# StandeHaas/Hydrodynamic-Limits-of-Active-Particle-Systems-with-Mean-Field-Interactions

Hardware: AMD Instinct MI355X
Metric: particle-steps/sec at N=1e5 (higher is better)
Workload: dtype f64; 1 GPU; BASELINE config 2: N=100000 particles, L=200000 sites, K=1, reflecting walls, sigma=0.005 (4001-tap table), beta=0.7, dt=0.0125, exclusion on; method=tiles

## Files before the change

### hydrodynamic-limits-of-active-particle-systems-with-mean-field-interactions_amd/capi.py

```python
from __future__ import annotations

import ctypes as C
import importlib.util
import os
import re
import sys

import numpy as np

HERE = os.path.dirname(os.path.abspath(__file__))
LIB_PATH = os.environ.get("APS_LIB") or os.path.join(HERE, "libaps_hip.so")
HEADER_PATH = os.path.join(os.path.dirname(HERE), "include", "aps.h")

APS_OK, APS_ERR_ARG, APS_ERR_HIP, APS_ERR_STATE, APS_ERR_NODEVICE = 0, -1, -2, -3, -4
METHODS = {"auto": 0, "pairs": 1, "lattice": 2, "tiles": 3}
KERNELS = ("pair_accumulate", "propose", "claim", "apply", "plan_tiles", "propose_lattice", "field_update", "tile_step")


class ApsError(RuntimeError):
    def __init__(self, code, text):
        super().__init__(f"libaps_hip error {code}: {text}")
        self.code = code


class ApsParams(C.Structure):
    _fields_ = [
        ("L", C.c_int32), ("K", C.c_int32), ("periodic", C.c_int32), ("minus_anchor", C.c_int32),
        ("immobilize", C.c_int32), ("suppress_flip", C.c_int32), ("crowding", C.c_int32),
        ("n_ensembles", C.c_int32), ("n_particles", C.c_int64), ("sigma_grid", C.c_double),
        ("rate_diffusion", C.c_double), ("rate_active", C.c_double), ("k_on", C.c_double),
        ("k_off", C.c_double), ("k_exit", C.c_double), ("dt", C.c_double), ("seed", C.c_uint64),
        ("beta", C.POINTER(C.c_double)), ("anchor_mask", C.POINTER(C.c_uint8)), ("device", C.c_int32),
        ("rank", C.c_int32), ("world", C.c_int32), ("sort_by_site", C.c_int32),
        ("ensemble_base", C.c_int32), ("method", C.c_int32), ("fp32", C.c_int32), ("halo_interval", C.c_int32),
    ]


_lib = None


def header_symbols():
    with open(HEADER_PATH) as fh:
        text = fh.read()
    return sorted(set(re.findall(r"\b(aps_[a-z_0-9]+)\s*\(", text)))


def _share_hip_runtime_with_torch():
    if "torch" in sys.modules or os.environ.get("APS_SYSTEM_HIP_RUNTIME") == "1":
        return None
    spec = importlib.util.find_spec("torch")
    if spec is None or not spec.submodule_search_locations:
        return None
    cand = os.path.join(list(spec.submodule_search_locations)[0], "lib", "libamdhip64.so")
    return C.CDLL(cand, mode=C.RTLD_GLOBAL) if os.path.exists(cand) else None


def load():
    global _lib
    if _lib is not None:
        return _lib
    _share_hip_runtime_with_torch()
    if not os.path.exists(LIB_PATH):
        raise ImportError(f"{LIB_PATH} is missing: build it with `python {os.path.join(HERE, 'build.py')}` "
                          "(hipcc --offload-arch=gfx950). There is no CPU fallback.")
    lib = C.CDLL(LIB_PATH)
    vp, i32, i64, dbl = C.c_void_p, C.c_int32, C.c_int64, C.c_double
    P = C.POINTER
    protos = {
        "aps_device_count": (C.c_int, []),
        "aps_last_error": (C.c_char_p, [vp]),
        "aps_create": (C.c_int, [P(ApsParams), P(vp)]),
        "aps_destroy": (None, [vp]),
        "aps_set_stream": (C.c_int, [vp, vp]),
        "aps_set_state": (C.c_int, [vp, i32, vp, vp, vp, vp, i64]),
        "aps_get_state": (C.c_int, [vp, i32, vp, vp, vp, vp, i64]),
        "aps_pair_accumulate": (C.c_int, [vp, i32, vp, vp, vp, i64]),
        "aps_step": (C.c_int, [vp, i64]),
        "aps_propose": (C.c_int, [vp]),
        "aps_commit": (C.c_int, [vp]),
        "aps_exchange_buffer": (C.c_int, [vp, P(vp), P(i64), P(i64), P(i64)]),
        "aps_bind_exchange_buffer": (C.c_int, [vp, vp, i64]),
        "aps_observe": (C.c_int, [vp, i32, vp, vp, vp]),
        "aps_field_from_counts": (C.c_int, [vp, i32, vp, vp, vp]),
        "aps_time": (C.c_int, [vp, P(dbl), P(i64)]),
        "aps_get_exits": (C.c_int, [vp, i32, vp, i64, P(i64)]),
        "aps_get_table": (C.c_int, [vp, vp, i32, P(i32), P(i32)]),
        "aps_resort": (C.c_int, [vp]),
        "aps_step_timed": (C.c_int, [vp, i64, P(dbl), P(i64), P(dbl)]),
        "aps_step_profile": (C.c_int, [vp, i64, vp, vp]),
        "aps_step_info": (C.c_int, [vp, P(i64), P(i64)]),
        "aps_set_resident_loop": (C.c_int, [vp, i32]),
        "aps_step_loop_timed": (C.c_int, [vp, i64, P(dbl), P(i64)]),
        "aps_loop_info": (C.c_int, [vp, P(i64), P(i32), C.c_char_p, i32]),
        "aps_copy_bandwidth": (C.c_int, [vp, i64, i32, P(dbl)]),
        "aps_lattice_accumulate": (C.c_int, [vp, i32, vp, vp, vp, i64]),
        "aps_get_lattice": (C.c_int, [vp, i32, vp, vp, vp]),
        "aps_method": (C.c_int, [vp]),
        "aps_mark_reference": (C.c_int, [vp, i32]),
        "aps_observe_scalars": (C.c_int, [vp, i32, i32, i32, i32, vp, vp]),
        "aps_observe_scalars_all": (C.c_int, [vp, i32, vp, vp, vp]),
        "aps_event_overhead": (C.c_int, [vp, i32, P(dbl)]),
        "aps_observe_structure": (C.c_int, [vp, i32, i32, vp]),
        "aps_observe_bins": (C.c_int, [vp, i32, i32, vp, vp]),
        "aps_rates_from_field": (C.c_int, [vp, i32, vp, vp, vp, i64, vp, vp, vp, vp]),
        "aps_comm_unique_id": (C.c_int, [vp]),
        "aps_comm_init": (C.c_int, [vp, vp]),
        "aps_comm_ranks": (C.c_int, [vp, P(i32)]),
        "aps_owned_sites": (C.c_int, [vp, P(i32), P(i32)]),
        "aps_halo_copy": (C.c_int, [vp, vp]),
        "aps_halo_pack": (C.c_int, [vp, i32, vp, i64, P(i64)]),
        "aps_halo_unpack": (C.c_int, [vp, i32, vp, i64]),
        "aps_halo_info": (C.c_int, [vp, P(i32), P(i32), P(i32)]),
        "aps_comm_selftest": (C.c_int, [vp, i64]),
        "aps_halo_sizes": (C.c_int, [vp, P(i64), P(i64)]),
        "aps_ipc_export": (C.c_int, [vp, vp]),
        "aps_ipc_connect": (C.c_int, [vp, vp, vp]),
        "aps_exchange_kind": (C.c_int, [vp]),
        "aps_set_flip_table": (C.c_int, [vp, vp, i32]),
        "aps_ntt_info": (C.c_int, [vp, P(i32), P(i32), P(dbl), P(i64)]),
        "aps_ntt_launches": (C.c_int, [vp]),
        "aps_tiles_info": (C.c_int, [vp, P(i32), P(i32), P(i32), P(i32)]),
    }
    lenient = os.environ.get("APS_LIB_LENIENT") == "1"
    for name, (res, args) in protos.items():
        if lenient and not hasattr(lib, name):
            continue
        fn = getattr(lib, name)
        fn.restype, fn.argtypes = res, args
    lib._aps_protos = protos
    _lib = lib
    return lib


def _ptr(a):
    return None if a is None else a.ctypes.data_as(C.c_void_p)


class Handle:

    def __init__(self, *, L, K, periodic, sigma_grid, rate_diffusion, rate_active, beta, dt, seed,
                 n_particles, minus_anchor=True, immobilize=True, suppress_flip=True, crowding=False,
                 k_on=0.0, k_off=0.0, k_exit=0.0, anchor_mask=None, device=0, rank=0, world=1,
                 sort_by_site=True, ensemble_base=0, method="auto", fp32=False, halo_interval=0):
        self.lib = load()
        self._h = C.c_void_p()
        betas = np.atleast_1d(np.asarray(beta, dtype=np.float64)).copy()
        self.E, self.n, self.L, self.K = len(betas), int(n_particles), int(L), int(K)
        self.dt = float(dt)
        mask = None if anchor_mask is None else np.ascontiguousarray(anchor_mask, dtype=np.uint8)
        if mask is not None and not mask.any():
            mask = None
        par = ApsParams(L=L, K=K, periodic=int(bool(periodic)), minus_anchor=int(bool(minus_anchor)),
                        immobilize=int(bool(immobilize)), suppress_flip=int(bool(suppress_flip)),
                        crowding=int(bool(crowding)), n_ensembles=self.E, n_particles=self.n,
                        sigma_grid=float(sigma_grid), rate_diffusion=float(rate_diffusion),
                        rate_active=float(rate_active), k_on=float(k_on), k_off=float(k_off),
                        k_exit=float(k_exit), dt=self.dt, seed=int(seed) & (2 ** 64 - 1),
                        beta=betas.ctypes.data_as(C.POINTER(C.c_double)),
                        anchor_mask=None if mask is None else mask.ctypes.data_as(C.POINTER(C.c_uint8)),
                        device=int(device), rank=int(rank), world=int(world),
                        sort_by_site=int(bool(sort_by_site)), ensemble_base=int(ensemble_base), method=METHODS[method],
                        fp32=int(bool(fp32)), halo_interval=int(halo_interval))
        rc = self.lib.aps_create(C.byref(par), C.byref(self._h))
        if rc != APS_OK:
            raise ApsError(rc, self.lib.aps_last_error(None).decode())
        self.method = {1: "pairs", 2: "lattice", 3: "tiles"}[self.lib.aps_method(self._h)]

    def _ck(self, rc):
        if rc != APS_OK:
            raise ApsError(rc, self.lib.aps_last_error(self._h).decode())

    def close(self):
        if getattr(self, "_h", None) is not None and self._h.value:
            self.lib.aps_destroy(self._h)
            self._h = C.c_void_p()

    def __del__(self):
        try:
            self.close()
        except Exception:
            pass

    def set_stream(self, raw_stream):
        self._ck(self.lib.aps_set_stream(self._h, C.c_void_p(raw_stream)))

    def set_state(self, pos, sigma, bound=None, alive=None, ensemble=0):
        pos = np.ascontiguousarray(pos, dtype=np.int32)
        sigma = np.ascontiguousarray(sigma, dtype=np.int8)
        bound = None if bound is None else np.ascontiguousarray(bound, dtype=np.uint8)
        alive = None if alive is None else np.ascontiguousarray(alive, dtype=np.uint8)
        self._ck(self.lib.aps_set_state(self._h, ensemble, _ptr(pos), _ptr(sigma), _ptr(bound), _ptr(alive), len(pos)))
        self._n_set = getattr(self, "_n_set", {})
        self._n_set[ensemble] = len(pos)

    def get_state(self, ensemble=0):
        n = self._n_set[ensemble]
        pos, sigma = np.zeros(n, np.int32), np.zeros(n, np.int8)
        bound, alive = np.zeros(n, np.uint8), np.zeros(n, np.uint8)
        self._ck(self.lib.aps_get_state(self._h, ensemble, _ptr(pos), _ptr(sigma), _ptr(bound), _ptr(alive), n))
        return pos, sigma, bound, alive

    def pair_accumulate(self, ensemble=0):
        n = self._n_set[ensemble]
        S, W, occ4 = np.zeros(n), np.zeros(n), np.zeros((n, 4), np.int32)
        self._ck(self.lib.aps_pair_accumulate(self._h, ensemble, _ptr(S), _ptr(W), _ptr(occ4), n))
        return S, W, occ4

    def lattice_accumulate(self, ensemble=0):
        n = self._n_set[ensemble]
        S, W, occ4 = np.zeros(n), np.zeros(n), np.zeros((n, 4), np.int32)
        self._ck(self.lib.aps_lattice_accumulate(self._h, ensemble, _ptr(S), _ptr(W), _ptr(occ4), n))
        return S, W, occ4

    def get_lattice(self, ensemble=0):
        W, S, occ = np.zeros(self.L), np.zeros(self.L), np.zeros(self.L, np.int32)
        self._ck(self.lib.aps_get_lattice(self._h, ensemble, _ptr(W), _ptr(S), _ptr(occ)))
        return W, S, occ

    def step(self, nsteps=1):
        self._ck(self.lib.aps_step(self._h, int(nsteps)))

    def propose(self):
        self._ck(self.lib.aps_propose(self._h))

    def commit(self):
        self._ck(self.lib.aps_commit(self._h))

    def exchange_buffer(self):
        ptr, tot, off, mine = C.c_void_p(), C.c_int64(), C.c_int64(), C.c_int64()
        self._ck(self.lib.aps_exchange_buffer(self._h, C.byref(ptr), C.byref(tot), C.byref(off), C.byref(mine)))
        return ptr.value, tot.value, off.value, mine.value

    def bind_exchange_buffer(self, dev_ptr, nbytes):
        self._ck(self.lib.aps_bind_exchange_buffer(self._h, C.c_void_p(dev_ptr), int(nbytes)))

    def comm_init(self, id128: bytes):
        buf = (C.c_uint8 * 128).from_buffer_copy(id128)
        self._ck(self.lib.aps_comm_init(self._h, C.cast(buf, C.c_void_p)))

    def owned_sites(self):
        lo, hi = C.c_int32(), C.c_int32()
        self._ck(self.lib.aps_owned_sites(self._h, C.byref(lo), C.byref(hi)))
        return lo.value, hi.value

    def halo_from(self, neighbour):
        self._ck(self.lib.aps_halo_copy(self._h, neighbour._h))

    def halo_info(self):
        k, age, due = C.c_int32(0), C.c_int32(0), C.c_int32(0)
        self._ck(self.lib.aps_halo_info(self._h, C.byref(k), C.byref(age), C.byref(due)))
        return int(k.value), int(age.value), bool(due.value)

    def halo_sizes(self):
        snd, rcv = (C.c_int64 * 2)(), (C.c_int64 * 2)()
        self._ck(self.lib.aps_halo_sizes(self._h, snd, rcv))
        return (int(snd[0]), int(snd[1])), (int(rcv[0]), int(rcv[1]))

    def halo_pack(self, side):
        n = C.c_int64()
        self._ck(self.lib.aps_halo_pack(self._h, int(side), None, 0, C.byref(n)))
        buf = np.zeros(max(n.value, 1), np.uint8)
        self._ck(self.lib.aps_halo_pack(self._h, int(side), _ptr(buf), len(buf), C.byref(n)))
        return buf[:n.value]

    def halo_unpack(self, from_side, data):
        data = np.ascontiguousarray(data, dtype=np.uint8)
        self._ck(self.lib.aps_halo_unpack(self._h, int(from_side), _ptr(data), len(data)))

    def comm_selftest(self, nbytes=1 << 16):
        self._ck(self.lib.aps_comm_selftest(self._h, int(nbytes)))

    def ipc_export(self) -> bytes:
        buf = (C.c_uint8 * 256)()
        self._ck(self.lib.aps_ipc_export(self._h, C.cast(buf, C.c_void_p)))
        return bytes(buf)

    def ipc_connect(self, left_blob, right_blob):
        keep = [None if b is None else (C.c_uint8 * 256).from_buffer_copy(b) for b in (left_blob, right_blob)]
        self._ck(self.lib.aps_ipc_connect(self._h, *[None if k is None else C.cast(k, C.c_void_p) for k in keep]))

    def set_flip_table(self, table):
        if table is None:
            self._ck(self.lib.aps_set_flip_table(self._h, None, 0))
            return
        tab = np.ascontiguousarray(table, dtype=np.float64)
        assert tab.ndim == 2 and tab.shape[0] == 2 and tab.shape[1] >= 2
        self._ck(self.lib.aps_set_flip_table(self._h, _ptr(tab), tab.shape[1] - 1))

    def ntt_info(self):
        on, m, ms, n = C.c_int32(), C.c_int32(), C.c_double(), C.c_int64()
        self._ck(self.lib.aps_ntt_info(self._h, C.byref(on), C.byref(m), C.byref(ms), C.byref(n)))
        return dict(on=bool(on.value), log2_m=m.value, prof_ms=ms.value, prof_launches=n.value, launches=int(self.lib.aps_ntt_launches(self._h)))

    def tiles_info(self):
        v = [C.c_int32() for _ in range(4)]
        self._ck(self.lib.aps_tiles_info(self._h, *[C.byref(x) for x in v]))
        return dict(frame_sites=v[0].value, owned_sites=v[1].value, n_tiles=v[2].value, table_in_lds=bool(v[3].value))

    def exchange_kind(self):
        return {0: "none", 1: "rccl", 2: "ipc-peer"}[self.lib.aps_exchange_kind(self._h)]

    def comm_ranks(self):
        n = C.c_int32()
        self._ck(self.lib.aps_comm_ranks(self._h, C.byref(n)))
        return n.value

    def step_timed(self, nsteps):
        ms, n, pairs = C.c_double(), C.c_int64(), C.c_double()
        self._ck(self.lib.aps_step_timed(self._h, int(nsteps), C.byref(ms), C.byref(n), C.byref(pairs)))
        return ms.value, n.value, pairs.value

    def step_profile(self, nsteps):
        ms, cnt = np.zeros(len(KERNELS)), np.zeros(len(KERNELS), np.int64)
        self._ck(self.lib.aps_step_profile(self._h, int(nsteps), _ptr(ms), _ptr(cnt)))
        return {k: (float(m), int(c)) for k, m, c in zip(KERNELS, ms, cnt)}

    def step_info(self):
        g, k = C.c_int64(), C.c_int64()
        self._ck(self.lib.aps_step_info(self._h, C.byref(g), C.byref(k)))
        return g.value, k.value

    def set_resident_loop(self, on=True):
        self._ck(self.lib.aps_set_resident_loop(self._h, 1 if on else 0))

    def step_loop_timed(self, nsteps):
        ms, n = C.c_double(), C.c_int64()
        self._ck(self.lib.aps_step_loop_timed(self._h, int(nsteps), C.byref(ms), C.byref(n)))
        return ms.value, n.value

    def loop_info(self):
        n, st, why = C.c_int64(), C.c_int32(), C.create_string_buffer(256)
        self._ck(self.lib.aps_loop_info(self._h, C.byref(n), C.byref(st), why, 256))
        return n.value, st.value, why.value.decode()

    def copy_bandwidth(self, nbytes=1 << 30, reps=5):
        r = C.c_double()
        self._ck(self.lib.aps_copy_bandwidth(self._h, int(nbytes), int(reps), C.byref(r)))
        return r.value

    def event_overhead(self, reps=50):
        ms = C.c_double()
        self._ck(self.lib.aps_event_overhead(self._h, int(reps), C.byref(ms)))
        return ms.value

    SCALARS = ("n", "sum_sigma", "sum_pos", "n_wall", "max_pos", "n_range", "attempts", "blocked", "sum_d", "sum_d2", "n_d")

    def mark_reference(self, ensemble=0):
        self._ck(self.lib.aps_mark_reference(self._h, ensemble))

    def observe_scalars(self, ensemble=0, x_wall=0, range_lo=0, range_hi=-1, block_table=None):
        out = np.zeros(len(self.SCALARS), np.int64)
        tab = None if block_table is None else np.ascontiguousarray(block_table, dtype=np.uint8)
        if tab is not None and tab.size != (self.K + 1) ** 2:
            raise ValueError("block_table must have (K+1)*(K+1) entries")
        self._ck(self.lib.aps_observe_scalars(self._h, ensemble, int(x_wall), int(range_lo), int(range_hi), _ptr(tab), _ptr(out)))
        return {k: int(v) for k, v in zip(self.SCALARS, out)}

    def observe_scalars_all(self, x_wall=0, ranges=None, block_table=None):
        out = np.zeros((self.E, len(self.SCALARS)), np.int64)
        tab = None if block_table is None else np.ascontiguousarray(block_table, dtype=np.uint8)
        rng = None if ranges is None else np.ascontiguousarray(ranges, dtype=np.int32).reshape(self.E, 2)
        self._ck(self.lib.aps_observe_scalars_all(self._h, int(x_wall), _ptr(rng), _ptr(tab), _ptr(out)))
        return [{k: int(v) for k, v in zip(self.SCALARS, row)} for row in out]

    def observe_bins(self, nbins, ensemble=0):
        cp, cm = np.zeros(nbins, np.int64), np.zeros(nbins, np.int64)
        self._ck(self.lib.aps_observe_bins(self._h, ensemble, int(nbins), _ptr(cp), _ptr(cm)))
        return cp, cm

    def observe_structure(self, ensemble=0, k_max=25):
        k_max = int(min(k_max, self.L))
        out = np.zeros(4 + 2 * k_max)
        self._ck(self.lib.aps_observe_structure(self._h, ensemble, k_max, _ptr(out)))
        return int(out[0]), float(out[1]), float(out[2]), float(out[3]), out[4:].reshape(k_max, 2)

    def observe(self, ensemble=0, want_field=True):
        cp, cm = np.zeros(self.L, np.int64), np.zeros(self.L, np.int64)
        m = np.zeros(self.L) if want_field else None
        self._ck(self.lib.aps_observe(self._h, ensemble, _ptr(cp), _ptr(cm), _ptr(m)))
        return cp, cm, m

    def field_from_counts(self, counts_p, counts_m, ensemble=0):
        cp = np.ascontiguousarray(counts_p, dtype=np.int64)
        cm = np.ascontiguousarray(counts_m, dtype=np.int64)
        m = np.zeros(self.L)
        self._ck(self.lib.aps_field_from_counts(self._h, ensemble, _ptr(cp), _ptr(cm), _ptr(m)))
        return m

    def rates_from_field(self, pos, sigma, bound, m_field, counts_p, counts_m, ensemble=0):
        pos = np.ascontiguousarray(pos, dtype=np.int32)
        sigma = np.ascontiguousarray(sigma, dtype=np.int8)
        bound = np.ascontiguousarray(bound, dtype=np.uint8)
        m_field = np.ascontiguousarray(m_field, dtype=np.float64)
        cp = np.ascontiguousarray(counts_p, dtype=np.int64)
        cm = np.ascontiguousarray(counts_m, dtype=np.int64)
        out = np.zeros((9, len(pos)))
        self._ck(self.lib.aps_rates_from_field(self._h, ensemble, _ptr(pos), _ptr(sigma), _ptr(bound), len(pos), _ptr(m_field),
                                               _ptr(cp), _ptr(cm), _ptr(out)))
        return dict(zip(("diff", "act", "flip", "bind", "unbind", "exit", "left", "right", "total"), out))

    def time(self):
        t, k = C.c_double(), C.c_int64()
        self._ck(self.lib.aps_time(self._h, C.byref(t), C.byref(k)))
        return t.value, k.value

    def exits(self, ensemble=0):
        n = C.c_int64()
        self._ck(self.lib.aps_get_exits(self._h, ensemble, None, 0, C.byref(n)))
        rows = np.zeros((max(n.value, 1), 3))
        self._ck(self.lib.aps_get_exits(self._h, ensemble, _ptr(rows), len(rows), C.byref(n)))
        return rows[:n.value]

    def table(self):
        tlen, q = C.c_int32(), C.c_int32()
        self._ck(self.lib.aps_get_table(self._h, None, 0, C.byref(tlen), C.byref(q)))
        out = np.zeros(max(tlen.value, 1))
        self._ck(self.lib.aps_get_table(self._h, _ptr(out), len(out), C.byref(tlen), C.byref(q)))
        return out[:tlen.value], q.value

    def resort(self):
        self._ck(self.lib.aps_resort(self._h))


def device_count():
    return load().aps_device_count()


def comm_unique_id() -> bytes:
    lib = load()
    buf = (C.c_uint8 * 128)()
    rc = lib.aps_comm_unique_id(C.cast(buf, C.c_void_p))
    if rc != APS_OK:
        raise ApsError(rc, lib.aps_last_error(None).decode())
    return bytes(buf)
```

### hydrodynamic-limits-of-active-particle-systems-with-mean-field-interactions_amd/csrc/aps_hip.hip

```cpp

#include <hip/hip_runtime.h>
#include <hip/hip_ext.h>
#include <dlfcn.h>
#include <unistd.h>
#include <rccl/rccl.h>
#include <algorithm>
#include <cmath>
#include <cstdint>
#include <cstdio>
#include <cstdlib>
#include <cstring>
#include <numeric>
#include <string>
#include <vector>

#include "aps.h"
#include "aps_common.hpp"
#include "dev_mem.hpp"

namespace {

constexpr uint32_t POS_MASK = 0x07FFFFFFu;
constexpr uint32_t SPIN_BIT = 1u << 27;
constexpr uint32_t BOUND_BIT = 1u << 28;
// ... 1161 lines not shown
            (uint32_t)s | ((c & CELL_PLUS) ? SPIN_BIT : 0u) | ((c & CELL_BOUND) ? BOUND_BIT : 0u);
    }
    occ_site[(size_t)e * L + s] = (uint32_t)n;
}

__global__ __launch_bounds__(256) void mark_away(uint32_t *src, size_t n) {
    const size_t i = (size_t)blockIdx.x * blockDim.x + threadIdx.x;
    if (i < n && !(src[i] & DEAD_BIT)) src[i] |= AWAY_BIT;
}

__global__ __launch_bounds__(256) void derive_slots(const uint32_t *__restrict__ src, uint32_t *sp8, int4 *tinfo, int Npad, int ntiles) {
    const size_t slot = (size_t)blockIdx.x * blockDim.x + threadIdx.x;
    const int e = blockIdx.y;
    const uint32_t me = src[(size_t)e * Npad + slot];
    const bool live = !(me & (DEAD_BIT | AWAY_BIT));
    const int p = (int)(me & POS_MASK);
    sp8[(size_t)e * Npad + slot] = live ? (((uint32_t)p << 3) | ((me & SPIN_BIT) ? 1u : 0u)) : DEAD_P8;
    int lo = live ? p : 0x7fffffff, hi = live ? p : -1, cnt = live ? 1 : 0;
#pragma unroll
    for (int off = 32; off > 0; off >>= 1) {
        lo = min(lo, __shfl_xor(lo, off)); hi = max(hi, __shfl_xor(hi, off)); cnt += __shfl_xor(cnt, off);
    }
    if ((threadIdx.x & 63) == 0) tinfo[(size_t)e * ntiles + slot / TILE] = make_int4(lo, hi, cnt < TILE ? 1 : 0, cnt);
}

__global__ __launch_bounds__(256) void tile_parts(const uint32_t *__restrict__ cell, long long *gpart, long long *gsum, int L, int K, int own, int ntile) {
    const int tile = blockIdx.x, e = blockIdx.y;
    const int s0 = tile * own, s1 = min(s0 + own, L);
    long long sp = 0, n = 0;
    for (int i = threadIdx.x; i < (s1 - s0) * K; i += blockDim.x) {
        const uint32_t c = cell[((size_t)e * L + s0) * K + i];
        if (c != CELL_EMPTY) { sp += (c & CELL_PLUS) ? 1 : -1; n += 1; }
    }
    __shared__ long long acc[2];
    if (threadIdx.x == 0) acc[0] = acc[1] = 0;
    __syncthreads();
    const long long a0 = wave_sum(sp), a1 = wave_sum(n);
    if ((threadIdx.x & 63) == 0) {
        atomicAdd(reinterpret_cast<unsigned long long *>(&acc[0]), (unsigned long long)a0);
        atomicAdd(reinterpret_cast<unsigned long long *>(&acc[1]), (unsigned long long)a1);
    }
    __syncthreads();
    if (threadIdx.x == 0) {
        gpart[((size_t)e * ntile + tile) * 2] = acc[0]; gpart[((size_t)e * ntile + tile) * 2 + 1] = acc[1];
        atomicAdd(reinterpret_cast<unsigned long long *>(&gsum[2 * e]), (unsigned long long)acc[0]);
        atomicAdd(reinterpret_cast<unsigned long long *>(&gsum[2 * e + 1]), (unsigned long long)acc[1]);
    }
}

__global__ __launch_bounds__(256) void structure_sites(const uint32_t *__restrict__ cnt_pm, const double *__restrict__ m_field, int L, double *out) {
    double c2 = 0.0, m1 = 0.0, m2 = 0.0;
    for (int x = blockIdx.x * blockDim.x + threadIdx.x; x < L; x += gridDim.x * blockDim.x) {
        const uint32_t c = cnt_pm[x];
        const double tot = (double)((c & 0xFFFFu) + (c >> 16)), m = m_field[x];
        c2 += tot * tot; m1 += m; m2 += m * m;
    }
#pragma unroll
    for (int off = 32; off > 0; off >>= 1) { c2 += __shfl_xor(c2, off); m1 += __shfl_xor(m1, off); m2 += __shfl_xor(m2, off); }
    if ((threadIdx.x & 63) == 0) { atomicAdd(&out[1], c2); atomicAdd(&out[2], m1); atomicAdd(&out[3], m2); }
}

__global__ __launch_bounds__(256) void structure_dft(const uint32_t *__restrict__ src, int Npad, int L, double *out) {
    const int k = blockIdx.x;
    double re = 0.0, im = 0.0, n = 0.0;
    for (int i = threadIdx.x; i < Npad; i += blockDim.x) {
        const uint32_t w = src[i];
        if (w & (DEAD_BIT | AWAY_BIT)) continue;
        const long long r = ((long long)k * (long long)(w & POS_MASK)) % (long long)L;
        double sn, cs;
        sincospi(-2.0 * ((double)r / (double)L), &sn, &cs);
        re += cs; im += sn; n += 1.0;
    }
    __shared__ double acc[3];
    if (threadIdx.x < 3) acc[threadIdx.x] = 0.0;
    __syncthreads();
#pragma unroll
    for (int off = 32; off > 0; off >>= 1) { re += __shfl_xor(re, off); im += __shfl_xor(im, off); n += __shfl_xor(n, off); }
    if ((threadIdx.x & 63) == 0) { atomicAdd(&acc[0], re); atomicAdd(&acc[1], im); atomicAdd(&acc[2], n); }
    __syncthreads();
    if (threadIdx.x == 0) { out[4 + 2 * k] = acc[0]; out[5 + 2 * k] = acc[1]; if (k == 0) out[0] = acc[2]; }
}

__global__ __launch_bounds__(256) void bin_counts(const uint32_t *__restrict__ src, int Npad, int bin_sites, unsigned long long *plus, unsigned long long *minus,
                                                  int site_lo, int site_hi) {
    const int i = blockIdx.x * blockDim.x + threadIdx.x;
    if (i >= Npad) return;
    const uint32_t w = src[i];
    if (w & (DEAD_BIT | AWAY_BIT)) return;
    if ((int)(w & POS_MASK) < site_lo || (int)(w & POS_MASK) >= site_hi) return;
    atomicAdd(((w & SPIN_BIT) ? plus : minus) + (w & POS_MASK) / (uint32_t)bin_sites, 1ull);
}

std::string g_create_error;

}

struct aps_handle {
    DevMem mem;
    aps_params p{};
    Model model{};
    std::vector<double> beta;
    std::vector<double> table;
    int tlen = 0, q = 0;
    bool table_in_lds = true;
    size_t lds_bytes = 0, lds_bytes_field = 0;
    int E = 1, world = 1, rank = 0;
    int64_t N = 0, Npad = 0, SH = 0, ntiles = 0;
    hipStream_t stream = nullptr;
    bool own_stream = false;
    uint32_t *d_src = nullptr, *d_orig = nullptr, *d_pcnt = nullptr, *d_plist = nullptr;
    uint8_t *d_prop = nullptr, *d_prop_own = nullptr, *d_anchor = nullptr;
    uint32_t *d_sp8 = nullptr;
    int4 *d_tinfo = nullptr;
    unsigned long long *d_stamps = nullptr;
    uint32_t *d_plan = nullptr, *d_plan_n = nullptr;
    double *d_accW = nullptr, *d_accS = nullptr;
    unsigned *d_occ = nullptr;
    int split = 1;
    bool plan_dirty = true;
    int plan_interval = 1, plan_age = 0;
    int num_cu = 256, wgs_per_cu = 1;
    double *d_table = nullptr, *d_beta = nullptr, *d_exit = nullptr, *d_S = nullptr, *d_W = nullptr, *d_mfield = nullptr;
    int *d_occ4 = nullptr;
    long long *d_gsum = nullptr;
    unsigned *d_nexit = nullptr;
    uint32_t *d_tmp_sp8 = nullptr; int4 *d_tmp_tinfo = nullptr; size_t tmp_cap = 0;
    int exit_cap = 0;
    int64_t step = 0;
    std::vector<int64_t> n_set;
    std::vector<hipEvent_t> events;
    ncclComm_t comm = nullptr;
    int method = APS_METHOD_PAIRS;
    double2 *d_ws = nullptr;
    uint32_t *d_occ_site = nullptr;
    uint32_t *d_dcnt = nullptr, *d_dep = nullptr;
    unsigned long long *d_stepw = nullptr;
    int bshift = 8, nb = 0, dcap = 0, fu_R = 1;
    bool fu_table_in_lds = true;
    bool field_dirty = true;
    hipStream_t cap_stream = nullptr;
    hipGraphExec_t gexec_f[2][2][6] = {};
    hipGraphExec_t gexact_f[2][2][65] = {};
    bool graphs_built_f[2] = {false, false};
    int flip = 0;
    int64_t last_graph_steps = 0, last_single_steps = 0;
    double2 *d_wsb[2] = {nullptr, nullptr};
    uint32_t *d_cell[2] = {nullptr, nullptr}, *d_tdcnt[2] = {nullptr, nullptr}, *d_tdep[2] = {nullptr, nullptr};
    long long *d_gpart[2] = {nullptr, nullptr};
    uint32_t *d_slot_of = nullptr;
    Model *d_model = nullptr; TileRare *d_rare = nullptr;
    unsigned long long *d_xrec = nullptr;
    unsigned *d_abort = nullptr, *h_abort = nullptr, *h_abort_dev = nullptr;
    int loop_rec = 0, loop_drec = 0, loop_seg = 0;
    int loop_state = -2;
    int loop_wanted = 1;
    uint32_t loop_tag = 0;
    int64_t last_loop_steps = 0;
    unsigned loop_stall = 0u;
    uint32_t *loop_dbg = nullptr; int loop_dbg_n = 0;
    bool loop_timed = false;
    hipEvent_t loop_ev[2] = {nullptr, nullptr};
    std::string loop_why;
    bool f32 = false, ws_view_stale = false;
    double *d_flip_tab = nullptr;
    bool ntt_on = false, ntt_fused = false;
    NttPlan ntt{};
    uint32_t *d_ntt_sig = nullptr, *d_ntt_tab = nullptr;
    int *d_ntt_csig = nullptr;
    double prof_ntt_ms = 0.0; int64_t prof_ntt_n = 0;
    int *d_table_i = nullptr;
    int2 *d_wsi[2] = {nullptr, nullptr};
    int ts_lo = 0, ts_hi = 0, own_lo = 0, own_hi = 0, ts_reach = 0;
    int ts_kx = 1, halo_age = 0;
    unsigned halo_got = 0;
    char *d_halo_send[2] = {nullptr, nullptr}, *d_halo_recv[2] = {nullptr, nullptr};
    HaloSegD *d_halo_seg_send[2] = {nullptr, nullptr}, *d_halo_seg_recv[2] = {nullptr, nullptr};
    int halo_nseg_send[2] = {0, 0}, halo_nseg_recv[2] = {0, 0};
    size_t halo_bytes_send[2] = {0, 0}, halo_bytes_recv[2] = {0, 0};
    char *ipc_land = nullptr;
    size_t ipc_land_bytes = 0, ipc_land_off[2][2] = {{0, 0}, {0, 0}};
    char *ipc_peer[2] = {nullptr, nullptr};
    void *ipc_opened[2] = {nullptr, nullptr};
    size_t ipc_peer_off[2][2] = {{0, 0}, {0, 0}};
    unsigned *d_ipc_done = nullptr, *h_ipc_err = nullptr, *h_ipc_err_dev = nullptr;
    uint32_t ipc_seq = 0;
    bool ipc_on = false;
    int ts_RS = 2, ts_own = 124, ts_ntile = 0, ts_dcap = 0;
    bool ts_table_in_lds = true;
    bool slots_dirty = false;
    bool field_pending = false;
    uint32_t *d_ref = nullptr, *d_cnt_pm = nullptr;
    uint8_t *d_block_table = nullptr, *d_ref_ok = nullptr; long long *d_scal = nullptr; int *d_lo_hi = nullptr;
    std::vector<char> ref_set;
    bool profiling = false;
    std::vector<int> prof_kind;
    size_t prof_n = 0;
    bool prof_dispatch = true;
    hipEvent_t k_start = nullptr, k_stop = nullptr;
    std::string err;
};

namespace {

#define HIP_TRY(h, expr)                                                                         \
    do {                                                                                         \
        hipError_t e_ = (expr);                                                                  \
        if (e_ != hipSuccess) {                                                                  \
            (h)->err = std::string(#expr) + ": " + hipGetErrorString(e_);                        \
            return APS_ERR_HIP;                                                                  \
        }                                                                                        \
    } while (0)

int fail(aps_handle *h, int code, const std::string &msg) { h->err = msg; return code; }
void drop_graphs(aps_handle *h);

struct Rccl {
    void *lib = nullptr;
    ncclResult_t (*GetUniqueId)(ncclUniqueId *) = nullptr;
    ncclResult_t (*CommInitRank)(ncclComm_t *, int, ncclUniqueId, int) = nullptr;
    ncclResult_t (*AllGather)(const void *, void *, size_t, ncclDataType_t, ncclComm_t, hipStream_t) = nullptr;
    ncclResult_t (*CommDestroy)(ncclComm_t) = nullptr;
    ncclResult_t (*CommCount)(const ncclComm_t, int *) = nullptr;
    ncclResult_t (*Send)(const void *, size_t, ncclDataType_t, int, ncclComm_t, hipStream_t) = nullptr;
    ncclResult_t (*Recv)(void *, size_t, ncclDataType_t, int, ncclComm_t, hipStream_t) = nullptr;
    ncclResult_t (*GroupStart)() = nullptr;
    ncclResult_t (*GroupEnd)() = nullptr;
    const char *(*GetErrorString)(ncclResult_t) = nullptr;
    std::string err;
    bool load() {
        if (lib) return true;
        for (const char *name : {"librccl.so.1", "librccl.so", "/opt/rocm/lib/librccl.so.1"}) {
            lib = dlopen(name, RTLD_NOW | RTLD_GLOBAL);
            if (lib) break;
        }
        if (!lib) { err = std::string("cannot load librccl: ") + dlerror(); return false; }
        GetUniqueId = reinterpret_cast<decltype(GetUniqueId)>(dlsym(lib, "ncclGetUniqueId"));
        CommInitRank = reinterpret_cast<decltype(CommInitRank)>(dlsym(lib, "ncclCommInitRank"));
        AllGather = reinterpret_cast<decltype(AllGather)>(dlsym(lib, "ncclAllGather"));
        CommDestroy = reinterpret_cast<decltype(CommDestroy)>(dlsym(lib, "ncclCommDestroy"));
        GetErrorString = reinterpret_cast<decltype(GetErrorString)>(dlsym(lib, "ncclGetErrorString"));
        CommCount = reinterpret_cast<decltype(CommCount)>(dlsym(lib, "ncclCommCount"));
        Send = reinterpret_cast<decltype(Send)>(dlsym(lib, "ncclSend"));
        Recv = reinterpret_cast<decltype(Recv)>(dlsym(lib, "ncclRecv"));
        GroupStart = reinterpret_cast<decltype(GroupStart)>(dlsym(lib, "ncclGroupStart"));
        GroupEnd = reinterpret_cast<decltype(GroupEnd)>(dlsym(lib, "ncclGroupEnd"));
        if (!GetUniqueId || !CommInitRank || !AllGather || !CommDestroy || !GetErrorString || !CommCount || !Send || !Recv || !GroupStart || !GroupEnd) {
            err = "librccl lacks a required symbol"; lib = nullptr; return false;
        }
        return true;
    }
} g_rccl;

void build_table(aps_handle *h) { weight_table(h->p.sigma_grid, h->p.L, h->p.K, h->p.periodic != 0, h->table, h->tlen, h->q, h->p.fp32 ? 29 : 51); }

template <typename T>
int dev_alloc(aps_handle *h, T **ptr, size_t count) {
    HIP_TRY(h, h->mem.alloc(ptr, count));
    HIP_TRY(h, hipMemsetAsync(*ptr, 0, std::max<size_t>(count, 1) * sizeof(T), h->stream));
    return APS_OK;
}

void derive_sources(const std::vector<uint32_t> &src, std::vector<uint32_t> &sp8, std::vector<int4> &tinfo) {
    const size_t n = src.size(), nt = n / TILE;
    sp8.resize(n);
    tinfo.assign(nt, make_int4(0x7fffffff, -1, 1, 0));
    for (size_t s = 0; s < n; ++s) {
        const uint32_t w = src[s];
        const bool live = !(w & DEAD_BIT);
        sp8[s] = live ? (((w & POS_MASK) << 3) | ((w & SPIN_BIT) ? 1u : 0u)) : DEAD_P8;
        if (!live) continue;
        int4 &t = tinfo[s / TILE];
        const int p = (int)(w & POS_MASK);
        t.x = std::min(t.x, p); t.y = std::max(t.y, p); t.w += 1;
    }
    for (int4 &t : tinfo) t.z = t.w < TILE ? 1 : 0;
}

void pack_ensemble(const aps_handle *h, const int32_t *pos, const int8_t *sigma, const uint8_t *bound,
                   const uint8_t *alive, int64_t n, std::vector<uint32_t> &src, std::vector<uint32_t> &orig,
                   long long gsum[2]) {
    const int64_t Npad = h->Npad;
    std::vector<uint32_t> order((size_t)n);
    std::iota(order.begin(), order.end(), 0u);
    if (h->p.sort_by_site)
        std::stable_sort(order.begin(), order.end(), [&](uint32_t a, uint32_t b) {
            const bool da = alive && !alive[a], db = alive && !alive[b];
            if (da != db) return db;
            return pos[a] < pos[b];
        });
    src.assign((size_t)Npad, DEAD_BIT);
    orig.assign((size_t)Npad, 0xFFFFFFFFu);
    gsum[0] = gsum[1] = 0;
    for (int64_t s = 0; s < n; ++s) {
        const uint32_t i = order[(size_t)s];
        uint32_t w = (uint32_t)pos[i] & POS_MASK;
        if (sigma[i] > 0) w |= SPIN_BIT;
        if (bound && bound[i]) w |= BOUND_BIT;
        const bool dead = alive && !alive[i];
        if (dead) w |= DEAD_BIT;
        else { gsum[0] += sigma[i] > 0 ? 1 : -1; gsum[1] += 1; }
        src[(size_t)s] = w;
        orig[(size_t)s] = i;
    }
}

int upload_ensemble(aps_handle *h, int e, const std::vector<uint32_t> &src, const std::vector<uint32_t> &orig) {
// ... 429 lines not shown

int ntt_setup(aps_handle *h) {
    h->ntt_on = false;
    const char *env = std::getenv("APS_NTT");
    if (env && env[0] == '0') return APS_OK;
    const bool forced = env && env[0] == '1';
    if (!is_tiles(h) || !h->model.field_mode) return APS_OK;
    if (h->ts_table_in_lds && !forced) return APS_OK;
    const int Rt = h->tlen - 1, L = h->p.L;
    const bool shard = h->world > 1;
    int64_t span = (int64_t)L + 2 * Rt;
    if (!shard) {
        if (h->p.periodic ? !(2 * Rt <= L && L >= 4 * TD_SITES) : !(2 * Rt + 64 * h->ts_RS + h->ts_own + 4 < L)) return APS_OK;
    } else {
        const char *kenv = std::getenv("APS_HALO_INTERVAL");
        if (h->p.halo_interval > 1 || (h->p.halo_interval == 0 && kenv && std::atoi(kenv) > 1)) return APS_OK;
        int own_min = L, own_max = 0;
        for (int r = 0; r < h->world; ++r) {
            int lo, hi;
            rank_tiles(h, r, lo, hi);
            const int n = std::min(L, hi * h->ts_own) - lo * h->ts_own;
            own_min = std::min(own_min, n); own_max = std::max(own_max, n);
        }
        span = (int64_t)own_max + 2 * (Rt + TD_HALO);
        if (own_min < Rt + TD_HALO + 1 || (h->p.periodic && span > L)) return APS_OK;
    }
    const int np = h->f32 ? 1 : 2;
    int m = shard && np == 2 ? 15 : 14;
    while (((int64_t)1 << m) < span) ++m;
    if (m > 21 || (np == 2 && m < 15) || td_lds_bytes(h->p.K) > 160 * 1024) return APS_OK;
    if (td_lds_bytes(h->p.K) > 48 * 1024) {
        const void *fn = h->f32 ? reinterpret_cast<const void *>(&tile_dense<false, true>) : reinterpret_cast<const void *>(&tile_dense<false, false>);
        if (hipFuncSetAttribute(fn, hipFuncAttributeMaxDynamicSharedMemorySize, (int)td_lds_bytes(h->p.K)) != hipSuccess) { (void)hipGetLastError(); return APS_OK; }
    }
    double wsum = 0.0;
    for (int t = 0; t < h->tlen; ++t) wsum += std::ldexp(h->table[(size_t)t], h->q) * (t ? 2.0 : 1.0);
    if (2.0 * h->p.K * wsum >= 0.5 * (np == 1 ? (double)NTT_PRIMES[0] : (double)NTT_PRIMES[0] * (double)NTT_PRIMES[1])) return APS_OK;
    NttPlan &pl = h->ntt;
    pl.m = m; ntt_split(m, pl.a0, pl.a1, pl.a2); pl.L = L; pl.Rt = Rt; pl.E = h->E; pl.np = np;
    pl.org = shard ? h->own_lo - Rt - TD_HALO : -Rt;
    pl.out_lo = shard ? h->own_lo - TD_HALO : 0;
    pl.out_hi = shard ? h->own_hi + TD_HALO : L;
    if (shard && !h->p.periodic) { pl.out_lo = std::max(pl.out_lo, 0); pl.out_hi = std::min(pl.out_hi, L); }
    pl.crt_inv = ntt_powmod(NTT_PRIMES[0] % NTT_PRIMES[1], NTT_PRIMES[1] - 2ull, NTT_PRIMES[1]);
    pl.unit = std::ldexp(1.0, -h->q);
    const size_t M = (size_t)1 << m;
    NttTables T[2];
    for (int k = 0; k < np; ++k) ntt_build_tables(m, NTT_PRIMES[k], NTT_ROOTS[k], T[k]);
    const size_t o_wr = 0, o_t1 = o_wr + T[0].wr.size(), o_hi = o_t1 + T[0].t1.size(), o_lo = o_hi + T[0].t2hi.size(), o_what = o_lo + T[0].t2lo.size(),
                 o_whatp = o_what + M, per_prime = o_whatp + M;
    int rc;
    if ((rc = dev_alloc(h, &h->d_ntt_tab, per_prime * np)) || (rc = dev_alloc(h, &h->d_ntt_sig, (size_t)np * h->E * 2 * M)) ||
        (rc = dev_alloc(h, &h->d_ntt_csig, (size_t)h->E * 2 * M))) return rc;
    for (int k = 0; k < np; ++k) {
        uint32_t *tb = h->d_ntt_tab + (size_t)k * per_prime;
        HIP_TRY(h, hipMemcpyAsync(tb + o_wr, T[k].wr.data(), T[k].wr.size() * 4, hipMemcpyHostToDevice, h->stream));
        HIP_TRY(h, hipMemcpyAsync(tb + o_t1, T[k].t1.data(), T[k].t1.size() * 4, hipMemcpyHostToDevice, h->stream));
        HIP_TRY(h, hipMemcpyAsync(tb + o_hi, T[k].t2hi.data(), T[k].t2hi.size() * 4, hipMemcpyHostToDevice, h->stream));
        HIP_TRY(h, hipMemcpyAsync(tb + o_lo, T[k].t2lo.data(), T[k].t2lo.size() * 4, hipMemcpyHostToDevice, h->stream));
        NttPrime &pp = pl.pr[k];
        pp.P = NTT_PRIMES[k]; pp.md.P = (double)NTT_PRIMES[k]; pp.md.Pinv = 1.0 / (double)NTT_PRIMES[k];
        pp.wr = tb + o_wr; pp.t1 = tb + o_t1; pp.t2hi = tb + o_hi; pp.t2lo = tb + o_lo; pp.what = tb + o_what; pp.whatp = tb + o_whatp;
    }
    if (np == 1) pl.pr[1] = pl.pr[0];
    const char *fenv = std::getenv("APS_NTT_FUSED");
    h->ntt_fused = pl.a0 == 7 && pl.a1 == 7 && pl.a2 >= 1 && !(fenv && fenv[0] == '0');
    if (h->ntt_fused && hipFuncSetAttribute(reinterpret_cast<const void *>(&ntt_mid), hipFuncAttributeMaxDynamicSharedMemorySize, (int)NTT_MID_LDS) != hipSuccess) {
        (void)hipGetLastError(); h->ntt_fused = false;
    }
    {
        NttPlan ps = pl;
        ps.E = 1;
        std::vector<uint32_t> wext((size_t)np * 2 * M, 0u);
        for (int k = 0; k < np; ++k)
            for (int t = 0; t < h->tlen; ++t) {
                const uint32_t v = (uint32_t)((unsigned long long)std::ldexp(h->table[(size_t)t], h->q) % NTT_PRIMES[k]);
                wext[(size_t)k * 2 * M + (size_t)t] = v;
                if (t && !(h->p.periodic && 2 * t == L)) wext[(size_t)k * 2 * M + M - (size_t)t] = v;
            }
        HIP_TRY(h, hipMemcpyAsync(h->d_ntt_sig, wext.data(), wext.size() * 4, hipMemcpyHostToDevice, h->stream));
        const dim3 grid((unsigned)(M / NTT_TILE), 1u, (unsigned)np), block(NTT_THREADS);
        if (pl.a2 > 0) ntt_launch_strided<2, false, 1>(pl.a2, grid, block, h->stream, nullptr, nullptr, false, ps, h->d_ntt_sig, nullptr, nullptr, 0);
        ntt_launch_strided<1, false, 1>(pl.a1, grid, block, h->stream, nullptr, nullptr, false, ps, h->d_ntt_sig, nullptr, nullptr, 0);
        hipLaunchKernelGGL((ntt_contig<true>), grid, block, 0, h->stream, ps, h->d_ntt_sig);
        HIP_TRY(h, hipGetLastError());
        std::vector<uint32_t> spec(M), specp;
        for (int k = 0; k < np; ++k) {
            HIP_TRY(h, hipMemcpyAsync(spec.data(), h->d_ntt_sig + (size_t)k * 2 * M, M * 4, hipMemcpyDeviceToHost, h->stream));
            HIP_TRY(h, hipStreamSynchronize(h->stream));
            const uint32_t P = NTT_PRIMES[k], minv = ntt_powmod((uint32_t)(M % P), P - 2ull, P);
            for (size_t i = 0; i < M; ++i) spec[i] = ntt_mulmod_u64(spec[i], minv, P);
            HIP_TRY(h, hipMemcpy(h->d_ntt_tab + (size_t)k * per_prime + o_what, spec.data(), M * 4, hipMemcpyHostToDevice));
            if (h->ntt_fused) {
                specp.resize(M);
                auto brev7 = [](size_t v) { size_t r = 0; for (int b = 0; b < 7; ++b) r |= ((v >> b) & 1) << (6 - b); return r; };
                for (size_t k2 = 0; k2 < (M >> 14); ++k2)
                    for (size_t s0 = 0; s0 < 128; ++s0)
                        for (size_t s1 = 0; s1 < 128; ++s1) specp[(k2 << 14) + s0 * 128 + s1] = spec[(k2 << 14) + brev7(s1) * 128 + brev7(s0)];
                HIP_TRY(h, hipMemcpy(h->d_ntt_tab + (size_t)k * per_prime + o_whatp, specp.data(), M * 4, hipMemcpyHostToDevice));
            }
        }
    }
    HIP_TRY(h, hipMemsetAsync(h->d_ntt_sig, 0, (size_t)np * h->E * 2 * M * 4, h->stream));
    HIP_TRY(h, hipStreamSynchronize(h->stream));
    if (h->d_wsi[1] != h->d_wsi[0]) { h->mem.release(h->d_wsi[1]); h->d_wsi[1] = h->d_wsi[0]; }
    if (!h->f32 && h->d_wsb[1] != h->d_wsb[0]) { h->mem.release(h->d_wsb[1]); h->d_wsb[1] = h->d_wsb[0]; }
    if (shard) h->ts_kx = 1;
    h->ntt_on = true;
    return APS_OK;
}

template <bool F32>
const void *tl_kernel_f(bool periodic, int RS, bool k1) {
#define TL_PICK(BC, R) (k1 ? (const void *)&tile_loop<BC, R, true, F32> : (const void *)&tile_loop<BC, R, false, F32>)
#define TL_CASE(R) case R: return periodic ? TL_PICK(1, R) : TL_PICK(0, R);
    if (!F32 && (RS == 8 || (RS == 7 && !k1))) return nullptr;
#ifdef APS_DEV_RS
    switch (RS) { TL_CASE(APS_DEV_RS) default: return nullptr; }
#else
    if constexpr (F32) { if (RS == 8) return periodic ? TL_PICK(1, 8) : TL_PICK(0, 8); }
    switch (RS) {
        TL_CASE(1) TL_CASE(2) TL_CASE(3) TL_CASE(4) TL_CASE(5) TL_CASE(6)
        case 7: return k1 ? (periodic ? (const void *)&tile_loop<1, 7, true, F32> : (const void *)&tile_loop<0, 7, true, F32>)
                          : (F32 ? (periodic ? (const void *)&tile_loop<1, 7, false, true> : (const void *)&tile_loop<0, 7, false, true>) : nullptr);
        default: return nullptr;
    }
#endif
#undef TL_CASE
#undef TL_PICK
}
const void *tl_kernel(const aps_handle *h) {
    return h->f32 ? tl_kernel_f<true>(h->p.periodic != 0, h->ts_RS, h->p.K == 1) : tl_kernel_f<false>(h->p.periodic != 0, h->ts_RS, h->p.K == 1);
}

int loop_prepare(aps_handle *h) {
    if (h->loop_state != -2) return APS_OK;
    h->loop_state = 0;
    auto no = [&](const char *why) { h->loop_why = why; return APS_OK; };
    if (!is_tiles(h)) return no("not the tiles formulation");
    if (h->world != 1) return no("sharded handle");
    if (h->ntt_on) return no("field updated by the exact convolution");
    if (!h->ts_table_in_lds) return no("weight table beyond LDS");
    if (!h->model.field_mode) return no("global mean field");
    if (h->p.K == 1 && h->model.immobilize && h->model.k_exit > 0.0) return no("particles can leave the system (one cell per site)");
    if (3 * h->p.K > 32) return no("site capacity above 10");
    if (h->p.L - (int64_t)(h->ts_ntile - 1) * h->ts_own < 3) return no("last tile shorter than three sites");
#ifdef APS_STAMPS
    return no("diagnostic build");
#endif
    const void *fn = tl_kernel(h);
    if (!fn) return no("no kernel for this frame");
    const int64_t need_per_cu = ((int64_t)h->ts_ntile * h->E + h->num_cu - 1) / h->num_cu;
    h->loop_seg = 0;
    size_t lds_total = 0;
    for (int seg : {256, 192, 128, TL_SEG_MIN}) {
        const TlLds lay = tl_lds_layout(h->tlen, h->ts_RS, h->ts_own, h->p.K, ts_wbytes(h), seg);
        if (lay.total > 160 * 1024) continue;
        if (128 / (int)((lay.total + 1279) / 1280) >= need_per_cu) { h->loop_seg = seg; lds_total = lay.total; break; }
    }
    if (!h->loop_seg) return no("more tiles than the device keeps resident at once (LDS)");
    if (lds_total > 48 * 1024 && hipFuncSetAttribute(fn, hipFuncAttributeMaxDynamicSharedMemorySize, (int)lds_total) != hipSuccess) { (void)hipGetLastError(); return no("hipFuncSetAttribute failed"); }
    int per_cu = 0;
    if (hipOccupancyMaxActiveBlocksPerMultiprocessor(&per_cu, fn, FU_THREADS, lds_total) != hipSuccess) { (void)hipGetLastError(); return no("occupancy query failed"); }
    if (need_per_cu > std::min(per_cu, 8)) return no("more tiles than the device keeps resident at once");
    h->loop_drec = (h->ts_dcap / 16 + 1) * 16;
    h->loop_rec = (h->loop_drec + 6 * h->p.K + 15) / 16 * 16;
    int rc;
    if ((rc = dev_alloc(h, &h->d_xrec, (size_t)2 * h->E * h->ts_ntile * h->loop_rec)) || (rc = dev_alloc(h, &h->d_abort, 4))) return rc;
    HIP_TRY(h, h->mem.alloc_host_mapped(&h->h_abort, &h->h_abort_dev, 16));
    h->h_abort[0] = 0u;
    h->loop_tag = 0;
    h->loop_state = 1;
    return APS_OK;
}

int launch_tile_loop(aps_handle *h, int64_t n) {
    LoopArgs la{};
    la.a = tile_args(h, false);
    la.a.tile_lo = 0;
    la.step0 = (unsigned long long)h->step;
    la.nsteps = (int)n;
    if ((uint64_t)h->loop_tag + (uint64_t)n + 2 > 0xFFFFFFF0ull) {
        HIP_TRY(h, hipMemsetAsync(h->d_xrec, 0, (size_t)2 * h->E * h->ts_ntile * h->loop_rec * sizeof(unsigned long long), h->stream));
        h->loop_tag = 0;
    }
    la.tag0 = h->loop_tag;
    h->loop_tag += (uint32_t)n + 1u;
    la.rec = h->loop_rec; la.drec = h->loop_drec; la.xrec = h->d_xrec; la.seg = h->loop_seg;
    la.abort_dev = h->d_abort; la.abort_host = h->h_abort_dev;
    la.timeout_ticks = 5000000ull;
    if (const char *env = std::getenv("APS_LOOP_TIMEOUT_MS")) la.timeout_ticks = (unsigned long long)std::max(1, std::atoi(env)) * 100000ull;
#ifdef APS_LOOP_DEBUG
    static uint32_t *dbg = nullptr;
    if (!dbg) (void)hipMalloc(reinterpret_cast<void **>(&dbg), (size_t)64 * 3 * h->p.L * 4);
    (void)hipMemsetAsync(dbg, 0xEE, (size_t)64 * 3 * h->p.L * 4, h->stream);
    la.dbg = n <= 64 ? dbg : nullptr;
    h->loop_dbg = dbg; h->loop_dbg_n = (int)n;
#endif
    if (std::getenv("APS_LOOP_TEST_ABORT")) HIP_TRY(h, hipMemsetAsync(h->d_abort, 1, 4, h->stream));
    {
        unsigned stall = 0u;
        if (const char *env = std::getenv("APS_LOOP_TEST_STALL")) {
            int st_tile = -1, st_it = 0;
            if (std::sscanf(env, "%d:%d", &st_tile, &st_it) == 2 && st_tile >= 0 && st_tile < h->ts_ntile && st_it >= 0 && st_it < 0xFFFF)
                stall = ((unsigned)(st_tile + 1) << 16) | (unsigned)st_it;
        }
        if (stall != h->loop_stall) {
            HIP_TRY(h, hipMemcpyAsync(h->d_abort + 1, &stall, 4, hipMemcpyHostToDevice, h->stream));
            HIP_TRY(h, hipStreamSynchronize(h->stream));
            h->loop_stall = stall;
        }
    }
    const void *fn = tl_kernel(h);
    const size_t lds = tl_lds_layout(h->tlen, h->ts_RS, h->ts_own, h->p.K, ts_wbytes(h), h->loop_seg).total;
    const void *table_ptr = h->f32 ? (const void *)h->d_table_i : (const void *)h->d_table;
    void *args[] = {(void *)&la, (void *)&table_ptr};
    const dim3 grid((unsigned)h->ts_ntile, (unsigned)h->E), block(FU_THREADS);
    if (h->loop_timed) {
        for (hipEvent_t &ev : h->loop_ev) if (!ev) HIP_TRY(h, hipEventCreate(&ev));
        HIP_TRY(h, hipExtLaunchKernel(fn, grid, block, args, lds, h->stream, h->loop_ev[0], h->loop_ev[1], 0));
    } else
        HIP_TRY(h, hipLaunchKernel(fn, grid, block, args, lds, h->stream));
    return APS_OK;
}

struct HaloSeg { size_t off, bytes; int array; };

void halo_segments(const aps_handle *h, int owner_lo_tile, int owner_hi_tile, int side, bool recv, std::vector<HaloSeg> &out) {
    const int L = h->p.L, K = h->p.K, own = h->ts_own;
    const int s_lo = owner_lo_tile * own, s_hi = std::min(L, owner_hi_tile * own);
    if (h->ntt_on) {
        const int reach = h->ntt.Rt + TD_HALO;
        const size_t M = (size_t)1 << h->ntt.m;
        const int p0 = !recv ? (side == 0 ? s_lo - 1 : s_hi - reach) - h->ntt.org
                             : (side == 0 ? h->own_hi - 1 : h->own_lo - reach) - h->ntt.org;
        for (int e = 0; e < h->E; ++e) {
            const int c0 = side == 0 ? s_lo : s_hi - 3, c1 = side == 0 ? s_lo + 3 : s_hi;
            out.push_back({((size_t)e * L + c0) * K * 4, (size_t)(c1 - c0) * K * 4, 0});
            for (int sg = 0; sg < 2; ++sg) out.push_back({(((size_t)e * 2 + sg) * M + (size_t)p0) * 4, (size_t)(reach + 1) * 4, 4});
        }
        return;
    }
    const int nt = std::min(h->ts_kx * h->ts_reach, owner_hi_tile - owner_lo_tile);
    const int64_t gs = (int64_t)(h->ts_kx - 1) * h->ts_reach * own;
    for (int e = 0; e < h->E; ++e) {
        const int64_t g1 = std::min<int64_t>(s_hi, (int64_t)owner_hi_tile * own - gs);
        const int c0 = side == 0 ? s_lo : (int)std::max<int64_t>(s_lo, g1 - 3);
        const int c1 = side == 0 ? (int)std::min<int64_t>(s_hi, s_lo + gs + 3) : s_hi;
        const int w0 = side == 0 ? s_lo : (int)std::max<int64_t>(s_lo, g1 - 2);
        const int w1 = side == 0 ? (int)std::min<int64_t>(s_hi, s_lo + gs + 2) : s_hi;
        const int t0 = side == 0 ? owner_lo_tile : owner_hi_tile - nt, t1 = t0 + nt;
        out.push_back({((size_t)e * L + c0) * K * 4, (size_t)(c1 - c0) * K * 4, 0});
        if (h->model.field_mode) {
            out.push_back({((size_t)e * L + w0) * 2 * ts_wbytes(h), (size_t)(w1 - w0) * 2 * ts_wbytes(h), 1});
            out.push_back({((size_t)e * h->ts_ntile + t0) * 4, (size_t)(t1 - t0) * 4, 2});
            out.push_back({((size_t)e * h->ts_ntile + t0) * h->ts_dcap * 4, (size_t)(t1 - t0) * h->ts_dcap * 4, 3});
        }
    }
}

char *halo_array(aps_handle *h, int array, int buf) {
    switch (array) {
        case 0: return reinterpret_cast<char *>(h->d_cell[buf]);
        case 1: return h->f32 ? reinterpret_cast<char *>(h->d_wsi[buf]) : reinterpret_cast<char *>(h->d_wsb[buf]);
        case 2: return reinterpret_cast<char *>(h->d_tdcnt[buf]);
        case 3: return reinterpret_cast<char *>(h->d_tdep[buf]);
        default: return reinterpret_cast<char *>(h->d_ntt_csig);
    }
}

void rank_tiles(const aps_handle *h, int r, int &lo, int &hi) {
    lo = (int)((int64_t)r * h->ts_ntile / h->world);
    hi = (int)((int64_t)(r + 1) * h->ts_ntile / h->world);
}

void halo_peers(const aps_handle *h, int &left, int &right) {
    left = h->rank - 1; right = h->rank + 1;
    if (h->p.periodic) { left = (left + h->world) % h->world; right %= h->world; }
    else { if (right >= h->world) right = -1; }
}

int halo_setup(aps_handle *h) {
    int left, right, lo, hi;
    halo_peers(h, left, right);
    for (int side = 0; side < 2; ++side) {
        for (int recv = 0; recv < 2; ++recv) {
            std::vector<HaloSeg> segs;
            if (!recv) halo_segments(h, h->ts_lo, h->ts_hi, side, false, segs);
            else {
                const int peer = side == 0 ? right : left;
                if (peer < 0) continue;
                rank_tiles(h, peer, lo, hi);
                halo_segments(h, lo, hi, side, true, segs);
            }
            std::vector<HaloSegD> tab;
            size_t off = 0;
            for (const HaloSeg &g : segs) {
                if (!g.bytes) continue;
                tab.push_back({(unsigned long long)g.off, (unsigned long long)off, (unsigned)g.bytes, g.array});
                off += (g.bytes + 15) / 16 * 16;
            }
            HaloSegD **dseg = recv ? &h->d_halo_seg_recv[side] : &h->d_halo_seg_send[side];
            char **dmsg = recv ? &h->d_halo_recv[side] : &h->d_halo_send[side];
            (recv ? h->halo_nseg_recv[side] : h->halo_nseg_send[side]) = (int)tab.size();
            (recv ? h->halo_bytes_recv[side] : h->halo_bytes_send[side]) = off;
            int rc;
            if ((rc = dev_alloc(h, dseg, tab.size())) || (rc = dev_alloc(h, dmsg, off))) return rc;
            HIP_TRY(h, hipMemcpyAsync(*dseg, tab.data(), tab.size() * sizeof(HaloSegD), hipMemcpyHostToDevice, h->stream));
        }
    }
    HIP_TRY(h, hipStreamSynchronize(h->stream));
    return APS_OK;
}

int halo_launch(aps_handle *h, int side, bool unpack) {
    const int buf = (int)((h->step & 1) ^ 1);
    const int nseg = unpack ? h->halo_nseg_recv[side] : h->halo_nseg_send[side];
    if (!nseg) return APS_OK;
    hipLaunchKernelGGL(halo_move, dim3((unsigned)(nseg * HALO_BPS)), dim3(256), 0, h->stream,
                       unpack ? h->d_halo_seg_recv[side] : h->d_halo_seg_send[side], halo_array(h, 0, buf), halo_array(h, 1, buf),
                       halo_array(h, 2, buf), halo_array(h, 3, buf), halo_array(h, HALO_ADD, buf), unpack ? h->d_halo_recv[side] : h->d_halo_send[side], unpack ? 1 : 0);
    HIP_TRY(h, hipGetLastError());
    return APS_OK;
}

unsigned halo_expected(const aps_handle *h) {
    int left, right;
    halo_peers(h, left, right);
    return (right >= 0 && h->halo_nseg_recv[0] ? 1u : 0u) | (left >= 0 && h->halo_nseg_recv[1] ? 2u : 0u);
}

bool halo_due(const aps_handle *h) { return h->world > 1 && h->halo_age + 1 == h->ts_kx; }

bool halo_prepacked(const aps_handle *h) { return h->ntt_on && h->world > 1 && !h->ipc_on && !h->comm; }

int halo_exchange_rccl(aps_handle *h) {
    int left, right, rc;
    halo_peers(h, left, right);
    if (left >= 0 && (rc = halo_launch(h, 0, false))) return rc;
    if (right >= 0 && (rc = halo_launch(h, 1, false))) return rc;
    ncclResult_t nr = g_rccl.GroupStart();
    if (nr == ncclSuccess && left >= 0 && h->halo_bytes_send[0]) nr = g_rccl.Send(h->d_halo_send[0], h->halo_bytes_send[0], ncclUint8, left, h->comm, h->stream);
    if (nr == ncclSuccess && right >= 0 && h->halo_bytes_send[1]) nr = g_rccl.Send(h->d_halo_send[1], h->halo_bytes_send[1], ncclUint8, right, h->comm, h->stream);
    if (nr == ncclSuccess && right >= 0 && h->halo_bytes_recv[0]) nr = g_rccl.Recv(h->d_halo_recv[0], h->halo_bytes_recv[0], ncclUint8, right, h->comm, h->stream);
    if (nr == ncclSuccess && left >= 0 && h->halo_bytes_recv[1]) nr = g_rccl.Recv(h->d_halo_recv[1], h->halo_bytes_recv[1], ncclUint8, left, h->comm, h->stream);
    const ncclResult_t ge = g_rccl.GroupEnd();
    if (nr == ncclSuccess) nr = ge;
    if (nr != ncclSuccess) return fail(h, APS_ERR_HIP, std::string("halo exchange (ncclSend/ncclRecv): ") + g_rccl.GetErrorString(nr));
    if (right >= 0 && (rc = halo_launch(h, 0, true))) return rc;
    if (left >= 0 && (rc = halo_launch(h, 1, true))) return rc;
    h->halo_got = halo_expected(h);
    return APS_OK;
}

int halo_exchange_ipc(aps_handle *h) {
    int left, right;
    halo_peers(h, left, right);
    const int buf = (int)((h->step & 1) ^ 1), par = (int)(h->ipc_seq & 1u);
    const unsigned tag = h->ipc_seq + 1u;
    HaloPushArgs pu{};
    HaloPullArgs pl{};
    const int peer_of_side[2] = {left, right};
    for (int side = 0; side < 2; ++side) {
        if (peer_of_side[side] >= 0 && h->halo_nseg_send[side]) {
            pu.segs[side] = h->d_halo_seg_send[side]; pu.nseg[side] = h->halo_nseg_send[side];
            pu.dst[side] = h->ipc_peer[side] + h->ipc_peer_off[side][par];
            pu.flag[side] = reinterpret_cast<unsigned long long *>(h->ipc_peer[side] + (size_t)(par * 2 + side) * 64);
// ... 112 lines not shown
        if (sigma[i] > 0) c |= CELL_PLUS;
        if (bound && bound[i]) c |= CELL_BOUND;
        cells[(size_t)pos[i] * K + (size_t)fill[(size_t)pos[i]]++] = c;
    }
    for (int64_t sl = 0; sl < h->Npad; ++sl) if (orig[(size_t)sl] != 0xFFFFFFFFu) slot_of[orig[(size_t)sl]] = (uint32_t)sl;
    HIP_TRY(h, hipMemcpyAsync(h->d_cell[cur] + (size_t)e * L * K, cells.data(), cells.size() * 4, hipMemcpyHostToDevice, h->stream));
    HIP_TRY(h, hipMemcpyAsync(h->d_slot_of + (size_t)e * h->N, slot_of.data(), (size_t)h->N * 4, hipMemcpyHostToDevice, h->stream));
    HIP_TRY(h, hipStreamSynchronize(h->stream));
    return APS_OK;
}

int do_propose(aps_handle *h) {
    if (is_tiles(h)) {
        int rc = launch_tile_step(h);
        if (!rc && h->ntt_on && h->world == 1) rc = run_ntt_conv(h);
        if (!rc && halo_prepacked(h)) {
            int left, right;
            halo_peers(h, left, right);
            if (left >= 0) rc = halo_launch(h, 0, false);
            if (!rc && right >= 0) rc = halo_launch(h, 1, false);
        }
        return rc;
    }
    if (h->method == APS_METHOD_LATTICE) {
        const LatticeArgs a = lattice_args(h, false, true);
        return launch_lattice_propose(h, a, a.tile_lo, a.tile_cnt);
    }
    const PairArgs a = pair_args(h, false, true);
    return launch_pair(h, a, a.tile_lo, a.tile_cnt);
}

int do_commit(aps_handle *h) {
    if (is_tiles(h)) {
        if (h->world > 1) {
            if (halo_due(h)) {
                if (h->halo_got != halo_expected(h)) return fail(h, APS_ERR_STATE, "aps_commit: the halo exchange is due before this commit (aps_halo_info)");
                if (h->ntt_on) {
                    int rc = run_ntt_conv(h);
                    if (rc) return rc;
                }
                h->halo_age = 0;
            } else h->halo_age += 1;
            h->halo_got = 0;
        }
        h->step += 1;
        return prof_mark(h, KIND_END);
    }
    const CommitArgs c = commit_args(h);
    const dim3 grid((unsigned)(h->Npad / 256), (unsigned)h->E), block(256);
    int rc;
    if (h->world != 1) {
        if ((rc = prof_mark(h, KIND_CLAIM))) return rc;
        APS_K(h, claim, grid, block, 0, c);
    }
    if ((rc = prof_mark(h, KIND_APPLY))) return rc;
    APS_K(h, apply, grid, block, 0, c);
    HIP_TRY(h, hipGetLastError());
    h->step += 1;
    if (h->method == APS_METHOD_LATTICE) {
        h->plan_dirty = true;
        if ((rc = launch_field_update(h))) return rc;
    } else if (++h->plan_age >= h->plan_interval) {
        if ((rc = launch_plan(h, (int)(h->rank * h->SH / TILE), (int)(h->SH / TILE)))) return rc;
        h->plan_dirty = false;
    }
    return prof_mark(h, KIND_END);
}

bool all_set(const aps_handle *h) {
    for (int64_t n : h->n_set) if (n < 0) return false;
    return true;
}

}

namespace { int download_hook(aps_handle *h, int e, double *S, double *W, int32_t *occ4); }

extern "C" {

int aps_device_count(void) {
    int n = 0;
    if (hipGetDeviceCount(&n) != hipSuccess) return 0;
    return n;
}

const char *aps_last_error(const aps_handle *h) { return h ? h->err.c_str() : g_create_error.c_str(); }

int aps_create(const aps_params *p, aps_handle **out) {
    if (!p || !out) { g_create_error = "aps_create: null argument"; return APS_ERR_ARG; }
    *out = nullptr;
    auto bad = [&](const char *m) { g_create_error = std::string("aps_create: ") + m; return APS_ERR_ARG; };
    if (p->L < 2 || p->L > (1 << 25)) return bad("L must be in [2, 2^25]");
    if (p->K < 1 || p->K > 32) return bad("site capacity K must be in [1, 32]");
    if (p->n_ensembles < 1) return bad("n_ensembles must be >= 1");
    if (p->n_particles < 0 || p->n_particles > (int64_t)p->K * p->L) return bad("n_particles must be in [0, K*L]");
    if (!(p->dt > 0.0)) return bad("dt must be > 0");
    if (!p->beta) return bad("beta pointer is null");
    if (p->world < 1 || p->rank < 0 || p->rank >= p->world) return bad("bad rank/world");
    if (p->method != APS_METHOD_AUTO && p->method != APS_METHOD_PAIRS && p->method != APS_METHOD_LATTICE && p->method != APS_METHOD_TILES)
        return bad("method must be APS_METHOD_AUTO, _PAIRS, _LATTICE or _TILES");
    int ndev = 0;
    if (hipGetDeviceCount(&ndev) != hipSuccess || ndev < 1) { g_create_error = "aps_create: no HIP device"; return APS_ERR_NODEVICE; }
    if (p->device < 0 || p->device >= ndev) return bad("device ordinal out of range");

    aps_handle *h = new aps_handle();
    h->p = *p;
    h->beta.assign(p->beta, p->beta + p->n_ensembles);
    h->p.beta = nullptr;
    h->E = p->n_ensembles; h->world = p->world; h->rank = p->rank; h->N = p->n_particles;
    const int64_t per_rank = (h->N + h->world - 1) / h->world;
    h->SH = std::max<int64_t>(256, (per_rank + 255) / 256 * 256);
    h->Npad = h->SH * h->world;
    h->ntiles = h->Npad / TILE;
    h->n_set.assign((size_t)h->E, -1);
    Model &M = h->model;
    M.L = p->L; M.K = p->K; M.periodic = p->periodic ? 1 : 0; M.field_mode = p->sigma_grid > 0.0 ? 1 : 0;
    M.minus_anchor = p->minus_anchor ? 1 : 0; M.immobilize = p->immobilize ? 1 : 0;
    M.suppress_flip = p->suppress_flip ? 1 : 0; M.crowding = p->crowding ? 1 : 0;
    M.rate_diffusion = p->rate_diffusion; M.rate_active = p->rate_active; M.k_on = p->k_on; M.k_off = p->k_off;
    M.k_exit = p->k_exit; M.dt = p->dt; M.seed_lo = (uint32_t)p->seed; M.seed_hi = (uint32_t)(p->seed >> 32);
    M.ens_base = p->ensemble_base;
    build_table(h);
    {
        const int B = 1 << h->bshift;
        h->nb = (p->L + B - 1) / B;
        h->dcap = (int)std::min<int64_t>(2LL * p->K * B, std::max<int64_t>(2 * p->n_particles, 2));
        const double dep_bytes = (double)h->E * h->nb * h->dcap * 4.0;
        const bool tiles_ok = p->n_particles < (int64_t)CELL_ID && dep_bytes <= 16e9 && (p->world == 1 || M.field_mode);
        if (p->method == APS_METHOD_TILES && !tiles_ok) { delete h; return bad("method tiles needs fewer than 2^30 - 1 particles and, sharded, a local field (sigma_grid > 0)"); }
        h->method = p->method == APS_METHOD_AUTO ? ((tiles_ok && p->world == 1) ? APS_METHOD_TILES : (dep_bytes <= 16e9 ? APS_METHOD_LATTICE : APS_METHOD_PAIRS)) : p->method;
        if (p->method == APS_METHOD_AUTO && h->method == APS_METHOD_TILES && !p->fp32 && dep_bytes <= 16e9 &&
            (32.0 + 8.0 * p->K) * (double)p->L * (double)h->E > 512e6)
            h->method = APS_METHOD_LATTICE;
        if (const char *env = std::getenv("APS_METHOD")) {
            if (p->method == APS_METHOD_AUTO && !std::strcmp(env, "pairs")) h->method = APS_METHOD_PAIRS;
            if (p->method == APS_METHOD_AUTO && !std::strcmp(env, "lattice")) h->method = APS_METHOD_LATTICE;
            if (p->method == APS_METHOD_AUTO && !std::strcmp(env, "tiles") && tiles_ok) h->method = APS_METHOD_TILES;
        }
        h->f32 = p->fp32 != 0 && h->method == APS_METHOD_TILES;
        if (p->fp32 && M.field_mode && h->q < 4) { delete h; return bad("fp32: the sums of this lattice do not fit a 32-bit field (q < 4)"); }
        ts_choose_geometry(h);
        h->fu_R = 2;
        double best = 1e300;
        for (int rs : {2, 3, 4, 5, 6, 7, 8}) {
            const double wgs = (double)(((int64_t)p->L + 64 * rs - 1) / (64 * rs)) * h->E;
            const double miss = std::fabs(wgs - 2.4 * 256.0);
            if (miss < best) { best = miss; h->fu_R = rs; }
        }
        if ((double)(((int64_t)p->L + 64 * 8 - 1) / (64 * 8)) * h->E > 8.0 * 256.0 && h->tlen <= 4096) h->fu_R = 7;
        if (const char *env = std::getenv("APS_FU_R")) { const int r = std::atoi(env); if (r >= 2 && r <= 8) h->fu_R = r; }
    }
    h->plan_interval = (!p->periodic && !(p->k_exit > 0.0)) ? 8 : 1;
    if (const char *env = std::getenv("APS_PLAN_INTERVAL")) h->plan_interval = std::max(1, std::atoi(env));

    auto die = [&](int code) { g_create_error = h->err; aps_destroy(h); return code; };
    if (hipSetDevice(p->device) != hipSuccess) { h->err = "hipSetDevice failed"; return die(APS_ERR_HIP); }
    if (hipStreamCreateWithFlags(&h->stream, hipStreamNonBlocking) != hipSuccess) { h->err = "hipStreamCreate failed"; return die(APS_ERR_HIP); }
    h->own_stream = true;
    int rc = set_lds_limit(h);
    if (rc) return die(rc);
    const size_t EN = (size_t)h->E * (size_t)h->Npad, EL = (size_t)h->E * (size_t)p->L;
    h->exit_cap = (int)std::max<int64_t>(h->N, 1);
    if ((rc = dev_alloc(h, &h->d_src, EN)) || (rc = dev_alloc(h, &h->d_orig, EN)) || (rc = dev_alloc(h, &h->d_prop_own, EN)) ||
        (rc = dev_alloc(h, &h->d_sp8, EN)) ||
        (rc = dev_alloc(h, &h->d_tinfo, (size_t)h->E * h->ntiles)) ||
        (rc = dev_alloc(h, &h->d_stamps, (size_t)8 * 4096)) ||
        (rc = dev_alloc(h, &h->d_plan, (size_t)h->E * h->ntiles * PLAN_CAP)) || (rc = dev_alloc(h, &h->d_plan_n, (size_t)h->E * h->ntiles)) ||
        (rc = dev_alloc(h, &h->d_accW, EN * MAX_SPLIT)) || (rc = dev_alloc(h, &h->d_accS, EN * MAX_SPLIT)) ||
        (rc = dev_alloc(h, &h->d_occ, EN * MAX_SPLIT)) || (rc = dev_alloc(h, &h->d_pcnt, 2 * EL)) ||
        (rc = dev_alloc(h, &h->d_plist, EL * 2 * p->K)) || (rc = dev_alloc(h, &h->d_table, h->table.size() + ((size_t)1 << h->bshift) + 8192))    ||
        (rc = dev_alloc(h, &h->d_beta, (size_t)h->E)) || (rc = dev_alloc(h, &h->d_gsum, (size_t)4 * h->E)) ||
        (rc = dev_alloc(h, &h->d_exit, (size_t)h->E * h->exit_cap * 3)) || (rc = dev_alloc(h, &h->d_nexit, (size_t)h->E)) ||
        (rc = dev_alloc(h, &h->d_mfield, (size_t)p->L)))
        return die(rc);
    h->d_prop = h->d_prop_own;
    if (h->method == APS_METHOD_LATTICE) {
        if ((rc = dev_alloc(h, &h->d_ws, EL)) || (rc = dev_alloc(h, &h->d_occ_site, EL)) ||
            (rc = dev_alloc(h, &h->d_dcnt, (size_t)h->E * h->nb)) || (rc = dev_alloc(h, &h->d_dep, (size_t)h->E * h->nb * h->dcap)) ||
            (rc = dev_alloc(h, &h->d_stepw, 2)))
            return die(rc);
    }
    if (h->method == APS_METHOD_TILES && h->world > 1 && (h->ts_kx < 1 || h->ts_kx * std::max(h->ts_reach, 1) > h->ts_ntile / h->world ||
                                                         (h->ts_ntile + h->world - 1) / h->world + 2 * (h->ts_kx - 1) * h->ts_reach > h->ts_ntile)) {
        h->err = "tiles, sharded: halo_interval " + std::to_string(h->ts_kx) + " x reach " + std::to_string(h->ts_reach) +
                 " tiles does not fit a rank's tile range (" + std::to_string(h->ts_ntile / h->world) + " tiles)";
        return die(APS_ERR_ARG);
    }
    if (h->method == APS_METHOD_TILES && h->world > 1 && 2 * h->ts_reach + 1 > h->ts_ntile / h->world) {
        h->err = "tiles, sharded: the table's reach (" + std::to_string(h->ts_reach) + " tiles) must stay below half a rank's tile range (" +
                 std::to_string(h->ts_ntile / h->world) + " tiles): fewer ranks or a larger lattice";
        return die(APS_ERR_ARG);
    }
    if (h->method == APS_METHOD_TILES) {
        const size_t ET = (size_t)h->E * h->ts_ntile;
        if ((rc = dev_alloc(h, &h->d_occ_site, EL)) || (rc = dev_alloc(h, &h->d_stepw, 2)) ||
            (rc = dev_alloc(h, &h->d_slot_of, (size_t)h->E * std::max<int64_t>(h->N, 1))))
            return die(rc);
        for (int b = 0; b < 2; ++b) {
            if ((rc = dev_alloc(h, &h->d_wsb[b], EL)) || (rc = dev_alloc(h, &h->d_cell[b], EL * p->K)) ||
                (rc = dev_alloc(h, &h->d_tdcnt[b], ET)) || (rc = dev_alloc(h, &h->d_tdep[b], ET * h->ts_dcap)) ||
                (rc = dev_alloc(h, &h->d_gpart[b], ET * 2)))
                return die(rc);
            if (hipMemsetAsync(h->d_cell[b], 0xFF, EL * p->K * 4, h->stream) != hipSuccess) { h->err = "cell init failed"; return die(APS_ERR_HIP); }
        }
        if ((rc = dev_alloc(h, &h->d_model, 1)) || (rc = dev_alloc(h, &h->d_rare, 1))) return die(rc);
        {
            const TileRare rare{h->d_exit, h->d_nexit, h->d_src, h->d_slot_of, h->d_stamps, (long long)h->N, h->exit_cap, (int)h->Npad, h->ts_lo, h->ts_hi};
            if (hipMemcpyAsync(h->d_model, &h->model, sizeof(Model), hipMemcpyHostToDevice, h->stream) != hipSuccess ||
                hipMemcpyAsync(h->d_rare, &rare, sizeof(TileRare), hipMemcpyHostToDevice, h->stream) != hipSuccess ||
                hipStreamSynchronize(h->stream) != hipSuccess) { h->err = "tile argument upload failed"; return die(APS_ERR_HIP); }
        }
        if (h->f32) {
            std::vector<int> ti(h->table.size());
            for (size_t i = 0; i < ti.size(); ++i) ti[i] = (int)std::ldexp(h->table[i], h->q);
            if ((rc = dev_alloc(h, &h->d_table_i, h->table.size() + ((size_t)1 << h->bshift) + 8192)) ||
                (rc = dev_alloc(h, &h->d_wsi[0], EL)) || (rc = dev_alloc(h, &h->d_wsi[1], EL))) return die(rc);
            if (hipMemcpyAsync(h->d_table_i, ti.data(), ti.size() * sizeof(int), hipMemcpyHostToDevice, h->stream) != hipSuccess ||
                hipStreamSynchronize(h->stream) != hipSuccess) { h->err = "integer table upload failed"; return die(APS_ERR_HIP); }
        }
        if ((rc = ntt_setup(h))) return die(rc);
        if (h->world > 1 && (rc = halo_setup(h))) return die(rc);
        const size_t need = ts_lds_layout(h->tlen, h->ts_table_in_lds, h->ts_RS, h->ts_own, p->K, ts_wbytes(h)).total;
        if (need > 160 * 1024) { h->err = "tiles: site capacity too large for the tile kernel's LDS staging"; return die(APS_ERR_ARG); }
        if (need > 48 * 1024 &&
            hipFuncSetAttribute(ts_kernel(p->periodic != 0, h->ts_table_in_lds, h->ts_RS, p->K == 1, h->f32), hipFuncAttributeMaxDynamicSharedMemorySize, (int)need) != hipSuccess) {
            h->err = "hipFuncSetAttribute(tile_step) failed"; return die(APS_ERR_HIP);
        }
    }
    if (p->anchor_mask) {
        if ((rc = dev_alloc(h, &h->d_anchor, (size_t)p->L))) return die(rc);
        if (hipMemcpyAsync(h->d_anchor, p->anchor_mask, (size_t)p->L, hipMemcpyHostToDevice, h->stream) != hipSuccess) { h->err = "anchor upload failed"; return die(APS_ERR_HIP); }
    }
    h->p.anchor_mask = nullptr;
    if (hipMemcpyAsync(h->d_table, h->table.data(), h->table.size() * sizeof(double), hipMemcpyHostToDevice, h->stream) != hipSuccess ||
        hipMemcpyAsync(h->d_beta, h->beta.data(), h->beta.size() * sizeof(double), hipMemcpyHostToDevice, h->stream) != hipSuccess ||
        hipStreamSynchronize(h->stream) != hipSuccess) { h->err = "table upload failed"; return die(APS_ERR_HIP); }
    *out = h;
    return APS_OK;
}

void aps_destroy(aps_handle *h) {
    if (!h) return;
    if (h->stream) (void)hipStreamSynchronize(h->stream);
    if (h->comm && g_rccl.CommDestroy) (void)g_rccl.CommDestroy(h->comm);
    for (hipEvent_t ev : h->events) (void)hipEventDestroy(ev);
    drop_graphs(h);
    if (h->cap_stream) (void)hipStreamDestroy(h->cap_stream);
    for (void *q : h->ipc_opened) if (q) (void)hipIpcCloseMemHandle(q);
    for (hipEvent_t ev : h->loop_ev) if (ev) (void)hipEventDestroy(ev);
    h->mem.free_all();
    if (h->own_stream && h->stream) (void)hipStreamDestroy(h->stream);
    delete h;
}

int aps_set_stream(aps_handle *h, void *hip_stream) {
    if (!h) return APS_ERR_ARG;
    HIP_TRY(h, hipStreamSynchronize(h->stream));
    if (h->own_stream && h->stream) { HIP_TRY(h, hipStreamDestroy(h->stream)); h->own_stream = false; }
    h->stream = reinterpret_cast<hipStream_t>(hip_stream);
    return APS_OK;
}

int aps_set_state(aps_handle *h, int32_t e, const int32_t *pos, const int8_t *sigma, const uint8_t *bound,
                  const uint8_t *alive, int64_t n) {
    if (!h) return APS_ERR_ARG;
    if (e < 0 || e >= h->E || !pos || !sigma || n < 0 || n > h->N) return fail(h, APS_ERR_ARG, "aps_set_state: bad ensemble, pointer or n");
    std::vector<int> occ((size_t)h->p.L, 0);
    for (int64_t i = 0; i < n; ++i) {
        if (pos[i] < 0 || pos[i] >= h->p.L) return fail(h, APS_ERR_ARG, "aps_set_state: position outside [0, L)");
        if (sigma[i] != 1 && sigma[i] != -1) return fail(h, APS_ERR_ARG, "aps_set_state: sigma must be +1 or -1");
        if (!(alive && !alive[i]) && ++occ[(size_t)pos[i]] > h->p.K) return fail(h, APS_ERR_ARG, "aps_set_state: site capacity exceeded");
    }
    std::vector<uint32_t> src, orig; long long gsum[2];
    int rc = sync_slots(h);
    if (rc) return rc;
    pack_ensemble(h, pos, sigma, bound, alive, n, src, orig, gsum);
    if ((rc = upload_ensemble(h, e, src, orig))) return rc;
    if (is_tiles(h) && (rc = upload_cells(h, e, pos, sigma, bound, alive, n, orig))) return rc;
    HIP_TRY(h, hipMemcpyAsync(h->d_gsum + (size_t)(h->step & 1) * 2 * h->E + 2 * e, gsum, sizeof(gsum), hipMemcpyHostToDevice, h->stream));
    HIP_TRY(h, hipMemsetAsync(h->d_nexit + e, 0, sizeof(unsigned), h->stream));
    if (h->d_occ_site) {
        static_assert(sizeof(int) == sizeof(uint32_t), "occupancy upload");
        HIP_TRY(h, hipMemcpyAsync(h->d_occ_site + (size_t)e * h->p.L, occ.data(), (size_t)h->p.L * 4, hipMemcpyHostToDevice, h->stream));
        h->field_dirty = true;
    }
    HIP_TRY(h, hipStreamSynchronize(h->stream));
    h->n_set[(size_t)e] = n;
    if (!h->ref_set.empty()) h->ref_set[(size_t)e] = 0;
    return APS_OK;
}

int aps_get_state(aps_handle *h, int32_t e, int32_t *pos, int8_t *sigma, uint8_t *bound, uint8_t *alive, int64_t n) {
    if (!h) return APS_ERR_ARG;
    if (e < 0 || e >= h->E) return fail(h, APS_ERR_ARG, "aps_get_state: bad ensemble");
    if (h->n_set[(size_t)e] < 0) return fail(h, APS_ERR_STATE, "aps_get_state: no state uploaded for this ensemble");
    if (n != h->n_set[(size_t)e]) return fail(h, APS_ERR_ARG, "aps_get_state: n differs from the uploaded particle count");
    { int rc_ = sync_slots(h); if (rc_) return rc_; }
    std::vector<uint32_t> src((size_t)h->Npad), orig((size_t)h->Npad);
    HIP_TRY(h, hipMemcpyAsync(src.data(), h->d_src + (size_t)e * h->Npad, src.size() * 4, hipMemcpyDeviceToHost, h->stream));
    HIP_TRY(h, hipMemcpyAsync(orig.data(), h->d_orig + (size_t)e * h->Npad, orig.size() * 4, hipMemcpyDeviceToHost, h->stream));
    HIP_TRY(h, hipStreamSynchronize(h->stream));
    for (int64_t s = 0; s < h->Npad; ++s) {
        const uint32_t i = orig[(size_t)s];
        if (i == 0xFFFFFFFFu) continue;
        if (i >= (uint64_t)n) return fail(h, APS_ERR_STATE, "aps_get_state: corrupt slot table");
        const uint32_t w = src[(size_t)s];
        if (pos) pos[i] = (int32_t)(w & POS_MASK);
        if (sigma) sigma[i] = (w & SPIN_BIT) ? 1 : -1;
        if (bound) bound[i] = (w & BOUND_BIT) ? 1 : 0;
        if (alive) alive[i] = (w & DEAD_BIT) ? 0 : ((w & AWAY_BIT) ? 2 : 1);
    }
    return APS_OK;
}

int aps_pair_accumulate(aps_handle *h, int32_t e, double *S, double *W, int32_t *occ4, int64_t n) {
    if (!h) return APS_ERR_ARG;
    if (e < 0 || e >= h->E || !S || !W || !occ4) return fail(h, APS_ERR_ARG, "aps_pair_accumulate: bad argument");
    if (!all_set(h)) return fail(h, APS_ERR_STATE, "aps_pair_accumulate: upload a state for every ensemble first");
    if (n != h->n_set[(size_t)e]) return fail(h, APS_ERR_ARG, "aps_pair_accumulate: n differs from the uploaded particle count");
    { int rc_ = sync_slots(h); if (rc_) return rc_; }
    const size_t EN = (size_t)h->E * (size_t)h->Npad;
    int rc;
    if (!h->d_S && ((rc = dev_alloc(h, &h->d_S, EN)) || (rc = dev_alloc(h, &h->d_W, EN)) || (rc = dev_alloc(h, &h->d_occ4, EN * 4)))) return rc;
    const PairArgs a = pair_args(h, true, false);
    if ((rc = launch_pair(h, a, 0, (int)h->ntiles))) return rc;
    return download_hook(h, e, S, W, occ4);
}

}

namespace {
int download_hook(aps_handle *h, int e, double *S, double *W, int32_t *occ4) {
    std::vector<double> s((size_t)h->Npad), w((size_t)h->Npad); std::vector<int> o((size_t)h->Npad * 4); std::vector<uint32_t> orig((size_t)h->Npad);
    HIP_TRY(h, hipMemcpyAsync(s.data(), h->d_S + (size_t)e * h->Npad, s.size() * 8, hipMemcpyDeviceToHost, h->stream));
    HIP_TRY(h, hipMemcpyAsync(w.data(), h->d_W + (size_t)e * h->Npad, w.size() * 8, hipMemcpyDeviceToHost, h->stream));
    HIP_TRY(h, hipMemcpyAsync(o.data(), h->d_occ4 + (size_t)e * h->Npad * 4, o.size() * 4, hipMemcpyDeviceToHost, h->stream));
    HIP_TRY(h, hipMemcpyAsync(orig.data(), h->d_orig + (size_t)e * h->Npad, orig.size() * 4, hipMemcpyDeviceToHost, h->stream));
    HIP_TRY(h, hipStreamSynchronize(h->stream));
    for (int64_t sl = 0; sl < h->Npad; ++sl) {
        const uint32_t i = orig[(size_t)sl];
        if (i == 0xFFFFFFFFu) continue;
        S[i] = s[(size_t)sl]; W[i] = w[(size_t)sl];
        for (int k = 0; k < 4; ++k) occ4[4 * (size_t)i + k] = o[4 * (size_t)sl + k];
    }
    return APS_OK;
}
}

extern "C" {

int aps_propose(aps_handle *h) {
    if (!h) return APS_ERR_ARG;
    if (!all_set(h)) return fail(h, APS_ERR_STATE, "aps_propose: upload a state for every ensemble first");
    int rc = ensure_lattice(h);
    if (rc) return rc;
    return do_propose(h);
}

int aps_commit(aps_handle *h) {
    if (!h) return APS_ERR_ARG;
    if (!all_set(h)) return fail(h, APS_ERR_STATE, "aps_commit: upload a state for every ensemble first");
    return do_commit(h);
}

}

namespace {

constexpr int NGRAPH = 6;
constexpr int GRAPH_SIZES[NGRAPH] = {32, 16, 8, 4, 2, 1};

// ... 67 lines not shown
        h->profiling = false;
        if (rc) return rc;
        HIP_TRY(h, hipStreamSynchronize(h->stream));
        if (h->prof_dispatch) {
            for (size_t i = 0; i < h->prof_kind.size(); ++i) {
                float t = 0.f;
                HIP_TRY(h, hipEventElapsedTime(&t, h->events[2 * i], h->events[2 * i + 1]));
                ms[h->prof_kind[i]] += t; counts[h->prof_kind[i]] += 1;
            }
        } else for (size_t i = 0; i + 1 < h->prof_n; ++i) {
            const int kind = h->prof_kind[i];
            if (kind == KIND_END) continue;
            float t = 0.f;
            HIP_TRY(h, hipEventElapsedTime(&t, h->events[i], h->events[i + 1]));
            ms[kind] += t; counts[kind] += 1;
        }
        if (work && (s == 0 || s == nsteps - 1)) {
            const double wgt = nsteps == 1 ? 1.0 : 0.5 * (double)nsteps;
            double t = 0.0;
            if (is_tiles(h)) {
                if (h->model.field_mode) {
                    HIP_TRY(h, hipMemcpy(pn.data(), h->d_tdcnt[h->step & 1], (size_t)h->E * h->ts_ntile * 4, hipMemcpyDeviceToHost));
                    for (size_t i = 0; i < (size_t)h->E * h->ts_ntile; ++i) t += (double)pn[i];
                }
            } else if (h->method == APS_METHOD_LATTICE) {
                if (h->model.field_mode) {
                    HIP_TRY(h, hipMemcpy(pn.data(), h->d_dcnt, (size_t)h->E * h->nb * 4, hipMemcpyDeviceToHost));
                    for (size_t i = 0; i < (size_t)h->E * h->nb; ++i) t += (double)pn[i];
                }
            } else {
                HIP_TRY(h, hipMemcpy(pn.data(), h->d_plan_n, (size_t)h->E * (h->ntiles / RT) * 4, hipMemcpyDeviceToHost));
                for (size_t i = 0; i < (size_t)h->E * (h->ntiles / RT); ++i) t += (double)pn[i] * RT * TILE * TILE;
            }
            *work += t * wgt;
        }
    }
    return APS_OK;
}

}

extern "C" {

int aps_step(aps_handle *h, int64_t nsteps) {
    if (!h) return APS_ERR_ARG;
    if (nsteps < 0) return fail(h, APS_ERR_ARG, "aps_step: nsteps < 0");
    if (h->world != 1 && !h->comm && !h->ipc_on)
        return fail(h, APS_ERR_STATE, "aps_step: sharded handle without transport; call aps_ipc_export / aps_ipc_connect or aps_comm_init, or use aps_propose / exchange / aps_commit");
    if (!all_set(h)) return fail(h, APS_ERR_STATE, "aps_step: upload a state for every ensemble first");
    int rc = ensure_lattice(h);
    if (rc) return rc;
    int64_t s = 0;
    static const bool no_graph = std::getenv("APS_NO_GRAPH") != nullptr;
    h->last_graph_steps = h->last_single_steps = h->last_loop_steps = 0;
    int64_t loop_min = (int64_t)h->ts_ntile * h->E > h->num_cu ? 10 : 3;
    if (const char *env = std::getenv("APS_LOOP_MIN")) loop_min = std::max(1, std::atoi(env));
    if (is_tiles(h) && h->world == 1 && !h->comm && h->loop_wanted && nsteps >= loop_min && h->loop_state != 0 && h->loop_state != -1) {
        const char *env = std::getenv("APS_TILE_LOOP");
        if (!(env && env[0] == '0')) {
            if ((rc = loop_prepare(h))) return rc;
            if (h->loop_state == 1) {
                const int64_t n = std::min<int64_t>(nsteps - s, (int64_t)1 << 30);
                const bool exits = h->model.k_exit > 0.0;
                std::vector<unsigned> n_exit_before;
                if (exits) {
                    n_exit_before.resize((size_t)h->E);
                    HIP_TRY(h, hipMemcpyAsync(n_exit_before.data(), h->d_nexit, (size_t)h->E * sizeof(unsigned), hipMemcpyDeviceToHost, h->stream));
                }
                if ((rc = launch_tile_loop(h, n))) return rc;
                HIP_TRY(h, hipStreamSynchronize(h->stream));
#ifdef APS_LOOP_DEBUG
                if (const char *path = std::getenv("APS_LOOP_DUMP")) {
                    std::vector<uint32_t> buf((size_t)h->loop_dbg_n * 3 * h->p.L);
                    (void)hipMemcpy(buf.data(), h->loop_dbg, buf.size() * 4, hipMemcpyDeviceToHost);
                    if (FILE *f = std::fopen(path, "wb")) { std::fwrite(buf.data(), 4, buf.size(), f); std::fclose(f); }
                }
#endif
                if (h->h_abort[0]) {
                    h->h_abort[0] = 0u;
                    h->loop_state = -1;
                    h->loop_why = "a wait ran out (the grid was not resident at once); steps repeated with one launch per step";
                    if ((rc = upload_stepw(h))) return rc;
                    if (exits) HIP_TRY(h, hipMemcpy(h->d_nexit, n_exit_before.data(), (size_t)h->E * sizeof(unsigned), hipMemcpyHostToDevice));
                } else {
                    h->step += n; s += n; h->last_loop_steps = n;
                    h->slots_dirty = true; h->field_pending = true; h->ws_view_stale = true;
                    if (!(n & 1)) {
                        std::swap(h->d_cell[0], h->d_cell[1]); std::swap(h->d_wsb[0], h->d_wsb[1]); std::swap(h->d_wsi[0], h->d_wsi[1]);
                        std::swap(h->d_tdcnt[0], h->d_tdcnt[1]); std::swap(h->d_tdep[0], h->d_tdep[1]); std::swap(h->d_gpart[0], h->d_gpart[1]);
                        h->d_ws = h->d_wsb[h->step & 1];
                        h->flip ^= 1;
                    }
                }
            }
        }
    }
    if ((h->method == APS_METHOD_LATTICE || is_tiles(h)) && h->world == 1 && !no_graph && nsteps > s) {
        if ((rc = build_graphs(h))) return rc;
        if (s == 0 && nsteps <= 64 && nsteps != 32 && nsteps != 16 && nsteps != 8 && nsteps != 4 && nsteps != 2 && nsteps != 1) {
            hipGraphExec_t &ge = h->gexact_f[h->flip][h->step & 1][nsteps];
            if (!ge && (rc = capture_run(h, (int)(h->step & 1), (int)nsteps, &ge))) return rc;
            HIP_TRY(h, hipGraphLaunch(ge, h->stream));
            h->step += nsteps; h->last_graph_steps += nsteps; s = nsteps;
            if (is_tiles(h)) { h->slots_dirty = true; h->field_pending = !h->ntt_on; h->ws_view_stale = true; }
        }
        for (int g = 0; g < NGRAPH; ++g)
            for (; nsteps - s >= GRAPH_SIZES[g]; s += GRAPH_SIZES[g]) {
                HIP_TRY(h, hipGraphLaunch(h->gexec_f[h->flip][h->step & 1][g], h->stream));
                h->step += GRAPH_SIZES[g];
                h->last_graph_steps += GRAPH_SIZES[g];
                if (is_tiles(h)) { h->slots_dirty = true; h->field_pending = !h->ntt_on; h->ws_view_stale = true; }
            }
    }
    for (; s < nsteps; ++s, ++h->last_single_steps)
        if ((rc = one_step(h))) return rc;
    HIP_TRY(h, hipStreamSynchronize(h->stream));
    if (h->h_ipc_err && h->h_ipc_err[0]) {
        h->h_ipc_err[0] = 0u;
        return fail(h, APS_ERR_STATE, "aps_step: a neighbour rank's halo did not arrive in time (peer-store transport); the state of this handle is incomplete");
    }
    return APS_OK;
}

int aps_set_resident_loop(aps_handle *h, int32_t on) {
    if (!h) return APS_ERR_ARG;
    h->loop_wanted = on ? 1 : 0;
    return APS_OK;
}

int aps_step_loop_timed(aps_handle *h, int64_t nsteps, double *kernel_ms, int64_t *loop_steps) {
    if (!h || !kernel_ms) return APS_ERR_ARG;
    h->loop_timed = true;
    const int rc = aps_step(h, nsteps);
    h->loop_timed = false;
    if (rc) return rc;
    *kernel_ms = 0.0;
    if (loop_steps) *loop_steps = h->last_loop_steps;
    if (h->last_loop_steps > 0) {
        float ms = 0.f;
        HIP_TRY(h, hipEventElapsedTime(&ms, h->loop_ev[0], h->loop_ev[1]));
        *kernel_ms = ms;
    }
    return APS_OK;
}

int aps_loop_info(aps_handle *h, int64_t *loop_steps, int32_t *state, char *why, int32_t why_len) {
    if (!h) return APS_ERR_ARG;
    if (loop_steps) *loop_steps = h->last_loop_steps;
    if (state) *state = h->loop_state;
    if (why && why_len > 0) { std::strncpy(why, h->loop_why.c_str(), (size_t)why_len - 1); why[why_len - 1] = 0; }
    return APS_OK;
}

int aps_step_info(aps_handle *h, int64_t *graph_steps, int64_t *single_steps) {
    if (!h) return APS_ERR_ARG;
    if (graph_steps) *graph_steps = h->last_graph_steps;
    if (single_steps) *single_steps = h->last_single_steps;
    return APS_OK;
}

int aps_copy_bandwidth(aps_handle *h, int64_t nbytes, int32_t reps, double *gbytes_per_s) {
    if (!h || !gbytes_per_s || nbytes < (1 << 20) || reps < 1) return APS_ERR_ARG;
    const size_t n16 = (size_t)nbytes / 16;
    DevMem tmp;
    EventPair ev;
    uint4 *a = nullptr, *b = nullptr;
    HIP_TRY(h, tmp.alloc(&a, n16));
    if (tmp.alloc(&b, n16) != hipSuccess) return fail(h, APS_ERR_HIP, "aps_copy_bandwidth: out of device memory");
    (void)hipMemsetAsync(a, 1, n16 * 16, h->stream);
    (void)ev.create();
    const unsigned blocks = (unsigned)((n16 + 1023) / 1024);
    hipLaunchKernelGGL(copy16, dim3(blocks), dim3(256), 0, h->stream, a, b, n16);
    ev.start(h->stream);
    for (int r = 0; r < reps; ++r) hipLaunchKernelGGL(copy16, dim3(blocks), dim3(256), 0, h->stream, a, b, n16);
    ev.stop(h->stream);
    const hipError_t se = hipStreamSynchronize(h->stream);
    const float ms = ev.ms();
    if (se != hipSuccess || !(ms > 0.f)) return fail(h, APS_ERR_HIP, "aps_copy_bandwidth: copy kernel failed");
    *gbytes_per_s = 2.0 * (double)(n16 * 16) * reps / (ms * 1e-3) / 1e9;
    return APS_OK;
}

int aps_step_timed(aps_handle *h, int64_t nsteps, double *kernel_ms, int64_t *launches, double *work) {
    if (!h) return APS_ERR_ARG;
    if (nsteps < 0 || !kernel_ms) return fail(h, APS_ERR_ARG, "aps_step_timed: bad argument");
    if (h->world != 1) return fail(h, APS_ERR_STATE, "aps_step_timed: sharded handle");
    if (!all_set(h)) return fail(h, APS_ERR_STATE, "aps_step_timed: upload a state for every ensemble first");
    double ms[KIND_N]; int64_t cnt[KIND_N];
    int rc = run_profiled(h, nsteps, ms, cnt, work);
    if (rc) return rc;
    const int kind = is_tiles(h) ? KIND_TILE_STEP : (h->method == APS_METHOD_LATTICE ? KIND_FIELD_UPDATE : KIND_PAIR);
    *kernel_ms = ms[kind];
    if (launches) *launches = cnt[kind];
    return APS_OK;
}

int aps_step_profile(aps_handle *h, int64_t nsteps, double *ms8, int64_t *launches8) {
    if (!h) return APS_ERR_ARG;
    if (nsteps < 0 || !ms8) return fail(h, APS_ERR_ARG, "aps_step_profile: bad argument");
    if (h->world != 1) return fail(h, APS_ERR_STATE, "aps_step_profile: sharded handle");
    if (!all_set(h)) return fail(h, APS_ERR_STATE, "aps_step_profile: upload a state for every ensemble first");
    double ms[KIND_N]; int64_t cnt[KIND_N];
    int rc = run_profiled(h, nsteps, ms, cnt, nullptr);
    if (rc) return rc;
    for (int k = 0; k < 8; ++k) { ms8[k] = ms[k]; if (launches8) launches8[k] = cnt[k]; }
    h->prof_ntt_ms = ms[KIND_NTT]; h->prof_ntt_n = cnt[KIND_NTT];
    return APS_OK;
}

int aps_ntt_info(aps_handle *h, int32_t *on, int32_t *log2_m, double *prof_ms, int64_t *prof_launches) {
    if (!h) return APS_ERR_ARG;
    if (on) *on = h->ntt_on ? 1 : 0;
    if (log2_m) *log2_m = h->ntt_on ? h->ntt.m : 0;
    if (prof_ms) *prof_ms = h->prof_ntt_ms;
    if (prof_launches) *prof_launches = h->prof_ntt_n;
    return APS_OK;
}
int aps_ntt_launches(aps_handle *h) {
    if (!h || !h->ntt_on) return 0;
    return h->ntt_fused ? 3 : h->ntt.a2 > 0 ? 5 : 3;
}

int aps_mark_reference(aps_handle *h, int32_t e) {
    if (!h) return APS_ERR_ARG;
    if (e < 0 || e >= h->E) return fail(h, APS_ERR_ARG, "aps_mark_reference: bad ensemble");
    if (h->n_set[(size_t)e] < 0) return fail(h, APS_ERR_STATE, "aps_mark_reference: no state uploaded for this ensemble");
    { int rc_ = sync_slots(h); if (rc_) return rc_; }
    int rc;
    if (!h->d_ref && (rc = dev_alloc(h, &h->d_ref, (size_t)h->E * h->Npad))) return rc;
    if (h->ref_set.empty()) h->ref_set.assign((size_t)h->E, 0);
    HIP_TRY(h, hipMemcpyAsync(h->d_ref + (size_t)e * h->Npad, h->d_src + (size_t)e * h->Npad, (size_t)h->Npad * 4, hipMemcpyDeviceToDevice, h->stream));
    HIP_TRY(h, hipStreamSynchronize(h->stream));
    h->ref_set[(size_t)e] = 1;
    return APS_OK;
}

}

namespace {
int observe_scalars_impl(aps_handle *h, int e0, int n, int32_t x_wall, const int32_t *lo_hi, int32_t lo, int32_t hi,
                         const uint8_t *block_table, int64_t *out11) {
    const int K = h->p.K, L = h->p.L;
    int rc;
    if ((rc = sync_slots(h))) return rc;
    if (!h->d_cnt_pm && (rc = dev_alloc(h, &h->d_cnt_pm, (size_t)L * h->E))) return rc;
    if (!h->d_scal && ((rc = dev_alloc(h, &h->d_scal, (size_t)16 * h->E)) ||
                       (rc = dev_alloc(h, &h->d_block_table, (size_t)(K + 1) * (K + 1))) || (rc = dev_alloc(h, &h->d_lo_hi, (size_t)2 * h->E)) ||
                       (rc = dev_alloc(h, &h->d_ref_ok, (size_t)h->E)))) return rc;
    std::vector<uint8_t> table((size_t)(K + 1) * (K + 1), 0);
    if (block_table) table.assign(block_table, block_table + table.size());
    else for (int cp = 0; cp <= K; ++cp) for (int cm = 0; cm <= K; ++cm) table[(size_t)cp * (K + 1) + cm] = cp + cm >= 1;
    std::vector<long long> init((size_t)16 * n, 0);
    for (int k = 0; k < n; ++k) init[(size_t)16 * k + SC_MAXPOS] = -1;
    std::vector<uint8_t> ok((size_t)n, 0);
    for (int k = 0; k < n; ++k) ok[(size_t)k] = (!h->ref_set.empty() && h->ref_set[(size_t)(e0 + k)]) ? 1 : 0;
    HIP_TRY(h, hipMemcpyAsync(h->d_block_table, table.data(), table.size(), hipMemcpyHostToDevice, h->stream));
    HIP_TRY(h, hipMemcpyAsync(h->d_scal, init.data(), init.size() * sizeof(long long), hipMemcpyHostToDevice, h->stream));
    HIP_TRY(h, hipMemcpyAsync(h->d_ref_ok, ok.data(), ok.size(), hipMemcpyHostToDevice, h->stream));
    if (lo_hi) HIP_TRY(h, hipMemcpyAsync(h->d_lo_hi, lo_hi, (size_t)2 * n * sizeof(int), hipMemcpyHostToDevice, h->stream));
    HIP_TRY(h, hipMemsetAsync(h->d_cnt_pm, 0, (size_t)L * n * 4, h->stream));
    const uint32_t *src = h->d_src + (size_t)e0 * h->Npad;
    hipLaunchKernelGGL(count_sites, dim3((unsigned)(h->Npad / 256), (unsigned)n), dim3(256), 0, h->stream, src, h->d_cnt_pm, (int)h->Npad, L);
    ScalarArgs a{};
    a.src = src; a.block_table = h->d_block_table; a.cnt_pm = h->d_cnt_pm; a.out = h->d_scal;
    a.ref = h->d_ref ? h->d_ref + (size_t)e0 * h->Npad : nullptr; a.ref_ok = h->d_ref_ok;
    a.lo_hi = lo_hi ? h->d_lo_hi : nullptr;
    a.Npad = (int)h->Npad; a.L = L; a.K = K; a.x_wall = x_wall; a.lo = lo; a.hi = hi;
    hipLaunchKernelGGL(observe_scalars, dim3((unsigned)std::min<int64_t>(h->Npad / 256, 512), (unsigned)n), dim3(256), 0, h->stream, a);
    HIP_TRY(h, hipGetLastError());
    std::vector<long long> res((size_t)16 * n);
    HIP_TRY(h, hipMemcpyAsync(res.data(), h->d_scal, res.size() * sizeof(long long), hipMemcpyDeviceToHost, h->stream));
    HIP_TRY(h, hipStreamSynchronize(h->stream));
    for (int k = 0; k < n; ++k) for (int q = 0; q < SC_COUNT; ++q) out11[(size_t)k * SC_COUNT + q] = res[(size_t)16 * k + q];
    return APS_OK;
}
}

extern "C" {

int aps_observe_scalars(aps_handle *h, int32_t e, int32_t x_wall, int32_t range_lo, int32_t range_hi, const uint8_t *block_table,
                        int64_t *out11) {
    if (!h) return APS_ERR_ARG;
    if (e < 0 || e >= h->E || !out11) return fail(h, APS_ERR_ARG, "aps_observe_scalars: bad argument");
    if (h->n_set[(size_t)e] < 0) return fail(h, APS_ERR_STATE, "aps_observe_scalars: no state uploaded for this ensemble");
    return observe_scalars_impl(h, e, 1, x_wall, nullptr, range_lo, range_hi, block_table, out11);
}

int aps_observe_scalars_all(aps_handle *h, int32_t x_wall, const int32_t *range_lo_hi, const uint8_t *block_table, int64_t *out11) {
    if (!h) return APS_ERR_ARG;
    if (!out11) return fail(h, APS_ERR_ARG, "aps_observe_scalars_all: bad argument");
    if (!all_set(h)) return fail(h, APS_ERR_STATE, "aps_observe_scalars_all: upload a state for every ensemble first");
    return observe_scalars_impl(h, 0, h->E, x_wall, range_lo_hi, 0, -1, block_table, out11);
}

int aps_observe_structure(aps_handle *h, int32_t e, int32_t k_max, double *out) {
    if (!h) return APS_ERR_ARG;
    if (e < 0 || e >= h->E || !out || k_max < 1 || k_max > h->p.L) return fail(h, APS_ERR_ARG, "aps_observe_structure: bad argument");
    if (h->n_set[(size_t)e] < 0) return fail(h, APS_ERR_STATE, "aps_observe_structure: no state uploaded for this ensemble");
    int rc = sync_slots(h);
    if (rc) return rc;
    const int L = h->p.L;
    const size_t nout = 4 + 2 * (size_t)k_max;
    if (!h->d_cnt_pm && (rc = dev_alloc(h, &h->d_cnt_pm, (size_t)L * h->E))) return rc;
    DevMem tmp;
    double *d_out = nullptr;
    HIP_TRY(h, tmp.alloc(&d_out, nout));
// ... 535 lines not shown
```

### hydrodynamic-limits-of-active-particle-systems-with-mean-field-interactions_amd/csrc/tile_loop.hpp

```cpp
#pragma once

constexpr int TL_SEG_MIN = 88;
constexpr int TL_NG = 2;
#ifndef TL_MIN_WAVES
#define TL_MIN_WAVES 2
#endif
constexpr int TL_ABORT = 31;

struct LoopArgs {
    TileArgs a;
    unsigned long long step0;
    int nsteps;
    uint32_t tag0;
    int rec, drec;
    int seg;
    unsigned long long *xrec;
    unsigned *abort_dev, *abort_host;
    unsigned long long timeout_ticks;
#ifdef APS_LOOP_DEBUG
    uint32_t *dbg;
#endif
};

struct TlLds { size_t seg, cells, cells2, props, occ, misc, plist, fw, fs, tab, total; };
__host__ __device__ inline TlLds tl_lds_layout(int tlen, int RS, int own, int K, int wbytes, int seg) {
    TlLds l;
    const size_t TS = 64 * (size_t)RS, ncell = (TS + 2) * K;
    auto up = [](size_t v, size_t a) { return (v + a - 1) / a * a; };
    l.seg = 0;
    l.cells = l.seg + (size_t)FU_WAVES * 4 * (seg + 4) * sizeof(uint32_t);
    l.cells2 = up(l.cells + ncell * 4, 8);
    l.props = up(l.cells2 + (K == 1 ? 0 : ncell * 4), 8);
    l.occ = up(l.props + TS * K, 8);
    l.misc = up(l.occ + TS + 2, 8);
    l.plist = l.misc + 128;
    l.fw = up(l.plist + TS * (size_t)K * 8, 16);
    l.fs = l.fw + TS * wbytes;
    l.tab = up(l.fs + TS * wbytes, 16);
    l.total = l.tab + (size_t)ts_table_chunks(tlen, RS, own, wbytes) * 1024;
    return l;
}

typedef __attribute__((address_space(1))) unsigned long long tl_gu64;
typedef __attribute__((address_space(1))) unsigned tl_gu32;

__device__ __forceinline__ void tl_store_granule(unsigned long long *p, uint32_t tag, uint32_t word) {
    __hip_atomic_store((tl_gu64 *)p, ((unsigned long long)tag << 32) | word, __ATOMIC_RELAXED, __HIP_MEMORY_SCOPE_AGENT);
}
__device__ __forceinline__ unsigned long long tl_load_granule(const unsigned long long *p) {
    return __hip_atomic_load((tl_gu64 *)p, __ATOMIC_RELAXED, __HIP_MEMORY_SCOPE_AGENT);
}

__device__ __forceinline__ void tl_lds_add(double *p, double v) { unsafeAtomicAdd(p, v); }
__device__ __forceinline__ void tl_lds_add(int *p, int v) { atomicAdd(p, v); }

template <int BC, int RS, bool K1, bool F32>
__global__ __launch_bounds__(FU_THREADS, TL_MIN_WAVES) void tile_loop(const LoopArgs la, const void *__restrict__ table_v) {
    using W = typename TsField<F32>::w_t;
    using WS = typename TsField<F32>::ws_t;
    constexpr int SH = TsField<F32>::SH, WB = (int)sizeof(W);
    constexpr bool TAB_LDS = true;
    const TileArgs &a = la.a;
    const W *__restrict__ table_g = reinterpret_cast<const W *>(table_v);
    constexpr int TS = 64 * RS, NOLD = (TS + FU_THREADS - 1) / FU_THREADS;
    constexpr int NSLOT = 16, GB = FU_WAVES * 4;
    const int SEG = la.seg;
    extern __shared__ double lds[];
    const int L = a.L, K = K1 ? 1 : a.K, OWN = a.own;
    const TlLds lay = tl_lds_layout(a.tlen, RS, OWN, K, WB, la.seg);
    char *lds_c = reinterpret_cast<char *>(lds);
    uint32_t *seg_all = reinterpret_cast<uint32_t *>(lds_c + lay.seg);
    uint32_t *cellL = reinterpret_cast<uint32_t *>(lds_c + lay.cells);
    uint32_t *cellN = reinterpret_cast<uint32_t *>(lds_c + lay.cells2);
    uint8_t *propL = reinterpret_cast<uint8_t *>(lds_c + lay.props);
    uint8_t *occL = reinterpret_cast<uint8_t *>(lds_c + lay.occ);
    int *misc = reinterpret_cast<int *>(lds_c + lay.misc);
    uint2 *plist = reinterpret_cast<uint2 *>(lds_c + lay.plist);
    W *fieldW = reinterpret_cast<W *>(lds_c + lay.fw), *fieldS = reinterpret_cast<W *>(lds_c + lay.fs);
    W *tab = reinterpret_cast<W *>(lds_c + lay.tab);
    const int t = threadIdx.x, lane = t & 63, wave = __builtin_amdgcn_readfirstlane(t >> 6), e = blockIdx.y;
    const int tile = (int)blockIdx.x;
    const int own0 = tile * OWN, own_n = min(OWN, L - own0), nfr = own_n + 4;
    const int x0 = own0 - 2;
    const int x0c = max(x0, 0), x1c = min(x0 + nfr - 1, L - 1);
    const int Rt = a.tlen - 1;
    if (__hip_atomic_load((tl_gu32 *)la.abort_dev, __ATOMIC_RELAXED, __HIP_MEMORY_SCOPE_AGENT)) {
        if (t == 0) __hip_atomic_store(la.abort_host, 1u, __ATOMIC_RELAXED, __HIP_MEMORY_SCOPE_SYSTEM);
        return;
    }
    int n_iter = la.nsteps;
    {
        const unsigned stall = la.abort_dev[1];
        if (stall && (int)(stall >> 16) - 1 == tile && e == 0) n_iter = min(n_iter, (int)(stall & 0xFFFFu));
    }
    const uint32_t *__restrict__ cell_e = a.cell_in + (size_t)e * L * K;
    const WS *__restrict__ ws_e = reinterpret_cast<const WS *>(a.ws_in) + (size_t)e * L;
    const uint32_t *__restrict__ dcnt_e = a.dcnt_in + (size_t)e * a.ntile;
    const uint32_t *__restrict__ dep_e = a.dep_in + (size_t)e * a.ntile * a.dcap;
    uint32_t tbase = 0;
    {
        typedef __attribute__((address_space(3))) W lds_w;
        tbase = (uint32_t)(size_t)(lds_w *)tab;
    }
    if (t < 32) misc[t] = 0;
    {
        const int nchunk = ts_table_chunks(a.tlen, RS, OWN, WB);
        const char *srct = reinterpret_cast<const char *>(table_g) + lane * 16;
        for (int c = wave; c < nchunk; c += FU_WAVES) {
            const uint32_t m0v = (uint32_t)__builtin_amdgcn_readfirstlane((int)(tbase + (uint32_t)c * 1024u));
            asm volatile("s_mov_b32 m0, %0\n\tglobal_load_lds_dwordx4 %1, off" :: "s"(m0v), "v"(srct + c * 1024) : "memory");
        }
    }
    const double beta = a.beta[e];
    auto frame_site = [&](int i) -> int {
        if (i < -1 || i > nfr) return -1;
        int s = x0 + i;
        if (BC == 1) { s %= L; if (s < 0) s += L; return s; }
        return (s < 0 || s >= L) ? -1 : s;
    };
    const int ncell = (TS + 2) * K;
    for (int c = t; c < ncell; c += FU_THREADS) {
        const int s = frame_site(c / K - 1);
        const uint32_t v = cell_e[(unsigned)max(s, 0) * (unsigned)K + (unsigned)(c % K)];
        cellL[c] = s >= 0 ? v : CELL_EMPTY;
        if (!K1) cellN[c] = CELL_EMPTY;
    }
#pragma unroll
    for (int r = 0; r < NOLD; ++r) {
        const int xi = r * FU_THREADS + t;
        if (xi < TS) {
            const int s = xi < nfr ? frame_site(xi) : -1;
            WS o = ws_e[(unsigned)max(s, 0)];
            if (s < 0) { o.x = 0; o.y = 0; }
            fieldW[xi] = o.x; fieldS[xi] = o.y;
        }
    }
    for (int i = t; i < (TS * K + 3) / 4; i += FU_THREADS) reinterpret_cast<uint32_t *>(propL)[i] = 0u;
    int b0 = 0, nbk = 0;
    if (BC == 0) {
        b0 = max(0, x0c - Rt - 1) / OWN;
        nbk = min(L - 1, x1c + Rt + 1) / OWN - b0 + 1;
    } else {
        const int lo = x0 - Rt - 1, hi = x0 + nfr - 1 + Rt + 1;
        if (hi - lo + 1 >= L) { b0 = 0; nbk = a.ntile; }
        else {
            const int lom = ((lo % L) + L) % L, him = ((hi % L) + L) % L;
            const int blo = lom / OWN, bhi = him / OWN;
            b0 = blo;
            nbk = (lom <= him) ? bhi - blo + 1 : (a.ntile - blo) + bhi + 1;
            if (nbk > a.ntile) { b0 = 0; nbk = a.ntile; }
        }
    }
    const bool wall = BC == 0 && ((x0c + 1 <= Rt) || (L - x1c <= Rt));
    const bool mirror_ok = 2 * Rt + TS + OWN + 4 < L;
    const int sub = lane >> 4, slot = lane & (NSLOT - 1);
    const uint32_t tlen8 = (uint32_t)a.tlen << SH, L8 = (uint32_t)L << SH;
    uint32_t x8[RS];
#pragma unroll
    for (int r = 0; r < RS; ++r) {
        int s = x0 + r * 64 + lane;
        if (BC == 1) { s %= L; if (s < 0) s += L; } else s = min(max(s, 0), L - 1);
        x8[r] = ((uint32_t)s + TS_BIAS) << SH;
    }
    const int nb_l = tile > 0 ? tile - 1 : (BC == 1 ? a.ntile - 1 : -1), nb_r = tile + 1 < a.ntile ? tile + 1 : (BC == 1 ? 0 : -1);
    const size_t rec_e = (size_t)e * a.ntile;
    const int null_site = x0c;
    const uint32_t tb = tbase;
    uint32_t *dep_o = a.dep_out + ((size_t)e * a.ntile + tile) * a.dcap;
    uint32_t *cell_o = a.cell_out + (size_t)e * L * K;
    const int ngroups = (nbk + GB - 1) / GB;
    const int npass = (wall && mirror_ok) ? 2 : 1;
    auto append = [&](bool occ, int pos, int k, uint32_t cw, int *counter) {
        const unsigned long long mm = __ballot(occ);
        const int cnt_u = __popcll(mm);
        int base = 0;
        if (lane == 0 && cnt_u) base = atomicAdd(counter, cnt_u);
        base = __builtin_amdgcn_readfirstlane(base);
        if (occ) plist[base + __builtin_amdgcn_mbcnt_hi((uint32_t)(mm >> 32), __builtin_amdgcn_mbcnt_lo((uint32_t)mm, 0u))] = make_uint2((uint32_t)pos | ((uint32_t)k << 16), cw);
    };
    asm volatile("s_waitcnt vmcnt(0)" ::: "memory");
    __syncthreads();
    for (int i = t; i < TS + 2; i += FU_THREADS) {
        int n = 0;
        for (int k = 0; k < K; ++k) n += cellL[i * K + k] != CELL_EMPTY;
        occL[i] = (uint8_t)n;
    }
    for (int c0 = 0; c0 < ncell; c0 += FU_THREADS) {
        const int c = c0 + t;
        const int pos = K1 ? c - 1 : c / K - 1, k = K1 ? 0 : c - (pos + 1) * K;
        const uint32_t cw = c < ncell ? cellL[c] : CELL_EMPTY;
        append(cw != CELL_EMPTY && pos >= 0 && pos < nfr, pos, k, cw, misc + 2);
    }
    __syncthreads();

#ifdef APS_LOOP_STAMPS
    unsigned long long st_acc[12] = {0, 0, 0, 0, 0, 0, 0, 0, 0, 0, 0, 0}, st_t0 = __builtin_amdgcn_s_memtime();
    const unsigned long long st_begin = st_t0;
#define TLSTAMP(k) { const unsigned long long t1_ = __builtin_amdgcn_s_memtime(); st_acc[k] += t1_ - st_t0; st_t0 = t1_; }
#else
#define TLSTAMP(k)
#endif
    unsigned long long xg[TL_NG], xh = 0;
#pragma unroll
    for (int g = 0; g < TL_NG; ++g) xg[g] = 0;
    const int h_side = lane >> 5, h_i = lane & 31;
    const int h_nb = h_side ? nb_r : nb_l;
    const bool h_act = wave == FU_WAVES - 1 && h_i < 3 * K && h_nb >= 0;
    auto bucket_of = [&](int j, bool &ok) -> int {
        const int bi = j * GB + sub * FU_WAVES + wave;
        ok = j < ngroups && bi < nbk;
        int b = b0 + (ok ? bi : 0);
        if (b >= a.ntile) b -= a.ntile;
        return b;
    };
    for (int it = 0; it < n_iter; ++it) {
        const unsigned long long step = la.step0 + (unsigned long long)it;
        const uint32_t tag_in = la.tag0 + (uint32_t)it, tag_out = tag_in + 1u;
        const bool first = it == 0, last = it + 1 == la.nsteps;
        const unsigned long long *rec_in = la.xrec + ((size_t)((it + 1) & 1) * a.E * a.ntile + rec_e) * la.rec;
        unsigned long long *rec_out = la.xrec + ((size_t)(it & 1) * a.E * a.ntile + rec_e + tile) * la.rec;
        int *dcount = misc + (it & 1), *pcount = misc + 2 + (it & 1);
        bool gave_up = false;
        const int n0 = *pcount;
        uint2 mine = make_uint2(0u, CELL_EMPTY);
        uint32_t rx[4] = {0u, 0u, 0u, 0u};
        if (t < n0) {
            mine = plist[t];
            philox4x32_10((uint32_t)step, (uint32_t)(step >> 32), mine.y & CELL_ID, (uint32_t)(a.ens_base + e), a.seed_lo, a.seed_hi, rx);
        }
        TLSTAMP(2)
        auto spin_check = [&](unsigned &spins, unsigned long long &t_w) -> bool {
            __builtin_amdgcn_s_sleep(1);
            if ((++spins & 63u) != 0u) return false;
            const bool other = __hip_atomic_load((tl_gu32 *)la.abort_dev, __ATOMIC_RELAXED, __HIP_MEMORY_SCOPE_AGENT) != 0;
            const unsigned long long now = __builtin_amdgcn_s_memrealtime();
            if (!t_w) t_w = now;
            if (!other && now - t_w <= la.timeout_ticks) return false;
            if (!other && lane == 0) {
                __hip_atomic_store((tl_gu32 *)la.abort_dev, 1u, __ATOMIC_RELAXED, __HIP_MEMORY_SCOPE_AGENT);
                __hip_atomic_store(la.abort_host, 1u, __ATOMIC_RELAXED, __HIP_MEMORY_SCOPE_SYSTEM);
            }
            gave_up = true;
            return true;
        };
        auto wait_granule = [&](const unsigned long long *p, bool active) -> uint32_t {
            unsigned long long x = 0, t_w = 0;
            for (unsigned spins = 0;;) {
                if (active) x = tl_load_granule(p);
                if (!__ballot(active && (uint32_t)(x >> 32) != tag_in)) break;
                if (spin_check(spins, t_w)) break;
            }
            return (uint32_t)x;
        };
        if (!first) {
            unsigned long long t_w = 0;
            for (unsigned spins = 0;;) {
                bool bad = false;
#pragma unroll
                for (int g = 0; g < TL_NG; ++g) {
                    bool ok;
                    const int b = bucket_of(g, ok);
                    if (ok && (uint32_t)(xg[g] >> 32) != tag_in) {
                        xg[g] = tl_load_granule(rec_in + (size_t)b * la.rec + slot);
                        bad |= (uint32_t)(xg[g] >> 32) != tag_in;
                    }
                }
                if (h_act && (uint32_t)(xh >> 32) != tag_in) {
                    xh = tl_load_granule(rec_in + (size_t)h_nb * la.rec + la.drec + (h_side ? 0 : 3 * K) + h_i);
                    bad |= (uint32_t)(xh >> 32) != tag_in;
                }
                if (!__ballot(bad)) break;
                if (spin_check(spins, t_w)) break;
            }
            if (wave == FU_WAVES - 1 && !gave_up) {
                const uint32_t v = h_act ? (uint32_t)xh : CELL_EMPTY;
                const int hs = h_i / K, hk = h_i - hs * K, pos = (h_side ? own_n + 2 : -1) + hs;
                if (h_act) cellL[(h_side ? (own_n + 3) * K : 0) + h_i] = v;
                const unsigned long long mo = __ballot(h_act && v != CELL_EMPTY);
                if (h_i < 3 * K && hk == 0 && h_nb >= 0) occL[pos + 1] = (uint8_t)__popcll((mo >> (h_side * 32 + hs * K)) & ((1ull << K) - 1ull));
                const bool hp = h_act && v != CELL_EMPTY && pos >= 0 && pos < nfr;
                const unsigned long long mh = __ballot(hp);
                if (hp) plist[n0 + __builtin_amdgcn_mbcnt_hi((uint32_t)(mh >> 32), __builtin_amdgcn_mbcnt_lo((uint32_t)mh, 0u))] = make_uint2((uint32_t)pos | ((uint32_t)hk << 16), v);
                if (lane == 0) misc[4 + (it & 1)] = __popcll(mh);
            }
        }
        TLSTAMP(0)
        W accP[RS], accM[RS], accF[RS], accWi[RS], accSi[RS];
#pragma unroll
        for (int r = 0; r < RS; ++r) accP[r] = accM[r] = accF[r] = accWi[r] = accSi[r] = 0;
        uint32_t *shl = seg_all;
        const int CAP = (FU_WAVES * 4 * (SEG + 4) / 4) & ~3;
        unsigned long long *shcnt = reinterpret_cast<unsigned long long *>(misc + 8 + 2 * (it & 1));
        auto sweep_now = [&](unsigned long long m, const uint32_t word, const int cls) {
            while (m) {
                const int src_lane = __builtin_ctzll(m);
                m &= m - 1;
                const uint32_t e1 = (uint32_t)__builtin_amdgcn_readlane((int)word, src_lane);
                if (BC == 0) {
                    if (cls == 0) ts_one_abs<RS, 0, F32>(e1, x8, tb, accP);
                    else if (cls == 1) ts_one_abs<RS, 0, F32>(e1, x8, tb, accM);
                    else if (cls == 2) ts_one_abs<RS, 1, F32>(e1, x8, tb, accF);
                    else ts_image_group<TAB_LDS, RS, F32>(make_uint4(e1, DEP_NULL | ((uint32_t)x0c + TS_BIAS), DEP_NULL | ((uint32_t)x0c + TS_BIAS), DEP_NULL | ((uint32_t)x0c + TS_BIAS)),
                                                          x8, tb, table_g, tlen8, L8, accWi, accSi);
                } else {
                    const uint4 q = make_uint4(e1, DEP_NULL | ((uint32_t)null_site + TS_BIAS), DEP_NULL | ((uint32_t)null_site + TS_BIAS), DEP_NULL | ((uint32_t)null_site + TS_BIAS));
                    if (cls == 0) ts_group<1, TAB_LDS, RS, 0, F32>(q, x8, tb, table_g, tlen8, L8, accP);
                    else if (cls == 1) ts_group<1, TAB_LDS, RS, 0, F32>(q, x8, tb, table_g, tlen8, L8, accM);
                    else ts_group<1, TAB_LDS, RS, 1, F32>(q, x8, tb, table_g, tlen8, L8, accF);
                }
            }
        };
#pragma unroll 1
        for (int j = 0; j < ngroups && !gave_up; ++j) {
            bool ok;
            const int b = bucket_of(j, ok);
            uint32_t cnt = 0u;
            if (first) { cnt = min(dcnt_e[(unsigned)b], (uint32_t)a.dcap); if (!ok) cnt = 0u; }
            const unsigned long long *rb = rec_in + (size_t)b * la.rec;
            bool active = ok;
#pragma unroll 1
            for (int page = 0;; ++page) {
                uint32_t en = DEP_NULL;
                bool valid = false, more = false;
                if (first) {
                    const uint32_t k0 = (uint32_t)page * NSLOT;
                    en = dep_e[(unsigned)b * (unsigned)a.dcap + min(k0 + slot, (uint32_t)a.dcap - 1u)];
                    valid = k0 + slot < cnt; more = k0 + NSLOT < cnt;
                } else if (__ballot(active)) {
                    if (page == 0 && j < TL_NG) {
                        unsigned long long x = xg[0];
#pragma unroll
                        for (int g = 1; g < TL_NG; ++g) if (j == g) x = xg[g];
                        en = (uint32_t)x;
                    } else {
                        en = wait_granule(rb + min(page * NSLOT + slot, la.drec - 1), active);
                        if (gave_up) break;
                    }
                    valid = active && en != DEP_NULL;
                    const unsigned long long mv = __ballot(valid);
                    more = active && ((mv >> (sub * 16 + 15)) & 1ull) && (page + 1) * NSLOT < la.drec;
                }
                const uint32_t en_ = en + TS_BIAS;
                if (!wall) {
                    const int cw = (int)((en_ >> 27) & 3u) - 1, cs = (int)(en_ >> 29) - 2;
                    const bool cP = valid && cw != 0 && cw == cs, cM = valid && cw != 0 && cw != cs, cF = valid && cw == 0;
                    const unsigned long long kP = __ballot(cP), kM = __ballot(cM), kF = __ballot(cF);
                    const unsigned long long add = (unsigned long long)__popcll(kP) | ((unsigned long long)__popcll(kM) << 16) | ((unsigned long long)__popcll(kF) << 32);
                    if (add) {
                        unsigned long long base = 0;
                        if (lane == 0) base = atomicAdd(shcnt, add);
                        const uint32_t blo = (uint32_t)__builtin_amdgcn_readfirstlane((int)(uint32_t)base), bhi = (uint32_t)__builtin_amdgcn_readfirstlane((int)(uint32_t)(base >> 32));
                        const bool room = (int)(blo & 0xFFFFu) + __popcll(kP) <= CAP && (int)(blo >> 16) + __popcll(kM) <= CAP && (int)(bhi & 0xFFFFu) + __popcll(kF) <= CAP;
#define TL_POOL(MASK, COND, WORD, CLS, BASE) { \
                        const int i_ = (int)(BASE) + (int)__builtin_amdgcn_mbcnt_hi((uint32_t)((MASK) >> 32), __builtin_amdgcn_mbcnt_lo((uint32_t)(MASK), 0u)); \
                        if ((COND) && (room || i_ < CAP)) shl[(CLS) * CAP + i_] = (WORD); \
                        if (!room) { const unsigned long long o_ = __ballot((COND) && i_ >= CAP); if (o_) sweep_now(o_, (WORD), (CLS)); } }
                        TL_POOL(kP, cP, en_, 0, blo & 0xFFFFu) TL_POOL(kM, cM, en_, 1, blo >> 16) TL_POOL(kF, cF, en_, 2, bhi & 0xFFFFu)
#undef TL_POOL
                    }
                    active = more;
                    if (!__ballot(active)) break;
                    continue;
                }
                const int dp = (int)(en & POS_MASK), cw = (int)((en_ >> 27) & 3u) - 1, cs = (int)(en_ >> 29) - 2;
                const bool img_l = valid && wall && (x0c + dp + 1 <= Rt), img_r = valid && wall && (2 * L - 1 - x1c - dp <= Rt);
                const bool cP = cw != 0 && cw == cs, cM = cw != 0 && cw != cs, cF = cw == 0;
                const bool im = img_l || img_r;
                const bool pl = valid && (mirror_ok || !im), mi = im && mirror_ok, ii = valid && im && !mirror_ok;
                const uint32_t mir = (en_ & ~POS_MASK) | (uint32_t)((int)TS_BIAS + (img_l ? -1 - dp : 2 * L - 1 - dp));
                const unsigned long long kP = __ballot(pl && cP), kM = __ballot(pl && cM), kF = __ballot(pl && cF);
                const unsigned long long gP = __ballot(mi && cP), gM = __ballot(mi && cM), gF = __ballot(mi && cF), kI = __ballot(ii);
                const unsigned long long add = (unsigned long long)(__popcll(kP) + __popcll(gP)) | ((unsigned long long)(__popcll(kM) + __popcll(gM)) << 16) |
                                               ((unsigned long long)(__popcll(kF) + __popcll(gF)) << 32) | ((unsigned long long)__popcll(kI) << 48);
                if (add) {
                    unsigned long long base = 0;
                    if (lane == 0) base = atomicAdd(shcnt, add);
                    const uint32_t blo = (uint32_t)__builtin_amdgcn_readfirstlane((int)(uint32_t)base), bhi = (uint32_t)__builtin_amdgcn_readfirstlane((int)(uint32_t)(base >> 32));
#define TL_POOL(MASK, COND, WORD, CLS, BASE) { \
                    const int i_ = (int)(BASE) + (int)__builtin_amdgcn_mbcnt_hi((uint32_t)((MASK) >> 32), __builtin_amdgcn_mbcnt_lo((uint32_t)(MASK), 0u)); \
                    if ((COND) && i_ < CAP) shl[(CLS) * CAP + i_] = (WORD); \
                    const unsigned long long o_ = __ballot((COND) && i_ >= CAP); \
                    if (o_) sweep_now(o_, (WORD), (CLS)); }
                    TL_POOL(kP, (pl && cP), en_, 0, blo & 0xFFFFu) TL_POOL(gP, (mi && cP), mir, 0, (blo & 0xFFFFu) + __popcll(kP))
                    TL_POOL(kM, (pl && cM), en_, 1, blo >> 16) TL_POOL(gM, (mi && cM), mir, 1, (blo >> 16) + __popcll(kM))
                    TL_POOL(kF, (pl && cF), en_, 2, bhi & 0xFFFFu) TL_POOL(gF, (mi && cF), mir, 2, (bhi & 0xFFFFu) + __popcll(kF))
                    TL_POOL(kI, ii, en_, 3, bhi >> 16)
#undef TL_POOL
                }
                active = more;
                if (!__ballot(active)) break;
            }
        }
        if (gave_up && lane == 0) misc[TL_ABORT] = 1;
        TLSTAMP(8)
        __syncthreads();
        TLSTAMP(9)
        if (misc[TL_ABORT]) return;
        {
            const unsigned long long tot = *shcnt;
            const int nP = min((int)(tot & 0xFFFFu), CAP), nM = min((int)((tot >> 16) & 0xFFFFu), CAP), nF = min((int)((tot >> 32) & 0xFFFFu), CAP),
                      nI = min((int)(tot >> 48), CAP);
            const uint32_t nullw = DEP_NULL | ((uint32_t)null_site + TS_BIAS);
            int rot = wave;
#define TL_SHARED(CLS, N, CALL4) { \
            const int ng_ = ((N) + 3) >> 2; \
            const uint4 *l4 = reinterpret_cast<const uint4 *>(shl + (CLS) * CAP); \
            int g = rot & 3; \
            uint4 q = l4[min(g, CAP / 4 - 1)]; \
            _Pragma("unroll 1") for (; g < ng_; g += FU_WAVES) { \
                const uint4 qn = l4[min(g + FU_WAVES, CAP / 4 - 1)]; \
                if (4 * g + 3 >= (N)) {                         \
                    if (4 * g + 1 >= (N)) q.y = nullw; \
                    if (4 * g + 2 >= (N)) q.z = nullw; \
                    q.w = nullw; } \
                CALL4; \
                q = qn; } \
            rot = (rot - ng_) & 3; }
            if (BC == 1) {
                TL_SHARED(0, nP, (ts_group<1, TAB_LDS, RS, 0, F32>(q, x8, tb, table_g, tlen8, L8, accP)))
                TL_SHARED(1, nM, (ts_group<1, TAB_LDS, RS, 0, F32>(q, x8, tb, table_g, tlen8, L8, accM)))
                TL_SHARED(2, nF, (ts_group<1, TAB_LDS, RS, 1, F32>(q, x8, tb, table_g, tlen8, L8, accF)))
            } else {
                TL_SHARED(0, nP, (ts_group<0, TAB_LDS, RS, 0, F32>(q, x8, tb, table_g, tlen8, L8, accP)))
                TL_SHARED(1, nM, (ts_group<0, TAB_LDS, RS, 0, F32>(q, x8, tb, table_g, tlen8, L8, accM)))
                TL_SHARED(2, nF, (ts_group<0, TAB_LDS, RS, 1, F32>(q, x8, tb, table_g, tlen8, L8, accF)))
            }
#undef TL_SHARED
            if (nI) {
                const uint32_t nulli = DEP_NULL | ((uint32_t)x0c + TS_BIAS);
                const uint4 *l4 = reinterpret_cast<const uint4 *>(shl + 3 * CAP);
#pragma unroll 1
                for (int g = rot & 3; g < (nI + 3) >> 2; g += FU_WAVES) {
                    uint4 q = l4[g];
                    if (4 * g + 1 >= nI) q.y = nulli;
                    if (4 * g + 2 >= nI) q.z = nulli;
                    if (4 * g + 3 >= nI) q.w = nulli;
                    ts_image_group<TAB_LDS, RS, F32>(q, x8, tb, table_g, tlen8, L8, accWi, accSi);
                }
            }
        }
        TLSTAMP(10)
#pragma unroll
        for (int r = 0; r < RS; ++r) {
            const W dw = (accP[r] + accM[r]) + accWi[r], ds = ((accP[r] - accM[r]) + accF[r]) + accSi[r];
            if (dw != 0) tl_lds_add(&fieldW[r * 64 + lane], dw);
            if (ds != 0) tl_lds_add(&fieldS[r * 64 + lane], ds);
        }
        TLSTAMP(11)
        __syncthreads();
        TLSTAMP(7)
        {
            const Model M = *a.model;
            const int n_part = n0 + misc[4 + (it & 1)];
            auto propose_one = [&](const uint2 pc, const uint32_t (&x)[4]) {
                const int pos = (int)(pc.x & 0xFFFFu), k = (int)(pc.x >> 16);
                const int s = frame_site(pos);
                const bool anch = a.anchor ? a.anchor[s] != 0 : false;
                propL[pos * K + k] = decide_proposal(M, anch, s, (pc.y & CELL_PLUS) ? 1 : -1, (pc.y & CELL_BOUND) != 0,
                                                     clip_field((double)fieldS[pos], (double)fieldW[pos]), beta, occL[pos + 1], occL[pos], occL[pos + 2], x);
            };
            if (t < n_part) {
                if (t >= n0) {
                    mine = plist[t];
                    philox4x32_10((uint32_t)step, (uint32_t)(step >> 32), mine.y & CELL_ID, (uint32_t)(a.ens_base + e), a.seed_lo, a.seed_hi, rx);
                }
                propose_one(mine, rx);
            }
            for (int j = FU_THREADS + t; j < n_part; j += FU_THREADS) {
                const uint2 pc = plist[j];
                uint32_t x[4];
                philox4x32_10((uint32_t)step, (uint32_t)(step >> 32), pc.y & CELL_ID, (uint32_t)(a.ens_base + e), a.seed_lo, a.seed_hi, x);
                propose_one(pc, x);
            }
        }
        __syncthreads();
        TLSTAMP(3)
        auto rank_at = [&](int j, uint32_t id) -> int {
            int n = 0;
            for (int k = 0; k < K; ++k) {
                const uint32_t cl_ = cellL[j * K + k], cr_ = cellL[(j + 2) * K + k];
                const int el = propL[(j - 1) * K + k] & 7, er = propL[(j + 1) * K + k] & 7;
                n += (cl_ != CELL_EMPTY && (el == EV_RIGHT || el == EV_FWD) && (cl_ & CELL_ID) < id);
                n += (cr_ != CELL_EMPTY && er == EV_LEFT && (cr_ & CELL_ID) < id);
            }
            return n;
        };
        auto cap_at = [&](int j) -> int { const int c = K - (int)occL[j + 1]; return c < 1 ? 1 : (c > 32 ? 32 : c); };
        auto put_deposit = [&](int kd, uint32_t d) { if (last) dep_o[kd] = d; else tl_store_granule(rec_out + kd, tag_out, d); };
        auto log_exit = [&](const uint32_t c, const int s) {
            const TileRare R = *a.rare;
            const unsigned kx = atomicAdd(&R.n_exit[e], 1u);
            if ((int)kx < R.exit_cap) {
                double *row = R.exit_log + ((size_t)e * R.exit_cap + kx) * 3;
                row[0] = (double)step; row[1] = (double)s; row[2] = (double)(c & CELL_ID);
            }
            R.src[(size_t)e * R.Npad + R.slot_of[(size_t)e * R.N + (c & CELL_ID)]] =
                (uint32_t)s | DEAD_BIT | ((c & CELL_PLUS) ? SPIN_BIT : 0u) | ((c & CELL_BOUND) ? BOUND_BIT : 0u);
        };
        uint32_t newc[NOLD];
        int newn[NOLD];
#pragma unroll
        for (int r = 0; r < NOLD; ++r) {
            newc[r] = CELL_EMPTY; newn[r] = 0;
            const int xi = r * FU_THREADS + t;
            if (xi < 2 || xi >= 2 + own_n || xi >= TS) continue;
            const int s = frame_site(xi);
            if constexpr (K1) {
                const uint32_t cm2 = cellL[xi - 1], cm1 = cellL[xi], c0 = cellL[xi + 1], cp1 = cellL[xi + 2], cp2 = cellL[xi + 3];
                const int pm2 = propL[xi - 2] & 7, pm1 = propL[xi - 1] & 7, p0 = propL[xi] & 7, pp1 = propL[xi + 1] & 7, pp2 = xi + 2 < TS ? propL[xi + 2] & 7 : 0;
                const bool from_l2 = cm2 != CELL_EMPTY && (pm2 == EV_RIGHT || pm2 == EV_FWD);
                const bool from_l1 = cm1 != CELL_EMPTY && (pm1 == EV_RIGHT || pm1 == EV_FWD);
                const bool from_r1 = cp1 != CELL_EMPTY && pp1 == EV_LEFT;
                const bool from_r2 = cp2 != CELL_EMPTY && pp2 == EV_LEFT;
                uint32_t c = c0;
                if (c != CELL_EMPTY) {
                    const int sgn = (c & CELL_PLUS) ? 1 : -1;
                    uint32_t d0 = 0, d1 = 0;
                    int nd = 0;
                    bool stays = true;
                    if (p0 == EV_LEFT || p0 == EV_RIGHT || p0 == EV_FWD) {
                        const bool left = p0 == EV_LEFT;
                        const int rivals = left ? (int)(from_l2 && (cm2 & CELL_ID) < (c & CELL_ID)) + (int)(false)
                                                : (int)(from_r2 && (cp2 & CELL_ID) < (c & CELL_ID));
                        if (rivals < 1) {
                            stays = false;
                            d0 = deposit(s, -1, -sgn); d1 = deposit(frame_site(left ? xi - 1 : xi + 1), 1, sgn); nd = 2;
                        }
                    } else if (p0 == EV_BIND) c |= CELL_BOUND;
                    else if (p0 == EV_UNBIND) c &= ~CELL_BOUND;
                    else if (p0 == EV_FLIP) { c ^= CELL_PLUS; d0 = deposit(s, 0, -2 * sgn); nd = 1; }
                    if (stays) { newc[r] = c; newn[r] = 1; }
                    if (nd) {
                        const int kd = atomicAdd(dcount, nd);
                        if (kd + nd <= a.dcap) { put_deposit(kd, d0); if (nd == 2) put_deposit(kd + 1, d1); }
                    }
                }
                if (from_l1 && !(from_r1 && (cp1 & CELL_ID) < (cm1 & CELL_ID))) { newc[r] = cm1; newn[r] += 1; }
                if (from_r1 && !(from_l1 && (cm1 & CELL_ID) < (cp1 & CELL_ID))) { newc[r] = cp1; newn[r] += 1; }
                continue;
            }
            uint32_t *outN = cellN + (xi + 1) * K;
            int n_out = 0;
            auto emit = [&](uint32_t c) { if (K1) newc[r] = c; else outN[n_out] = c; ++n_out; };
            for (int k = 0; k < K; ++k) {
                uint32_t c = cellL[(xi + 1) * K + k];
                if (c == CELL_EMPTY) continue;
                const int ev = propL[xi * K + k] & 7, sgn = (c & CELL_PLUS) ? 1 : -1;
                uint32_t d0 = 0, d1 = 0;
                int nd = 0;
                bool stays = true;
                if (ev == EV_LEFT || ev == EV_RIGHT || ev == EV_FWD) {
                    const int j = ev == EV_LEFT ? xi - 1 : xi + 1;
                    if (rank_at(j, c & CELL_ID) < cap_at(j)) {
                        stays = false;
                        d0 = deposit(s, -1, -sgn); d1 = deposit(frame_site(j), 1, sgn); nd = 2;
                    }
                } else if (ev == EV_BIND) c |= CELL_BOUND;
                else if (ev == EV_UNBIND) c &= ~CELL_BOUND;
                else if (ev == EV_FLIP) { c ^= CELL_PLUS; d0 = deposit(s, 0, -2 * sgn); nd = 1; }
                else if (ev == EV_EXIT) { stays = false; log_exit(c, s); d0 = deposit(s, -1, -sgn); nd = 1; }
                if (stays) emit(c);
                if (nd) {
                    const int kd = atomicAdd(dcount, nd);
                    if (kd + nd <= a.dcap) { put_deposit(kd, d0); if (nd == 2) put_deposit(kd + 1, d1); }
                }
            }
            const int cap = cap_at(xi);
            for (int k = 0; k < K; ++k) {
                const uint32_t cl_ = cellL[xi * K + k], cr_ = cellL[(xi + 2) * K + k];
                const int el = propL[(xi - 1) * K + k] & 7, er = propL[(xi + 1) * K + k] & 7;
                if (cl_ != CELL_EMPTY && (el == EV_RIGHT || el == EV_FWD) && rank_at(xi, cl_ & CELL_ID) < cap) emit(cl_);
                if (cr_ != CELL_EMPTY && er == EV_LEFT && rank_at(xi, cr_ & CELL_ID) < cap) emit(cr_);
            }
            if (!K1) for (int k = n_out; k < K; ++k) outN[k] = CELL_EMPTY;
            newn[r] = n_out;
        }
        __syncthreads();
        TLSTAMP(4)
        const int count = min(*dcount, a.dcap);
        int *pnext = misc + 2 + ((it + 1) & 1);
#pragma unroll
        for (int r = 0; r < NOLD; ++r) {
            const int xi = r * FU_THREADS + t;
            const bool mine_site = !(xi < 2 || xi >= 2 + own_n || xi >= TS);
            const int io = xi - 2;
            for (int k = 0; k < K; ++k) {
                uint32_t c = CELL_EMPTY;
                if (mine_site) {
                    c = K1 ? newc[r] : cellN[(xi + 1) * K + k];
                    cellL[(xi + 1) * K + k] = c;
                    if (last) cell_o[(unsigned)frame_site(xi) * (unsigned)K + (unsigned)k] = c;
                    else {
                        if (io < 3) tl_store_granule(rec_out + la.drec + io * K + k, tag_out, c);
                        if (io >= own_n - 3) tl_store_granule(rec_out + la.drec + 3 * K + (io - (own_n - 3)) * K + k, tag_out, c);
                    }
                }
                if (!last) append(mine_site && c != CELL_EMPTY, xi, k, c, pnext);
            }
            if (mine_site) {
                occL[xi + 1] = (uint8_t)newn[r];
                if (last) {
                    WS f; f.x = fieldW[xi]; f.y = fieldS[xi];
                    reinterpret_cast<WS *>(a.ws_out)[(size_t)e * L + (unsigned)frame_site(xi)] = f;
                }
            }
        }
        if (!last && t < NSLOT) {
            const int idx = count + t;
            if (idx < (count / NSLOT + 1) * NSLOT && idx < la.drec) tl_store_granule(rec_out + idx, tag_out, DEP_NULL);
        }
        for (int i = t; i < (TS * K + 3) / 4; i += FU_THREADS) reinterpret_cast<uint32_t *>(propL)[i] = 0u;
        if (t == 0) {
            misc[(it + 1) & 1] = 0;
            misc[2 + (it & 1)] = 0; misc[4 + (it & 1)] = 0;
            misc[8 + 2 * (it & 1)] = 0; misc[9 + 2 * (it & 1)] = 0;
            if (last) {
                a.dcnt_out[(size_t)e * a.ntile + tile] = (uint32_t)count;
                if (tile == 0 && e == 0) a.stepw[(a.par + la.nsteps) & 1] = la.step0 + (unsigned long long)la.nsteps;
            }
        }
        if (!last) {
            const unsigned long long *rn = la.xrec + ((size_t)(it & 1) * a.E * a.ntile + rec_e) * la.rec;
#pragma unroll
            for (int g = 0; g < TL_NG; ++g) {
                bool ok;
                const int b = bucket_of(g, ok);
                xg[g] = ok ? tl_load_granule(rn + (size_t)b * la.rec + slot) : 0ull;
            }
            xh = h_act ? tl_load_granule(rn + (size_t)h_nb * la.rec + la.drec + (h_side ? 0 : 3 * K) + h_i) : 0ull;
        }
        TLSTAMP(5)
        __syncthreads();
    }
#ifdef APS_LOOP_STAMPS
    if (lane == 0 && tile < 512 && e == 0) {
        unsigned long long *o = a.rare->stamps + ((size_t)tile * FU_WAVES + wave) * 16;
        for (int k = 0; k < 12; ++k) o[k] = st_acc[k];
        o[6] = __builtin_amdgcn_s_memtime() - st_begin;
        o[1] = st_acc[8] + st_acc[9] + st_acc[10] + st_acc[11];
    }
#endif
}
```

### hydrodynamic-limits-of-active-particle-systems-with-mean-field-interactions_amd/csrc/tile_step.hpp

```cpp
#pragma once

constexpr uint32_t CELL_EMPTY = 0xFFFFFFFFu, CELL_ID = 0x3FFFFFFFu, CELL_BOUND = 1u << 30, CELL_PLUS = 1u << 31;
constexpr int TS_CREG = 4;

struct TileRare { double *exit_log; unsigned *n_exit; uint32_t *src; const uint32_t *slot_of; unsigned long long *stamps; long long N; int exit_cap, Npad;
                  int rec_lo, rec_hi; };

struct TileArgs {
    int L, K, tlen, own, ntile, dcap, par, tile_lo, field_only, field_mode, ens_base, E, periodic;
    int dense_rt, dense_m;
    int *dense;
    int dense_org, dense_lo, dense_hi, dense_shard;
    uint32_t seed_lo, seed_hi;
    const Model *model;
    const TileRare *rare;
    const void *ws_in; void *ws_out;
    const uint32_t *cell_in; uint32_t *cell_out;
    const uint32_t *dcnt_in, *dep_in;
    uint32_t *dcnt_out, *dep_out;
    const long long *gpart_in; long long *gpart_out;
    unsigned long long *stepw;
    const double *beta; const uint8_t *anchor;
};

template <bool TAB_LDS> struct TsGeom { static constexpr int SB = TAB_LDS ? 4 : 5, NSLOT = 1 << SB, GB = FU_WAVES * (64 >> SB); };

__host__ __device__ inline int ts_table_pad(int RS, int own) { return 64 * RS + own + 2; }
__host__ __device__ inline int ts_table_chunks(int tlen, int RS, int own, int wbytes) { return ((tlen + ts_table_pad(RS, own) + 1) * wbytes + 1023) / 1024; }
constexpr int TS_WH = 8;
__host__ __device__ inline int ts_win_entries(int RS, int own) { return ((TS_WH + 1) * own + 64 * RS + 8 + 127) / 128 * 128; }
constexpr int TS_SHCAP = 320;
constexpr int TS_SEG = 128;
struct TsLds { size_t seg, cells, props, occ, misc, plist, tab, field, total; int Q; bool cells_in_regs; };
__host__ __device__ inline TsLds ts_lds_layout(int tlen, bool tab_lds, int RS, int own, int K, int wbytes = 8) {
    TsLds l;
    const size_t TS = 64 * (size_t)RS;
    const int ncell = (int)(TS + 2) * K;
    l.Q = (ncell + FU_WAVES - 1) / FU_WAVES;
    l.cells_in_regs = l.Q <= 64 * TS_CREG;
    l.seg = 0;
    l.cells = l.seg + (size_t)FU_WAVES * 4 * (TS_SEG + 4) * sizeof(uint32_t);
    l.props = l.cells + ((TS + 2) * K * 4 + 7) / 8 * 8;
    l.occ = l.props + (TS * K + 7) / 8 * 8;
    l.misc = l.occ + (TS + 2 + 7) / 8 * 8;
    l.plist = l.misc + 128;
    l.tab = (l.plist + (l.cells_in_regs ? TS * (size_t)K * 8 : 0) + 15) / 16 * 16;
    const size_t table = tab_lds ? (size_t)ts_table_chunks(tlen, RS, own, wbytes) * 1024 : (size_t)2 * ts_win_entries(RS, own) * wbytes;
    const size_t red = (size_t)FU_WAVES * TS * 2 * wbytes;
    l.field = l.tab + red;
    const size_t after = red + TS * sizeof(double2);
    l.total = l.tab + (table > after ? table : after);
    return l;
}

template <bool F32> struct TsField;
template <> struct TsField<false> { using w_t = double; using ws_t = double2; static constexpr int SH = 3; };
template <> struct TsField<true> { using w_t = int; using ws_t = int2; static constexpr int SH = 2; };

template <bool TAB_LDS, typename W>
__device__ __forceinline__ W ts_table_at(const W *__restrict__ table_g, uint32_t byte_addr) {
    if (TAB_LDS) {
        typedef __attribute__((address_space(3))) const W lds_cw;
        return *reinterpret_cast<lds_cw *>(byte_addr);
    }
    return *reinterpret_cast<const W *>(reinterpret_cast<const char *>(table_g) + byte_addr);
}

__device__ __forceinline__ void ts_acc(double &acc, double w, int c) { acc = fma(w, (double)c, acc); }
__device__ __forceinline__ void ts_acc(int &acc, int w, int c) { asm("v_mad_i32_i24 %0, %1, %2, %0" : "+v"(acc) : "v"(w), "s"(c)); }

__device__ __forceinline__ uint32_t sad3s(uint32_t a, uint32_t b_uniform, uint32_t c) {
    uint32_t d;
    asm("v_sad_u32 %0, %1, %2, %3" : "=v"(d) : "v"(a), "s"(b_uniform), "v"(c));
    return d;
}

template <int VAR, bool TAB_LDS, int RS, bool F32>
__device__ __forceinline__ void ts_weights(const uint32_t (&ent)[4], const uint32_t (&x8)[RS], const uint32_t tbase,
                                           const typename TsField<F32>::w_t *__restrict__ table_g, const uint32_t tlen8, const uint32_t L8,
                                           typename TsField<F32>::w_t (&w)[4][RS]) {
    using W = typename TsField<F32>::w_t;
#pragma unroll
    for (int k = 0; k < 4; ++k) {
        const uint32_t p8 = (ent[k] & POS_MASK) << TsField<F32>::SH;
#pragma unroll
        for (int r = 0; r < RS; ++r) {
            if (VAR == 0) {
                const uint32_t d = sad3s(x8[r], p8, tbase);
                w[k][r] = ts_table_at<TAB_LDS, W>(table_g, TAB_LDS ? d : min(d, tlen8));
            } else {
                const uint32_t d8 = sad3s(x8[r], p8, 0u);
                w[k][r] = ts_table_at<TAB_LDS, W>(table_g, min(min(d8, L8 - d8), tlen8) + tbase);
            }
        }
    }
}

template <int VAR, bool TAB_LDS, int RS, int MODE, bool F32>
__device__ __forceinline__ void ts_group(const uint4 q, const uint32_t (&x8)[RS], const uint32_t tbase,
                                         const typename TsField<F32>::w_t *__restrict__ table_g,
                                         const uint32_t tlen8, const uint32_t L8, typename TsField<F32>::w_t (&acc)[RS]) {
    const uint32_t ent[4] = {(uint32_t)__builtin_amdgcn_readfirstlane((int)q.x), (uint32_t)__builtin_amdgcn_readfirstlane((int)q.y),
                             (uint32_t)__builtin_amdgcn_readfirstlane((int)q.z), (uint32_t)__builtin_amdgcn_readfirstlane((int)q.w)};
    typename TsField<F32>::w_t w[4][RS];
    ts_weights<VAR, TAB_LDS, RS, F32>(ent, x8, tbase, table_g, tlen8, L8, w);
#pragma unroll
    for (int k = 0; k < 4; ++k) {
        const int c = MODE == 0 ? (int)((ent[k] >> 27) & 3u) - 1 : (int)(ent[k] >> 29) - 2;
#pragma unroll
        for (int r = 0; r < RS; ++r) ts_acc(acc[r], w[k][r], c);
    }
}

template <int RS, int MODE, bool F32, int DIR>
__device__ __forceinline__ void ts_group_dir(const uint4 q, const uint32_t xb, typename TsField<F32>::w_t (&acc)[RS]) {
    using W = typename TsField<F32>::w_t;
    typedef __attribute__((address_space(3))) const char lds_cc;
    typedef __attribute__((address_space(3))) const W lds_cw;
    constexpr int SH = TsField<F32>::SH;
    const uint32_t ent[4] = {(uint32_t)__builtin_amdgcn_readfirstlane((int)q.x), (uint32_t)__builtin_amdgcn_readfirstlane((int)q.y),
                             (uint32_t)__builtin_amdgcn_readfirstlane((int)q.z), (uint32_t)__builtin_amdgcn_readfirstlane((int)q.w)};
    W w[4][RS];
#pragma unroll
    for (int k = 0; k < 4; ++k) {
        const uint32_t p8 = (ent[k] & POS_MASK) << SH;
        lds_cc *a0 = reinterpret_cast<lds_cc *>(DIR == 0 ? p8 - xb : xb - p8);
#pragma unroll
        for (int r = 0; r < RS; ++r) w[k][r] = *reinterpret_cast<lds_cw *>(a0 + ((DIR == 0 ? RS - 1 - r : r) * (64 << SH)));
    }
#pragma unroll
    for (int k = 0; k < 4; ++k) {
        const int c = MODE == 0 ? (int)((ent[k] >> 27) & 3u) - 1 : (int)(ent[k] >> 29) - 2;
#pragma unroll
        for (int r = 0; r < RS; ++r) ts_acc(acc[r], w[k][r], c);
    }
}

template <int RS, int MODE, bool F32, int DIR>
__device__ __forceinline__ void ts_one_dir(const uint32_t entry, const uint32_t xb, typename TsField<F32>::w_t (&acc)[RS]) {
    using W = typename TsField<F32>::w_t;
    typedef __attribute__((address_space(3))) const char lds_cc;
    typedef __attribute__((address_space(3))) const W lds_cw;
    constexpr int SH = TsField<F32>::SH;
    const uint32_t ent = (uint32_t)__builtin_amdgcn_readfirstlane((int)entry);
    const uint32_t p8 = (ent & POS_MASK) << SH;
    W w[RS];
    lds_cc *a0 = reinterpret_cast<lds_cc *>(DIR == 0 ? p8 - xb : xb - p8);
#pragma unroll
    for (int r = 0; r < RS; ++r) w[r] = *reinterpret_cast<lds_cw *>(a0 + ((DIR == 0 ? RS - 1 - r : r) * (64 << SH)));
    const int c = MODE == 0 ? (int)((ent >> 27) & 3u) - 1 : (int)(ent >> 29) - 2;
#pragma unroll
    for (int r = 0; r < RS; ++r) ts_acc(acc[r], w[r], c);
}

template <int RS, int MODE, bool F32>
__device__ __forceinline__ void ts_one_abs(const uint32_t entry, const uint32_t (&x8)[RS], const uint32_t tbase, typename TsField<F32>::w_t (&acc)[RS]) {
    using W = typename TsField<F32>::w_t;
    const uint32_t ent = (uint32_t)__builtin_amdgcn_readfirstlane((int)entry);
    const uint32_t p8 = (ent & POS_MASK) << TsField<F32>::SH;
    W w[RS];
#pragma unroll
    for (int r = 0; r < RS; ++r) w[r] = ts_table_at<true, W>(nullptr, sad3s(x8[r], p8, tbase));
    const int c = MODE == 0 ? (int)((ent >> 27) & 3u) - 1 : (int)(ent >> 29) - 2;
#pragma unroll
    for (int r = 0; r < RS; ++r) ts_acc(acc[r], w[r], c);
}

constexpr uint32_t TS_BIAS = 1u << 26;

template <bool TAB_LDS, int RS, bool F32>
__device__ __forceinline__ void ts_image_group(const uint4 q, const uint32_t (&x8)[RS], const uint32_t tbase,
                                               const typename TsField<F32>::w_t *__restrict__ table_g,
                                               const uint32_t tlen8, const uint32_t L8, typename TsField<F32>::w_t (&accW)[RS],
                                               typename TsField<F32>::w_t (&accS)[RS]) {
    using W = typename TsField<F32>::w_t;
    constexpr int SH = TsField<F32>::SH;
    const uint32_t ent[4] = {(uint32_t)__builtin_amdgcn_readfirstlane((int)q.x), (uint32_t)__builtin_amdgcn_readfirstlane((int)q.y),
                             (uint32_t)__builtin_amdgcn_readfirstlane((int)q.z), (uint32_t)__builtin_amdgcn_readfirstlane((int)q.w)};
#pragma unroll
    for (int k = 0; k < 4; ++k) {
        const uint32_t p8 = (ent[k] & POS_MASK) << SH;
        const int cw = (int)((ent[k] >> 27) & 3u) - 1, cs = (int)(ent[k] >> 29) - 2;
#pragma unroll
        for (int r = 0; r < RS; ++r) {
            const uint32_t s8 = x8[r] + p8 + (1u << SH) - 2u * (TS_BIAS << SH);
            const W w = ts_table_at<TAB_LDS, W>(table_g, min(sad3s(x8[r], p8, 0u), tlen8) + tbase) +
                        ts_table_at<TAB_LDS, W>(table_g, min(min(s8, 2u * L8 - s8), tlen8) + tbase);
            ts_acc(accW[r], w, cw);
            ts_acc(accS[r], w, cs);
        }
    }
}

#ifdef APS_TS_WAVES
#define TS_WAVES_ATTR __attribute__((amdgpu_waves_per_eu(APS_TS_WAVES, APS_TS_WAVES)))
#else
#define TS_WAVES_ATTR
#endif
template <int BC, bool TAB_LDS, int RS, bool K1, bool F32>
__global__ TS_WAVES_ATTR __launch_bounds__(FU_THREADS) void tile_step(const TileArgs a, const void *__restrict__ table_v) {
    using W = typename TsField<F32>::w_t;
    using WS = typename TsField<F32>::ws_t;
    constexpr int SH = TsField<F32>::SH, WB = (int)sizeof(W);
    const W *__restrict__ table_g = reinterpret_cast<const W *>(table_v);
    constexpr int TS = 64 * RS, NOLD = (TS + FU_THREADS - 1) / FU_THREADS;
    constexpr int SEG = TS_SEG;
    constexpr int SB = TsGeom<TAB_LDS>::SB, NSLOT = TsGeom<TAB_LDS>::NSLOT, GB = TsGeom<TAB_LDS>::GB;
    constexpr int NR = K1 ? ((TS + 2 + FU_WAVES - 1) / FU_WAVES + 63) / 64 : TS_CREG;
    extern __shared__ double lds[];
    const int L = a.L, K = K1 ? 1 : a.K, OWN = a.own;
    const TsLds lay = ts_lds_layout(a.tlen, TAB_LDS, RS, OWN, K, WB);
    char *lds_c = reinterpret_cast<char *>(lds);
    uint32_t *seg_all = reinterpret_cast<uint32_t *>(lds_c + lay.seg);
    uint32_t *cellL = reinterpret_cast<uint32_t *>(lds_c + lay.cells);
    uint8_t *propL = reinterpret_cast<uint8_t *>(lds_c + lay.props);
    uint8_t *occL = reinterpret_cast<uint8_t *>(lds_c + lay.occ);
    int *misc = reinterpret_cast<int *>(lds_c + lay.misc);
    W *tab = reinterpret_cast<W *>(lds_c + lay.tab);
    WS *red = reinterpret_cast<WS *>(tab);
    double2 *fieldL = reinterpret_cast<double2 *>(lds_c + lay.field);
    const int t = threadIdx.x, lane = t & 63, wave = __builtin_amdgcn_readfirstlane(t >> 6), e = blockIdx.y;
    uint32_t *segP = seg_all + wave * 4 * (SEG + 4), *segM = segP + SEG + 4, *segF = segM + SEG + 4, *segI = segF + SEG + 4;
    uint2 *plist = reinterpret_cast<uint2 *>(lds_c + lay.plist);
    const int tile = a.tile_lo + (int)blockIdx.x;
    const int own0 = tile * OWN, own_n = min(OWN, L - own0), nfr = own_n + 4;
    const int x0 = own0 - 2;
    const int x0c = max(x0, 0), x1c = min(x0 + TS - 1, L - 1);
    const int Rt = a.tlen - 1;
    const uint32_t *__restrict__ cell_e = a.cell_in + (size_t)e * L * K;
    const WS *__restrict__ ws_e = reinterpret_cast<const WS *>(a.ws_in) + (size_t)e * L;
    const uint32_t *__restrict__ dcnt_e = a.dcnt_in + (size_t)e * a.ntile;
    const uint32_t *__restrict__ dep_e = a.dep_in + (size_t)e * a.ntile * a.dcap;
    uint32_t tbase = 0;
    {
        typedef __attribute__((address_space(3))) W lds_w;
        tbase = (uint32_t)(size_t)(lds_w *)tab;
    }
    if (t < 32) misc[t] = 0;
    __syncthreads();
#ifdef APS_STAMPS
    unsigned long long f_cnt = 0, f_stage = 0, f_copy = 0, f_proc = 0, f_part = 0, f_n = 0, t0 = __builtin_amdgcn_s_memtime();
    const unsigned long long f_start = t0, r_start = __builtin_amdgcn_s_memrealtime();
#define TSTAMP(var) { const unsigned long long t1_ = __builtin_amdgcn_s_memtime(); var += t1_ - t0; t0 = t1_; }
#else
#define TSTAMP(var)
#endif
    if (TAB_LDS) {
        const int nchunk = ts_table_chunks(a.tlen, RS, OWN, WB);
        const char *srct = reinterpret_cast<const char *>(table_g) + lane * 16;
        for (int c = wave; c < nchunk; c += FU_WAVES) {
            const uint32_t m0v = (uint32_t)__builtin_amdgcn_readfirstlane((int)(tbase + (uint32_t)c * 1024u));
            asm volatile("s_mov_b32 m0, %0\n\tglobal_load_lds_dwordx4 %1, off" :: "s"(m0v), "v"(srct + c * 1024) : "memory");
        }
    }
    const unsigned long long step = a.stepw[a.par];
    const double beta = a.beta[e];
    if (blockIdx.x == 0 && e == 0 && t == 0 && !a.field_only) a.stepw[a.par ^ 1] = step + 1ull;
    auto frame_site = [&](int i) -> int {
        if (i < -1 || i > nfr) return -1;
        int s = x0 + i;
        if (BC == 1) { s %= L; if (s < 0) s += L; return s; }
        return (s < 0 || s >= L) ? -1 : s;
    };
    const int ncell = (TS + 2) * K, Q = lay.Q;
    const int c_lo = wave * Q, c_hi = min(c_lo + Q, ncell);
    uint32_t creg[NR];
    int cpk[NR];
    const bool regs = K1 || lay.cells_in_regs;
    if (regs) {
#pragma unroll
        for (int u = 0; u < NR; ++u) {
            const int c = c_lo + lane + 64 * u;
            const int pos = K1 ? c - 1 : c / K - 1, k = K1 ? 0 : c - (pos + 1) * K;
            const int s = c < c_hi ? frame_site(pos) : -1;
            creg[u] = cell_e[(unsigned)max(s, 0) * (unsigned)K + (unsigned)k];
            cpk[u] = s < 0 ? -2 : ((pos >= 0 && pos < nfr) ? (pos | (k << 16)) : -1);
        }
    } else {
        for (int c = t; c < ncell; c += FU_THREADS) {
            const int s = frame_site(c / K - 1);
            const uint32_t v = cell_e[(unsigned)max(s, 0) * (unsigned)K + (unsigned)(c % K)];
            cellL[c] = s >= 0 ? v : CELL_EMPTY;
        }
    }
    int b0 = 0, nbk = 0;
    if (a.field_mode) {
        if (BC == 0) {
            b0 = max(0, x0c - Rt - 1) / OWN;
            nbk = min(L - 1, x1c + Rt + 1) / OWN - b0 + 1;
        } else {
            const int lo = x0 - Rt - 1, hi = x0 + TS - 1 + Rt + 1;
            if (hi - lo + 1 >= L) { b0 = 0; nbk = a.ntile; }
            else {
                const int lom = ((lo % L) + L) % L, him = ((hi % L) + L) % L;
                const int blo = lom / OWN, bhi = him / OWN;
                b0 = blo;
                nbk = (lom <= him) ? bhi - blo + 1 : (a.ntile - blo) + bhi + 1;
                if (nbk > a.ntile) { b0 = 0; nbk = a.ntile; }
            }
        }
    }
    const bool wall = BC == 0 && ((x0c + 1 <= Rt) || (L - x1c <= Rt));
    const bool mirror_ok = 2 * Rt + TS + OWN + 4 < L;
    const int sub = lane >> SB, slot = lane & (NSLOT - 1);
    const unsigned slot_c = (unsigned)min(slot, a.dcap - 1);
    uint32_t pre_cnt[FU_PRE], pre_ent[FU_PRE];
#pragma unroll
    for (int j = 0; j < FU_PRE; ++j) {
        const int bi = j * GB + sub * FU_WAVES + wave;
        const bool ok = bi < nbk;
        int b = b0 + (ok ? bi : 0);
        if (b >= a.ntile) b -= a.ntile;
        pre_cnt[j] = dcnt_e[(unsigned)b];
        pre_ent[j] = dep_e[(unsigned)b * (unsigned)a.dcap + slot_c];
        if (!ok) pre_cnt[j] = 0u;
    }
    WS old[NOLD];
#pragma unroll
// ... 419 lines not shown
```

### include/aps.h

```cpp
#ifndef APS_H
#define APS_H

#include <stdint.h>

#ifdef __cplusplus
extern "C" {
#endif

#define APS_OK 0
#define APS_ERR_ARG (-1)
#define APS_ERR_HIP (-2)
#define APS_ERR_STATE (-3)
#define APS_ERR_NODEVICE (-4)

typedef struct aps_handle aps_handle;

typedef struct aps_params {
    int32_t L;
    int32_t K;
    int32_t periodic;
    int32_t minus_anchor;
    int32_t immobilize;
    int32_t suppress_flip;
    int32_t crowding;
    int32_t n_ensembles;
    int64_t n_particles;
    double sigma_grid;
    double rate_diffusion;
    double rate_active;
    double k_on, k_off, k_exit;
    double dt;
    uint64_t seed;
    const double *beta;
    const uint8_t *anchor_mask;
    int32_t device;
    int32_t rank, world;
    int32_t sort_by_site;
    int32_t ensemble_base;
    int32_t method;
    int32_t fp32;
    int32_t halo_interval;
} aps_params;

#define APS_METHOD_AUTO 0
#define APS_METHOD_PAIRS 1
#define APS_METHOD_LATTICE 2
#define APS_METHOD_TILES 3

int aps_device_count(void);
const char *aps_last_error(const aps_handle *h);

int aps_create(const aps_params *p, aps_handle **out);
void aps_destroy(aps_handle *h);

int aps_set_stream(aps_handle *h, void *hip_stream);

int aps_set_state(aps_handle *h, int32_t ensemble, const int32_t *pos, const int8_t *sigma,
                  const uint8_t *bound, const uint8_t *alive, int64_t n);
int aps_get_state(aps_handle *h, int32_t ensemble, int32_t *pos, int8_t *sigma, uint8_t *bound,
                  uint8_t *alive, int64_t n);

int aps_pair_accumulate(aps_handle *h, int32_t ensemble, double *S, double *W, int32_t *occ4, int64_t n);

int aps_lattice_accumulate(aps_handle *h, int32_t ensemble, double *S, double *W, int32_t *occ4, int64_t n);

int aps_get_lattice(aps_handle *h, int32_t ensemble, double *W, double *S, int32_t *occ);

int aps_method(aps_handle *h);

int aps_step(aps_handle *h, int64_t nsteps);

int aps_propose(aps_handle *h);
int aps_commit(aps_handle *h);
int aps_exchange_buffer(aps_handle *h, void **dev_ptr, int64_t *total_bytes, int64_t *my_offset,
                        int64_t *my_bytes);

int aps_bind_exchange_buffer(aps_handle *h, void *dev_ptr, int64_t nbytes);

int aps_comm_unique_id(uint8_t *out128);
int aps_comm_init(aps_handle *h, const uint8_t *id128);
int aps_owned_sites(aps_handle *h, int32_t *lo, int32_t *hi);
int aps_halo_copy(aps_handle *dst, aps_handle *src_neighbour);
int aps_halo_pack(aps_handle *h, int32_t side, uint8_t *host, int64_t cap, int64_t *nbytes);
int aps_halo_unpack(aps_handle *h, int32_t from_side, const uint8_t *host, int64_t nbytes);
int aps_halo_info(aps_handle *h, int32_t *interval, int32_t *age, int32_t *due);
int aps_halo_sizes(aps_handle *h, int64_t send_bytes[2], int64_t recv_bytes[2]);

#define APS_IPC_BLOB_BYTES 256
int aps_ipc_export(aps_handle *h, uint8_t *blob256);
int aps_ipc_connect(aps_handle *h, const uint8_t *left_blob256, const uint8_t *right_blob256);
int aps_exchange_kind(aps_handle *h);

int aps_comm_ranks(aps_handle *h, int32_t *nranks);
int aps_comm_selftest(aps_handle *h, int64_t nbytes);

int aps_observe(aps_handle *h, int32_t ensemble, int64_t *counts_p, int64_t *counts_m, double *m_field);

int aps_mark_reference(aps_handle *h, int32_t ensemble);
int aps_observe_scalars(aps_handle *h, int32_t ensemble, int32_t x_wall, int32_t range_lo, int32_t range_hi,
                        const uint8_t *block_table, int64_t *out11);

int aps_observe_scalars_all(aps_handle *h, int32_t x_wall, const int32_t *range_lo_hi, const uint8_t *block_table,
                            int64_t *out11);

int aps_observe_structure(aps_handle *h, int32_t ensemble, int32_t k_max, double *out);

int aps_observe_bins(aps_handle *h, int32_t ensemble, int32_t nbins, int64_t *plus, int64_t *minus);

int aps_field_from_counts(aps_handle *h, int32_t ensemble, const int64_t *counts_p, const int64_t *counts_m,
                          double *m_field);

int aps_rates_from_field(aps_handle *h, int32_t ensemble, const int32_t *pos, const int8_t *sigma, const uint8_t *bound,
                         int64_t n, const double *m_field, const int64_t *counts_p, const int64_t *counts_m,
                         double *out9n);

int aps_time(aps_handle *h, double *t, int64_t *step_index);

int aps_get_exits(aps_handle *h, int32_t ensemble, double *rows3, int64_t cap_rows, int64_t *n_rows);

int aps_get_table(aps_handle *h, double *out, int32_t cap, int32_t *tlen, int32_t *q);

int aps_resort(aps_handle *h);

int aps_step_timed(aps_handle *h, int64_t nsteps, double *kernel_ms, int64_t *launches, double *work);

int aps_step_info(aps_handle *h, int64_t *graph_steps, int64_t *single_steps);

int aps_set_flip_table(aps_handle *h, const double *table, int32_t n);

int aps_ntt_info(aps_handle *h, int32_t *on, int32_t *log2_m, double *prof_ms, int64_t *prof_launches);
int aps_ntt_launches(aps_handle *h);

int aps_tiles_info(aps_handle *h, int32_t *frame_sites, int32_t *owned_sites, int32_t *n_tiles, int32_t *table_in_lds);

int aps_set_resident_loop(aps_handle *h, int32_t on);
int aps_loop_info(aps_handle *h, int64_t *loop_steps, int32_t *state, char *why, int32_t why_len);
int aps_step_loop_timed(aps_handle *h, int64_t nsteps, double *kernel_ms, int64_t *loop_steps);

int aps_copy_bandwidth(aps_handle *h, int64_t nbytes, int32_t reps, double *gbytes_per_s);

int aps_event_overhead(aps_handle *h, int32_t reps, double *ms_per_pair);

int aps_step_profile(aps_handle *h, int64_t nsteps, double *ms8, int64_t *launches8);

#ifdef __cplusplus
}
#endif
#endif
```

Baseline: 8.218 billion particle-steps/s.

## Encode nearest-neighbour hops as single difference-table entries in resident tile loop

When a particle hops to an adjacent site, the resident tile loop now records one 'hop' entry instead of a remove-plus-add pair of deposits. The field contribution of that entry comes from a precomputed integer table of consecutive weight differences, kept in LDS. This is meant to halve the deposit traffic and field-accumulation work for hops. It costs extra LDS for the difference table, a smaller per-class pool capacity, more ballots per record, and a fallback path for wall images; it is disabled on periodic, f32, or small-box configurations.

Result: slower. 7.084 billion particle-steps/s (-13.8%).

```diff
diff --git a/hydrodynamic-limits-of-active-particle-systems-with-mean-field-interactions_amd/capi.py b/hydrodynamic-limits-of-active-particle-systems-with-mean-field-interactions_amd/capi.py
--- a/hydrodynamic-limits-of-active-particle-systems-with-mean-field-interactions_amd/capi.py
+++ b/hydrodynamic-limits-of-active-particle-systems-with-mean-field-interactions_amd/capi.py
@@ -92,6 +92,7 @@
         "aps_set_resident_loop": (C.c_int, [vp, i32]),
         "aps_step_loop_timed": (C.c_int, [vp, i64, P(dbl), P(i64)]),
         "aps_loop_info": (C.c_int, [vp, P(i64), P(i32), C.c_char_p, i32]),
+        "aps_loop_hops": (C.c_int, [vp, P(i32), C.c_char_p, i32]),
         "aps_copy_bandwidth": (C.c_int, [vp, i64, i32, P(dbl)]),
         "aps_lattice_accumulate": (C.c_int, [vp, i32, vp, vp, vp, i64]),
         "aps_get_lattice": (C.c_int, [vp, i32, vp, vp, vp]),
@@ -333,6 +334,11 @@
         self._ck(self.lib.aps_loop_info(self._h, C.byref(n), C.byref(st), why, 256))
         return n.value, st.value, why.value.decode()
 
+    def loop_hops(self):
+        on, why = C.c_int32(), C.create_string_buffer(256)
+        self._ck(self.lib.aps_loop_hops(self._h, C.byref(on), why, 256))
+        return on.value, why.value.decode()
+
     def copy_bandwidth(self, nbytes=1 << 30, reps=5):
         r = C.c_double()
         self._ck(self.lib.aps_copy_bandwidth(self._h, int(nbytes), int(reps), C.byref(r)))
diff --git a/hydrodynamic-limits-of-active-particle-systems-with-mean-field-interactions_amd/csrc/aps_hip.hip b/hydrodynamic-limits-of-active-particle-systems-with-mean-field-interactions_amd/csrc/aps_hip.hip
--- a/hydrodynamic-limits-of-active-particle-systems-with-mean-field-interactions_amd/csrc/aps_hip.hip
+++ b/hydrodynamic-limits-of-active-particle-systems-with-mean-field-interactions_amd/csrc/aps_hip.hip
@@ -1337,6 +1337,9 @@
     unsigned long long *d_xrec = nullptr;
     unsigned *d_abort = nullptr, *h_abort = nullptr, *h_abort_dev = nullptr;
     int loop_rec = 0, loop_drec = 0, loop_seg = 0;
+    int *d_dtable = nullptr;
+    bool hops_switch = true, loop_hops = false;
+    std::string hops_table_why, loop_hops_why = "the loop has not been looked at yet";
     int loop_state = -2;
     int loop_wanted = 1;
     uint32_t loop_tag = 0;
@@ -2072,13 +2075,31 @@
     if (!fn) return no("no kernel for this frame");
     const int64_t need_per_cu = ((int64_t)h->ts_ntile * h->E + h->num_cu - 1) / h->num_cu;
     h->loop_seg = 0;
+    h->loop_hops = false;
+    const char *hops_no = nullptr;
+    if (!h->hops_switch) hops_no = "switch: APS_LOOP_HOPS=0";
+    else if (h->p.periodic) hops_no = "torus: the one-sided identity fails near the antipode";
+    else if (h->f32) hops_no = "32-bit field keeps plain entries";
+    else if (!(2 * (int64_t)(h->tlen - 1) + 64 * h->ts_RS + h->ts_own + 4 < h->p.L)) hops_no = "small box: deposits with two wall images (image list)";
+    else if (!tl_hops_built(0, h->ts_RS, h->p.K == 1, false)) hops_no = "frame: no registers to spare for site capacity above 1 on frames of 6 x 64 sites";
+    else if (!h->d_dtable) hops_no = h->hops_table_why.c_str();
     size_t lds_total = 0;
-    for (int seg : {256, 192, 128, TL_SEG_MIN}) {
-        const TlLds lay = tl_lds_layout(h->tlen, h->ts_RS, h->ts_own, h->p.K, ts_wbytes(h), seg);
-        if (lay.total > 160 * 1024) continue;
-        if (128 / (int)((lay.total + 1279) / 1280) >= need_per_cu) { h->loop_seg = seg; lds_total = lay.total; break; }
-    }
+    for (int hops = hops_no ? 0 : 1; hops >= 0 && !h->loop_seg; --hops) {
+        for (int seg : {256, 192, 128, TL_SEG_MIN}) {
+            const TlLds lay = tl_lds_layout(h->tlen, h->ts_RS, h->ts_own, h->p.K, ts_wbytes(h), seg, hops);
+            if (lay.total > 160 * 1024) continue;
+            if (128 / (int)((lay.total + 1279) / 1280) >= need_per_cu) { h->loop_seg = seg; h->loop_hops = hops != 0; lds_total = lay.total; break; }
+        }
+        if (hops && !h->loop_seg) hops_no = "LDS: with the difference table the grid is not resident at once";
+    }
+    h->loop_hops_why = h->loop_hops ? "" : (hops_no ? hops_no : "");
     if (!h->loop_seg) return no("more tiles than the device keeps resident at once (LDS)");
+    {
+        TlHops hp{h->d_dtable, 0ull, h->loop_hops ? 1 : 0};
+        const double unit = std::ldexp(1.0, -h->q);
+        std::memcpy(&hp.scale, &unit, sizeof unit);
+        HIP_TRY(h, hipMemcpy(reinterpret_cast<char *>(h->d_rare) + offsetof(TileRare, hop), &hp, sizeof hp, hipMemcpyHostToDevice));
+    }
     if (lds_total > 48 * 1024 && hipFuncSetAttribute(fn, hipFuncAttributeMaxDynamicSharedMemorySize, (int)lds_total) != hipSuccess) { (void)hipGetLastError(); return no("hipFuncSetAttribute failed"); }
     int per_cu = 0;
     if (hipOccupancyMaxActiveBlocksPerMultiprocessor(&per_cu, fn, FU_THREADS, lds_total) != hipSuccess) { (void)hipGetLastError(); return no("occupancy query failed"); }
@@ -2132,7 +2153,7 @@
         }
     }
     const void *fn = tl_kernel(h);
-    const size_t lds = tl_lds_layout(h->tlen, h->ts_RS, h->ts_own, h->p.K, ts_wbytes(h), h->loop_seg).total;
+    const size_t lds = tl_lds_layout(h->tlen, h->ts_RS, h->ts_own, h->p.K, ts_wbytes(h), h->loop_seg, h->loop_hops ? 1 : 0).total;
     const void *table_ptr = h->f32 ? (const void *)h->d_table_i : (const void *)h->d_table;
     void *args[] = {(void *)&la, (void *)&table_ptr};
     const dim3 grid((unsigned)h->ts_ntile, (unsigned)h->E), block(FU_THREADS);
@@ -2551,6 +2572,7 @@
     }
     h->plan_interval = (!p->periodic && !(p->k_exit > 0.0)) ? 8 : 1;
     if (const char *env = std::getenv("APS_PLAN_INTERVAL")) h->plan_interval = std::max(1, std::atoi(env));
+    if (const char *env = std::getenv("APS_LOOP_HOPS")) h->hops_switch = std::atoi(env) != 0;
 
     auto die = [&](int code) { g_create_error = h->err; aps_destroy(h); return code; };
     if (hipSetDevice(p->device) != hipSuccess) { h->err = "hipSetDevice failed"; return die(APS_ERR_HIP); }
@@ -2616,6 +2638,19 @@
                 (rc = dev_alloc(h, &h->d_wsi[0], EL)) || (rc = dev_alloc(h, &h->d_wsi[1], EL))) return die(rc);
             if (hipMemcpyAsync(h->d_table_i, ti.data(), ti.size() * sizeof(int), hipMemcpyHostToDevice, h->stream) != hipSuccess ||
                 hipStreamSynchronize(h->stream) != hipSuccess) { h->err = "integer table upload failed"; return die(APS_ERR_HIP); }
+        }
+        if (!h->f32 && !p->periodic && h->ts_table_in_lds) {
+            std::vector<int> dt(h->table.size());
+            for (size_t i = 0; i < dt.size() && h->hops_table_why.empty(); ++i) {
+                const double d = std::ldexp(h->table[i], h->q) - (i + 1 < dt.size() ? std::ldexp(h->table[i + 1], h->q) : 0.0);
+                if (d != std::nearbyint(d) || std::fabs(d) > 2147483647.0) h->hops_table_why = "table: a weight difference does not fit int32 in units of 2^-q";
+                else dt[i] = (int)d;
+            }
+            if (h->hops_table_why.empty()) {
+                if ((rc = dev_alloc(h, &h->d_dtable, h->table.size() + ((size_t)1 << h->bshift) + 8192))) return die(rc);
+                if (hipMemcpyAsync(h->d_dtable, dt.data(), dt.size() * sizeof(int), hipMemcpyHostToDevice, h->stream) != hipSuccess ||
+                    hipStreamSynchronize(h->stream) != hipSuccess) { h->err = "difference table upload failed"; return die(APS_ERR_HIP); }
+            }
         }
         if ((rc = ntt_setup(h))) return die(rc);
         if (h->world > 1 && (rc = halo_setup(h))) return die(rc);
@@ -2989,6 +3024,17 @@
     return APS_OK;
 }
 
+int aps_loop_hops(aps_handle *h, int32_t *on, char *why, int32_t why_len) {
+    if (!h) return APS_ERR_ARG;
+    const bool used = h->loop_state == 1 && h->loop_hops;
+    if (on) *on = used ? 1 : 0;
+    if (why && why_len > 0) {
+        const std::string w = used ? std::string() : (h->loop_state == 1 || h->loop_state == -2 ? h->loop_hops_why : "loop not used: " + h->loop_why);
+        std::strncpy(why, w.c_str(), (size_t)why_len - 1); why[why_len - 1] = 0;
+    }
+    return APS_OK;
+}
+
 int aps_step_info(aps_handle *h, int64_t *graph_steps, int64_t *single_steps) {
     if (!h) return APS_ERR_ARG;
     if (graph_steps) *graph_steps = h->last_graph_steps;
diff --git a/hydrodynamic-limits-of-active-particle-systems-with-mean-field-interactions_amd/csrc/tile_loop.hpp b/hydrodynamic-limits-of-active-particle-systems-with-mean-field-interactions_amd/csrc/tile_loop.hpp
--- a/hydrodynamic-limits-of-active-particle-systems-with-mean-field-interactions_amd/csrc/tile_loop.hpp
+++ b/hydrodynamic-limits-of-active-particle-systems-with-mean-field-interactions_amd/csrc/tile_loop.hpp
@@ -22,8 +22,10 @@
 #endif
 };
 
-struct TlLds { size_t seg, cells, cells2, props, occ, misc, plist, fw, fs, tab, total; };
-__host__ __device__ inline TlLds tl_lds_layout(int tlen, int RS, int own, int K, int wbytes, int seg) {
+__host__ __device__ constexpr bool tl_hops_built(int BC, int RS, bool K1, bool F32) { return BC == 0 && !F32 && (K1 || RS <= 5); }
+
+struct TlLds { size_t seg, cells, cells2, props, occ, misc, plist, fw, fs, tab, dtab, total; };
+__host__ __device__ inline TlLds tl_lds_layout(int tlen, int RS, int own, int K, int wbytes, int seg, int hops) {
     TlLds l;
     const size_t TS = 64 * (size_t)RS, ncell = (TS + 2) * K;
     auto up = [](size_t v, size_t a) { return (v + a - 1) / a * a; };
@@ -37,7 +39,8 @@
     l.fw = up(l.plist + TS * (size_t)K * 8, 16);
     l.fs = l.fw + TS * wbytes;
     l.tab = up(l.fs + TS * wbytes, 16);
-    l.total = l.tab + (size_t)ts_table_chunks(tlen, RS, own, wbytes) * 1024;
+    l.dtab = l.tab + (size_t)ts_table_chunks(tlen, RS, own, wbytes) * 1024;
+    l.total = l.dtab + (hops ? (size_t)ts_table_chunks(tlen, RS, own, 4) * 1024 : 0);
     return l;
 }
 
@@ -67,7 +70,12 @@
     const int SEG = la.seg;
     extern __shared__ double lds[];
     const int L = a.L, K = K1 ? 1 : a.K, OWN = a.own;
-    const TlLds lay = tl_lds_layout(a.tlen, RS, OWN, K, WB, la.seg);
+    constexpr bool HOPS_C = tl_hops_built(BC, RS, K1, F32);
+    bool hops = false;
+    const int *__restrict__ dtable_g = nullptr;
+    unsigned long long hop_scale = 0ull;
+    if constexpr (HOPS_C) { const TlHops hp = a.rare->hop; hops = hp.on != 0; dtable_g = hp.dtable; hop_scale = hp.scale; }
+    const TlLds lay = tl_lds_layout(a.tlen, RS, OWN, K, WB, la.seg, hops ? 1 : 0);
     char *lds_c = reinterpret_cast<char *>(lds);
     uint32_t *seg_all = reinterpret_cast<uint32_t *>(lds_c + lay.seg);
     uint32_t *cellL = reinterpret_cast<uint32_t *>(lds_c + lay.cells);
@@ -102,6 +110,7 @@
         typedef __attribute__((address_space(3))) W lds_w;
         tbase = (uint32_t)(size_t)(lds_w *)tab;
     }
+    const uint32_t dbase = tbase + (uint32_t)(lay.dtab - lay.tab);
     if (t < 32) misc[t] = 0;
     {
         const int nchunk = ts_table_chunks(a.tlen, RS, OWN, WB);
@@ -109,6 +118,14 @@
         for (int c = wave; c < nchunk; c += FU_WAVES) {
             const uint32_t m0v = (uint32_t)__builtin_amdgcn_readfirstlane((int)(tbase + (uint32_t)c * 1024u));
             asm volatile("s_mov_b32 m0, %0\n\tglobal_load_lds_dwordx4 %1, off" :: "s"(m0v), "v"(srct + c * 1024) : "memory");
+        }
+        if (hops) {
+            const int ndchunk = ts_table_chunks(a.tlen, RS, OWN, 4);
+            const char *srcd = reinterpret_cast<const char *>(dtable_g) + lane * 16;
+            for (int c = wave; c < ndchunk; c += FU_WAVES) {
+                const uint32_t m0v = (uint32_t)__builtin_amdgcn_readfirstlane((int)(dbase + (uint32_t)c * 1024u));
+                asm volatile("s_mov_b32 m0, %0\n\tglobal_load_lds_dwordx4 %1, off" :: "s"(m0v), "v"(srcd + c * 1024) : "memory");
+            }
         }
     }
     const double beta = a.beta[e];
@@ -196,9 +213,12 @@
 #ifdef APS_LOOP_STAMPS
     unsigned long long st_acc[12] = {0, 0, 0, 0, 0, 0, 0, 0, 0, 0, 0, 0}, st_t0 = __builtin_amdgcn_s_memtime();
     const unsigned long long st_begin = st_t0;
+    unsigned long long st_entries = 0;
 #define TLSTAMP(k) { const unsigned long long t1_ = __builtin_amdgcn_s_memtime(); st_acc[k] += t1_ - st_t0; st_t0 = t1_; }
+#define TLCOUNT(n) st_entries += (unsigned long long)(n);
 #else
 #define TLSTAMP(k)
+#define TLCOUNT(n)
 #endif
     unsigned long long xg[TL_NG], xh = 0;
 #pragma unroll
@@ -289,13 +309,18 @@
 #pragma unroll
         for (int r = 0; r < RS; ++r) accP[r] = accM[r] = accF[r] = accWi[r] = accSi[r] = 0;
         uint32_t *shl = seg_all;
-        const int CAP = (FU_WAVES * 4 * (SEG + 4) / 4) & ~3;
+        const int CAP = (hops ? FU_WAVES * 4 * (SEG + 4) / 6 : FU_WAVES * 4 * (SEG + 4) / 4) & ~3;
         unsigned long long *shcnt = reinterpret_cast<unsigned long long *>(misc + 8 + 2 * (it & 1));
+        unsigned long long *shcnt2 = reinterpret_cast<unsigned long long *>(misc + 12 + 2 * (it & 1));
         auto sweep_now = [&](unsigned long long m, const uint32_t word, const int cls) {
             while (m) {
                 const int src_lane = __builtin_ctzll(m);
                 m &= m - 1;
                 const uint32_t e1 = (uint32_t)__builtin_amdgcn_readlane((int)word, src_lane);
+                if constexpr (HOPS_C) {
+                    if (cls == 4) { ts_hop_one<RS>(e1, x8, 2u * dbase, hop_scale, accP); continue; }
+                    if (cls == 5) { ts_hop_one<RS>(e1, x8, 2u * dbase, hop_scale, accM); continue; }
+                }
                 if (BC == 0) {
                     if (cls == 0) ts_one_abs<RS, 0, F32>(e1, x8, tb, accP);
                     else if (cls == 1) ts_one_abs<RS, 0, F32>(e1, x8, tb, accM);
@@ -341,6 +366,52 @@
                     more = active && ((mv >> (sub * 16 + 15)) & 1ull) && (page + 1) * NSLOT < la.drec;
                 }
                 const uint32_t en_ = en + TS_BIAS;
+                if constexpr (HOPS_C) if (hops) {
+                    const uint32_t f = (en_ >> 27) & 3u;
+                    const int dp = (int)(en & POS_MASK), cw = (int)f - 1, cs = (int)(en_ >> 29) - 2;
+                    const bool hop = valid && f == 3u, plain = valid && f != 3u;
+                    const bool img_l = wall && (x0c + dp + 1 <= Rt), img_r = wall && (2 * L - 1 - x1c - dp <= Rt);
+                    const bool im = plain && (img_l || img_r);
+                    const uint32_t mir = (en_ & ~POS_MASK) | (uint32_t)((int)TS_BIAS + (img_l ? -1 - dp : 2 * L - 1 - dp));
+                    const bool cP = cw != 0 && cw == cs, cM = cw != 0 && cw != cs, cF = cw == 0;
+                    const bool sp = ((en_ >> 29) & 1u) != 0u, dr = ((en_ >> 30) & 1u) != 0u;
+                    const int lo = dr ? dp : dp - 1, hi = lo + 1, sg = sp ? 1 : -1;
+                    const bool lft = hi <= x0c, rgt = lo >= x1c;
+                    const bool one = hop && (lft || rgt), two = hop && !(lft || rgt);
+                    const uint32_t hw = (TS_BIAS + (uint32_t)(lft ? hi : lo)) | ((lft == dr) ? (2u << 27) : 0u);
+                    const bool h_il = hop && wall && (x0c + lo + 1 <= Rt), h_ir = hop && wall && !h_il && (2 * L - 1 - x1c - hi <= Rt);
+                    const bool hi_any = h_il || h_ir;
+                    const uint32_t hiw = (uint32_t)((int)TS_BIAS + (h_il ? -1 - lo : 2 * L - 1 - hi)) | (((h_il ? !dr : dr)) ? (2u << 27) : 0u);
+                    const uint32_t w1 = two ? deposit(dp, -1, -sg) + TS_BIAS : en_, w2 = two ? deposit(dr ? dp + 1 : dp - 1, 1, sg) + TS_BIAS : mir;
+                    const bool c1P = (plain && cP) || (two && sp), c1M = (plain && cM) || (two && !sp), c1F = plain && cF;
+                    const bool c2P = (im && cP) || (two && sp), c2M = (im && cM) || (two && !sp), c2F = im && cF;
+                    const bool h1P = one && sp, h1M = one && !sp, h2P = hi_any && sp, h2M = hi_any && !sp;
+                    const unsigned long long k1P = __ballot(c1P), k1M = __ballot(c1M), k1F = __ballot(c1F), k2P = __ballot(c2P), k2M = __ballot(c2M), k2F = __ballot(c2F);
+                    const unsigned long long j1P = __ballot(h1P), j1M = __ballot(h1M), j2P = __ballot(h2P), j2M = __ballot(h2M);
+                    const unsigned long long add = (unsigned long long)(__popcll(k1P) + __popcll(k2P)) | ((unsigned long long)(__popcll(k1M) + __popcll(k2M)) << 16) |
+                                                   ((unsigned long long)(__popcll(k1F) + __popcll(k2F)) << 32);
+                    const unsigned long long addh = (unsigned long long)(__popcll(j1P) + __popcll(j2P)) | ((unsigned long long)(__popcll(j1M) + __popcll(j2M)) << 16);
+                    if (add | addh) {
+                        unsigned long long base = 0, baseh = 0;
+                        if (lane == 0) { if (add) base = atomicAdd(shcnt, add); if (addh) baseh = atomicAdd(shcnt2, addh); }
+                        const uint32_t blo = (uint32_t)__builtin_amdgcn_readfirstlane((int)(uint32_t)base), bhi = (uint32_t)__builtin_amdgcn_readfirstlane((int)(uint32_t)(base >> 32));
+                        const uint32_t bh = (uint32_t)__builtin_amdgcn_readfirstlane((int)(uint32_t)baseh);
+#define TL_POOL(MASK, COND, WORD, CLS, BASE) { \
+                        const int i_ = (int)(BASE) + (int)__builtin_amdgcn_mbcnt_hi((uint32_t)((MASK) >> 32), __builtin_amdgcn_mbcnt_lo((uint32_t)(MASK), 0u)); \
+                        if ((COND) && i_ < CAP) shl[(CLS) * CAP + i_] = (WORD); \
+                        const unsigned long long o_ = __ballot((COND) && i_ >= CAP); \
+                        if (o_) sweep_now(o_, (WORD), (CLS)); }
+                        TL_POOL(k1P, c1P, w1, 0, blo & 0xFFFFu) TL_POOL(k2P, c2P, w2, 0, (blo & 0xFFFFu) + __popcll(k1P))
+                        TL_POOL(k1M, c1M, w1, 1, blo >> 16) TL_POOL(k2M, c2M, w2, 1, (blo >> 16) + __popcll(k1M))
+                        TL_POOL(k1F, c1F, w1, 2, bhi & 0xFFFFu) TL_POOL(k2F, c2F, w2, 2, (bhi & 0xFFFFu) + __popcll(k1F))
+                        TL_POOL(j1P, h1P, hw, 4, bh & 0xFFFFu) TL_POOL(j2P, h2P, hiw, 4, (bh & 0xFFFFu) + __popcll(j1P))
+                        TL_POOL(j1M, h1M, hw, 5, bh >> 16) TL_POOL(j2M, h2M, hiw, 5, (bh >> 16) + __popcll(j1M))
+#undef TL_POOL
+                    }
+                    active = more;
+                    if (!__ballot(active)) break;
+                    continue;
+                }
                 if (!wall) {
                     const int cw = (int)((en_ >> 27) & 3u) - 1, cs = (int)(en_ >> 29) - 2;
                     const bool cP = valid && cw != 0 && cw == cs, cM = valid && cw != 0 && cw != cs, cF = valid && cw == 0;
@@ -424,6 +495,14 @@
                 TL_SHARED(0, nP, (ts_group<0, TAB_LDS, RS, 0, F32>(q, x8, tb, table_g, tlen8, L8, accP)))
                 TL_SHARED(1, nM, (ts_group<0, TAB_LDS, RS, 0, F32>(q, x8, tb, table_g, tlen8, L8, accM)))
                 TL_SHARED(2, nF, (ts_group<0, TAB_LDS, RS, 1, F32>(q, x8, tb, table_g, tlen8, L8, accF)))
+                if constexpr (HOPS_C) if (hops) {
+                    const unsigned long long toth = *shcnt2;
+                    const int nHP = min((int)(toth & 0xFFFFu), CAP), nHM = min((int)((toth >> 16) & 0xFFFFu), CAP);
+                    TL_SHARED(4, nHP, (ts_hop_group<RS>(q, x8, 2u * dbase, hop_scale, accP)))
+                    TL_SHARED(5, nHM, (ts_hop_group<RS>(q, x8, 2u * dbase, hop_scale, accM)))
+                    TLCOUNT(nHP + nHM)
+                }
+                TLCOUNT(nP + nM + nF + nI)
             }
 #undef TL_SHARED
             if (nI) {
@@ -486,6 +565,8 @@
             return n;
         };
         auto cap_at = [&](int j) -> int { const int c = K - (int)occL[j + 1]; return c < 1 ? 1 : (c > 32 ? 32 : c); };
+        const bool hop_rec = hops && !last;
+        auto hop_entry = [&](int s, int sgn, bool right) -> uint32_t { return (uint32_t)s | (3u << 27) | ((uint32_t)((sgn > 0 ? 1 : 0) | (right ? 2 : 0)) << 29); };
         auto put_deposit = [&](int kd, uint32_t d) { if (last) dep_o[kd] = d; else tl_store_granule(rec_out + kd, tag_out, d); };
         auto log_exit = [&](const uint32_t c, const int s) {
             const TileRare R = *a.rare;
@@ -524,7 +605,8 @@
                                                 : (int)(from_r2 && (cp2 & CELL_ID) < (c & CELL_ID));
                         if (rivals < 1) {
                             stays = false;
-                            d0 = deposit(s, -1, -sgn); d1 = deposit(frame_site(left ? xi - 1 : xi + 1), 1, sgn); nd = 2;
+                            if (hop_rec) { d0 = hop_entry(s, sgn, !left); nd = 1; }
+                            else { d0 = deposit(s, -1, -sgn); d1 = deposit(frame_site(left ? xi - 1 : xi + 1), 1, sgn); nd = 2; }
                         }
                     } else if (p0 == EV_BIND) c |= CELL_BOUND;
                     else if (p0 == EV_UNBIND) c &= ~CELL_BOUND;
@@ -553,7 +635,8 @@
                     const int j = ev == EV_LEFT ? xi - 1 : xi + 1;
                     if (rank_at(j, c & CELL_ID) < cap_at(j)) {
                         stays = false;
-                        d0 = deposit(s, -1, -sgn); d1 = deposit(frame_site(j), 1, sgn); nd = 2;
+                        if (hop_rec) { d0 = hop_entry(s, sgn, ev != EV_LEFT); nd = 1; }
+                        else { d0 = deposit(s, -1, -sgn); d1 = deposit(frame_site(j), 1, sgn); nd = 2; }
                     }
                 } else if (ev == EV_BIND) c |= CELL_BOUND;
                 else if (ev == EV_UNBIND) c &= ~CELL_BOUND;
@@ -614,6 +697,7 @@
             misc[(it + 1) & 1] = 0;
             misc[2 + (it & 1)] = 0; misc[4 + (it & 1)] = 0;
             misc[8 + 2 * (it & 1)] = 0; misc[9 + 2 * (it & 1)] = 0;
+            if constexpr (HOPS_C) { misc[12 + 2 * (it & 1)] = 0; misc[13 + 2 * (it & 1)] = 0; }
             if (last) {
                 a.dcnt_out[(size_t)e * a.ntile + tile] = (uint32_t)count;
                 if (tile == 0 && e == 0) a.stepw[(a.par + la.nsteps) & 1] = la.step0 + (unsigned long long)la.nsteps;
@@ -638,6 +722,7 @@
         for (int k = 0; k < 12; ++k) o[k] = st_acc[k];
         o[6] = __builtin_amdgcn_s_memtime() - st_begin;
         o[1] = st_acc[8] + st_acc[9] + st_acc[10] + st_acc[11];
+        o[12] = st_entries;
     }
 #endif
 }
diff --git a/hydrodynamic-limits-of-active-particle-systems-with-mean-field-interactions_amd/csrc/tile_step.hpp b/hydrodynamic-limits-of-active-particle-systems-with-mean-field-interactions_amd/csrc/tile_step.hpp
--- a/hydrodynamic-limits-of-active-particle-systems-with-mean-field-interactions_amd/csrc/tile_step.hpp
+++ b/hydrodynamic-limits-of-active-particle-systems-with-mean-field-interactions_amd/csrc/tile_step.hpp
@@ -3,8 +3,10 @@
 constexpr uint32_t CELL_EMPTY = 0xFFFFFFFFu, CELL_ID = 0x3FFFFFFFu, CELL_BOUND = 1u << 30, CELL_PLUS = 1u << 31;
 constexpr int TS_CREG = 4;
 
+struct TlHops { const int *dtable; unsigned long long scale; int on; };
 struct TileRare { double *exit_log; unsigned *n_exit; uint32_t *src; const uint32_t *slot_of; unsigned long long *stamps; long long N; int exit_cap, Npad;
-                  int rec_lo, rec_hi; };
+                  int rec_lo, rec_hi;
+                  TlHops hop; };
 
 struct TileArgs {
     int L, K, tlen, own, ntile, dcap, par, tile_lo, field_only, field_mode, ens_base, E, periodic;
@@ -164,6 +166,45 @@
     const int c = MODE == 0 ? (int)((ent >> 27) & 3u) - 1 : (int)(ent >> 29) - 2;
 #pragma unroll
     for (int r = 0; r < RS; ++r) ts_acc(acc[r], w[r], c);
+}
+
+__device__ __forceinline__ double ts_hop_coef(const uint32_t ent, const unsigned long long scale_bits) {
+    const uint32_t f = (ent >> 27) & 3u;
+    const unsigned long long b = f == 1u ? 0ull : (scale_bits ^ (f == 0u ? 0x8000000000000000ull : 0ull));
+    return __longlong_as_double((long long)b);
+}
+__device__ __forceinline__ int ts_hop_at(uint32_t byte_addr) {
+    typedef __attribute__((address_space(3))) const int lds_ci;
+    return *reinterpret_cast<lds_ci *>(byte_addr);
+}
+template <int RS>
+__device__ __forceinline__ void ts_hop_group(const uint4 q, const uint32_t (&x8)[RS], const uint32_t dbase2, const unsigned long long scale_bits, double (&acc)[RS]) {
+    const uint32_t ent[4] = {(uint32_t)__builtin_amdgcn_readfirstlane((int)q.x), (uint32_t)__builtin_amdgcn_readfirstlane((int)q.y),
+                             (uint32_t)__builtin_amdgcn_readfirstlane((int)q.z), (uint32_t)__builtin_amdgcn_readfirstlane((int)q.w)};
+    int d[4][RS];
+#pragma unroll
+    for (int k = 0; k < 4; ++k) {
+        const uint32_t p8 = (ent[k] & POS_MASK) << 3;
+#pragma unroll
+        for (int r = 0; r < RS; ++r) d[k][r] = ts_hop_at(sad3s(x8[r], p8, dbase2) >> 1);
+    }
+#pragma unroll
+    for (int k = 0; k < 4; ++k) {
+        const double c = ts_hop_coef(ent[k], scale_bits);
+#pragma unroll
+        for (int r = 0; r < RS; ++r) acc[r] = fma((double)d[k][r], c, acc[r]);
+    }
+}
+template <int RS>
+__device__ __forceinline__ void ts_hop_one(const uint32_t entry, const uint32_t (&x8)[RS], const uint32_t dbase2, const unsigned long long scale_bits, double (&acc)[RS]) {
+    const uint32_t ent = (uint32_t)__builtin_amdgcn_readfirstlane((int)entry);
+    const uint32_t p8 = (ent & POS_MASK) << 3;
+    int d[RS];
+#pragma unroll
+    for (int r = 0; r < RS; ++r) d[r] = ts_hop_at(sad3s(x8[r], p8, dbase2) >> 1);
+    const double c = ts_hop_coef(ent, scale_bits);
+#pragma unroll
+    for (int r = 0; r < RS; ++r) acc[r] = fma((double)d[r], c, acc[r]);
 }
 
 constexpr uint32_t TS_BIAS = 1u << 26;
diff --git a/include/aps.h b/include/aps.h
--- a/include/aps.h
+++ b/include/aps.h
@@ -135,6 +135,7 @@
 
 int aps_set_resident_loop(aps_handle *h, int32_t on);
 int aps_loop_info(aps_handle *h, int64_t *loop_steps, int32_t *state, char *why, int32_t why_len);
+int aps_loop_hops(aps_handle *h, int32_t *on, char *why, int32_t why_len);
 int aps_step_loop_timed(aps_handle *h, int64_t nsteps, double *kernel_ms, int64_t *loop_steps);
 
 int aps_copy_bandwidth(aps_handle *h, int64_t nbytes, int32_t reps, double *gbytes_per_s);
```
